# andreeaiana/newsreclib

Hardware: AMD Instinct MI355X
Metric: impressions/sec (train step) NRMS MINDsmall-shape (higher is better)
Workload: dtype f32 (projections: 3xbf16 split MFMA); 1 GPU; NRMS pretrained-emb (d=300, 15 heads, Q=200) MINDsmall-shaped train step: B=128/GPU, H=50, C=5, L=30, V=70000, dropout 0.2, Adam lr 1e-4 (BASELINE.json configs[1]); global_batch=128, parallelism=dp1, gemm_engine=bf16x3

## Files before the change

### include/newsreclib_amd.h

```cpp
#ifndef NEWSRECLIB_AMD_H
#define NEWSRECLIB_AMD_H

#include <stddef.h>
#include <stdint.h>

#ifdef __cplusplus
extern "C" {
#endif

#define NRL_ABI_VERSION 19

#define NRL_OK 0
#define NRL_E_INVALID (-1)
#define NRL_E_WORKSPACE (-2)
#define NRL_E_HIP (-3)

typedef struct NrlBlockParams {
  const float* in_proj_weight;
  const float* in_proj_bias;
  const float* out_proj_weight;
  const float* out_proj_bias;
  const float* att_weight;
  const float* att_bias;
  const float* att_query;
  int32_t embed_dim;
  int32_t num_heads;
  int32_t query_dim;
  int32_t gemm_engine;
  int32_t options;
} NrlBlockParams;
#define NRL_OPTIONS_EXPLICIT 0x40000000

typedef struct NrlBlockGrads {
  float* in_proj_weight;
  float* in_proj_bias;
  float* out_proj_weight;
  float* out_proj_bias;
  float* att_weight;
  float* att_bias;
  float* att_query;
} NrlBlockGrads;

int nrl_abi_version(void);
const char* nrl_build_id(void);
const char* nrl_last_error(void);

int nrl_set_gemm_engine(int32_t engine);
int nrl_get_gemm_engine(void);

int nrl_set_option(const char* name, int32_t value);
int32_t nrl_get_options(void);

int nrl_prof_enable(int32_t on);
int nrl_prof_read(double* total_ms, int64_t* launches, double* total_flops);

uint32_t nrl_dropout_key(uint64_t seed, uint32_t stream);
int nrl_dropout_mask(uint8_t* keep, int64_t n_elems, double p, uint64_t seed, uint32_t stream,
                     void* stream_handle);

size_t nrl_sort_positions_workspace_bytes(int64_t n, int64_t vocab);
int nrl_sort_positions(const int64_t* ids, int64_t n, int64_t vocab, int64_t* order, void* ws, size_t ws_bytes,
                       void* stream);

size_t nrl_news_encoder_workspace_bytes(int64_t n_news, int32_t seq_len, int32_t embed_dim,
                                        int32_t num_heads, int32_t query_dim);
int nrl_news_encoder_fwd(const NrlBlockParams* p, const float* emb_table, int64_t vocab,
                         const int64_t* ids, int64_t n_news, int32_t seq_len, double p_drop,
                         uint64_t seed, uint32_t stream0, int32_t save_for_backward, float* out,
                         void* ws, size_t ws_bytes, void* stream);
int32_t nrl_token_table_supported(int32_t seq_len, int32_t embed_dim, int32_t num_heads, int32_t query_dim);
size_t nrl_token_table_bytes(int64_t vocab, int32_t embed_dim, int32_t num_heads, int32_t query_dim);
int nrl_token_table_build(const NrlBlockParams* p, const float* emb_table, int64_t vocab, void* table, size_t table_bytes,
                          void* stream);
size_t nrl_news_encoder_fwd_table_workspace_bytes(int64_t n_news, int32_t seq_len, int32_t num_heads);
int nrl_news_encoder_fwd_table(const NrlBlockParams* p, const void* table, size_t table_bytes, int64_t vocab,
                               const int64_t* ids, int64_t n_news, int32_t seq_len, float* out, void* ws, size_t ws_bytes,
                               void* stream);
int nrl_news_encoder_bwd(const NrlBlockParams* p, const NrlBlockGrads* g, const float* emb_table,
                         float* d_emb_table, int64_t vocab, const int64_t* ids, const int64_t* sorted_positions,
                         int64_t n_news, int32_t seq_len, double p_drop, uint64_t seed,
                         uint32_t stream0, const float* d_out, int32_t phase, void* ws,
                         size_t ws_bytes, void* stream);

size_t nrl_user_encoder_workspace_bytes(int64_t batch, int64_t hist_len, int32_t embed_dim,
                                        int32_t num_heads, int32_t query_dim);
int nrl_user_encoder_fwd(const NrlBlockParams* p, const float* hist, int64_t batch,
                         int64_t hist_len, double p_drop, uint64_t seed, uint32_t stream0,
                         int32_t input_dropout, int32_t save_for_backward, float* out, void* ws,
                         size_t ws_bytes, void* stream);
int nrl_user_encoder_bwd(const NrlBlockParams* p, const NrlBlockGrads* g, const float* hist,
                         int64_t batch, int64_t hist_len, double p_drop, uint64_t seed,
                         uint32_t stream0, int32_t input_dropout, const float* d_out, float* d_hist,
                         void* ws, size_t ws_bytes, void* stream);
int nrl_user_encoder_bwd_phase(const NrlBlockParams* p, const NrlBlockGrads* g, const float* hist,
                               int64_t batch, int64_t hist_len, double p_drop, uint64_t seed,
                               uint32_t stream0, int32_t input_dropout, const float* d_out,
                               float* d_hist, int32_t phase, void* ws, size_t ws_bytes, void* stream);

int nrl_to_dense_batch_fwd(const float* x, const int64_t* offsets, int64_t batch, int64_t max_len,
                           int32_t dim, float* dense, void* stream);
int nrl_to_dense_batch_bwd(const float* d_dense, const int64_t* offsets, int64_t batch,
                           int64_t max_len, int32_t dim, int64_t n_rows, float* d_x, void* stream);

int nrl_hist_mean_fwd(const float* hist, const int64_t* offsets, int64_t batch, int64_t max_len,
                      int32_t dim, float* user, void* stream);
int nrl_hist_mean_bwd(const float* d_user, const int64_t* offsets, int64_t batch, int64_t max_len,
                      int32_t dim, float* d_hist, void* stream);

int nrl_dot_scores_fwd(const float* user, const float* cand, int64_t batch, int64_t n_cand,
                       int32_t dim, float* scores, void* stream);
int nrl_dot_scores_bwd(const float* d_scores, const float* user, const float* cand, int64_t batch,
                       int64_t n_cand, int32_t dim, float* d_user, float* d_cand, void* stream);

int nrl_ce_loss_fwd_bwd(const float* scores, const float* y_true, int64_t batch, int64_t n_cand,
                        float grad_scale, float* loss, float* d_scores, void* stream);

int nrl_supcon_loss_fwd_bwd(const float* scores, const float* y_true, const int64_t* cand_sizes, int64_t batch,
                            int64_t n_cand, float temperature, float grad_scale, float* loss, float* d_scores,
                            void* stream);

int nrl_adam_step(float* param, float* grad, float* exp_avg, float* exp_avg_sq, int64_t n,
                  double lr, double beta1, double beta2, double eps, int64_t step, float grad_scale,
                  int32_t zero_grad, void* stream);

int nrl_adam_rows_mark(const int64_t* ids, int64_t n_ids, int64_t rows, int32_t* mark, int64_t step, void* stream);
int nrl_adam_rows_advance(float* param, float* grad, float* exp_avg, float* exp_avg_sq, int64_t rows, int32_t dim,
                          int32_t* last_step, const int32_t* mark, int32_t* status, int64_t stride, int64_t offset,
                          int64_t upto_step, int32_t with_grad, double lr, double beta1, double beta2, double eps,
                          float grad_scale, const int32_t* exclude_mark, int32_t exclude_tag, void* stream);

int nrl_dropout_add_layernorm_fwd(const float* x, const float* residual, const float* gamma, const float* beta, int64_t rows,
                                  int32_t dim, float eps, double p_drop, uint64_t seed, uint32_t stream0, float* z_save,
                                  float* mean_save, float* rstd_save, float* y, void* stream);
int nrl_dropout_add_layernorm_bwd(const float* d_y, const float* z_saved, const float* gamma, const float* mean_saved,
                                  const float* rstd_saved, int64_t rows, int32_t dim, double p_drop, uint64_t seed,
                                  uint32_t stream0, float* d_x, float* d_residual, float* d_gamma, float* d_beta, void* stream);


typedef struct NrlCnnParams {
  const float* conv_weight;
  const float* conv_bias;
  const float* att_weight;
  const float* att_bias;
  const float* att_query;
  int32_t embed_dim;
  int32_t num_filters;
  int32_t window;
  int32_t query_dim;
} NrlCnnParams;

typedef struct NrlCnnGrads {
  float* conv_weight;
  float* conv_bias;
  float* att_weight;
  float* att_bias;
  float* att_query;
} NrlCnnGrads;

size_t nrl_cnn_encoder_workspace_bytes(int64_t n_news, int32_t seq_len, int32_t embed_dim,
                                       int32_t num_filters, int32_t window, int32_t query_dim);
int nrl_cnn_encoder_fwd(const NrlCnnParams* p, const float* emb_table, int64_t vocab,
                        const int64_t* ids, int64_t n_news, int32_t seq_len, double p_drop,
                        uint64_t seed, uint32_t stream0, int32_t save_for_backward, float* out,
                        void* ws, size_t ws_bytes, void* stream);
int nrl_cnn_encoder_bwd(const NrlCnnParams* p, const NrlCnnGrads* g, float* d_emb_table,
                        int64_t vocab, const int64_t* ids, const int64_t* sorted_positions,
                        int64_t n_news, int32_t seq_len, double p_drop, uint64_t seed,
                        uint32_t stream0, const float* d_out, void* ws, size_t ws_bytes,
                        void* stream);

size_t nrl_cnn_mhsa_encoder_workspace_bytes(int64_t n_news, int32_t seq_len, int32_t embed_dim,
                                            int32_t num_filters, int32_t window, int32_t num_heads,
                                            int32_t query_dim);
int nrl_cnn_mhsa_encoder_fwd(const NrlCnnParams* cp, const NrlBlockParams* bp, const float* emb_table,
                             int64_t vocab, const int64_t* ids, int64_t n_news, int32_t seq_len,
                             double p_drop, uint64_t seed, uint32_t stream0, int32_t save_for_backward,
                             float* out, void* ws, size_t ws_bytes, void* stream);
int nrl_cnn_mhsa_encoder_bwd(const NrlCnnParams* cp, const NrlCnnGrads* cg, const NrlBlockParams* bp,
                             const NrlBlockGrads* bg, float* d_emb_table, int64_t vocab,
                             const int64_t* ids, const int64_t* sorted_positions, int64_t n_news,
// ... 398 lines not shown
```

### newsreclib_amd/_lib.py

```python
from __future__ import annotations

import ctypes
import os
from ctypes import POINTER, c_char_p, c_double, c_float, c_int32, c_int64, c_size_t, c_uint8, c_uint32, c_uint64, c_void_p

_PKG = os.path.dirname(os.path.abspath(__file__))
LIB_PATH = os.path.join(_PKG, "libnewsreclib_amd.so")
ABI_VERSION = 19


class NrlBlockParams(ctypes.Structure):
    _fields_ = [
        ("in_proj_weight", c_void_p), ("in_proj_bias", c_void_p),
        ("out_proj_weight", c_void_p), ("out_proj_bias", c_void_p),
        ("att_weight", c_void_p), ("att_bias", c_void_p), ("att_query", c_void_p),
        ("embed_dim", c_int32), ("num_heads", c_int32), ("query_dim", c_int32), ("gemm_engine", c_int32),
        ("options", c_int32),
    ]


OPTIONS_EXPLICIT = 0x40000000


class NrlBlockGrads(ctypes.Structure):
# ... 40 lines not shown

class NrlDknGrads(ctypes.Structure):
    _fields_ = [("word_table", c_void_p), ("entity_table", c_void_p), ("context_table", c_void_p),
                ("transform_matrix", c_void_p), ("transform_bias", c_void_p), ("conv_weight", c_void_p * 4),
                ("conv_bias", c_void_p * 4)]


class NrlDknClickParams(ctypes.Structure):
    _fields_ = [("att_w1", c_void_p), ("att_b1", c_void_p), ("att_w2", c_void_p), ("att_b2", c_void_p),
                ("pred_w1", c_void_p), ("pred_b1", c_void_p), ("pred_w2", c_void_p), ("pred_b2", c_void_p),
                ("hidden", c_int32)]


class NrlDknClickGrads(ctypes.Structure):
    _fields_ = [("att_w1", c_void_p), ("att_b1", c_void_p), ("att_w2", c_void_p), ("att_b2", c_void_p),
                ("pred_w1", c_void_p), ("pred_b1", c_void_p), ("pred_w2", c_void_p), ("pred_b2", c_void_p)]


class NrlGruParams(ctypes.Structure):
    _fields_ = [("weight_ih", c_void_p), ("weight_hh", c_void_p), ("bias_ih", c_void_p), ("bias_hh", c_void_p),
                ("input_dim", c_int32), ("hidden_dim", c_int32)]


class NrlGruGrads(ctypes.Structure):
    _fields_ = [("weight_ih", c_void_p), ("weight_hh", c_void_p), ("bias_ih", c_void_p), ("bias_hh", c_void_p)]


class NrlAddAttParams(ctypes.Structure):
    _fields_ = [("att_weight", c_void_p), ("att_bias", c_void_p), ("att_query", c_void_p),
                ("dim", c_int32), ("query_dim", c_int32)]


class NrlAddAttGrads(ctypes.Structure):
    _fields_ = [("att_weight", c_void_p), ("att_bias", c_void_p), ("att_query", c_void_p)]


class NrlMhaParams(ctypes.Structure):
    _fields_ = [("in_proj_weight", c_void_p), ("in_proj_bias", c_void_p), ("out_proj_weight", c_void_p),
                ("out_proj_bias", c_void_p), ("embed_dim", c_int32), ("num_heads", c_int32), ("scale", ctypes.c_float),
                ("gemm_engine", c_int32)]


class NrlMhaGrads(ctypes.Structure):
    _fields_ = [("in_proj_weight", c_void_p), ("in_proj_bias", c_void_p), ("out_proj_weight", c_void_p),
                ("out_proj_bias", c_void_p)]


SIGNATURES = {
    "nrl_abi_version": (c_int32, []),
    "nrl_build_id": (c_char_p, []),
    "nrl_last_error": (c_char_p, []),
    "nrl_set_gemm_engine": (c_int32, [c_int32]),
    "nrl_get_gemm_engine": (c_int32, []),
    "nrl_set_option": (c_int32, [c_char_p, c_int32]),
    "nrl_get_options": (c_int32, []),
    "nrl_prof_enable": (c_int32, [c_int32]),
    "nrl_prof_read": (c_int32, [POINTER(c_double), POINTER(c_int64), POINTER(c_double)]),
    "nrl_dropout_key": (c_uint32, [c_uint64, c_uint32]),
    "nrl_dropout_mask": (c_int32, [c_void_p, c_int64, c_double, c_uint64, c_uint32, c_void_p]),
    "nrl_sort_positions_workspace_bytes": (c_size_t, [c_int64, c_int64]),
    "nrl_sort_positions": (c_int32, [c_void_p, c_int64, c_int64, c_void_p, c_void_p, c_size_t, c_void_p]),
    "nrl_news_encoder_workspace_bytes": (c_size_t, [c_int64, c_int32, c_int32, c_int32, c_int32]),
    "nrl_news_encoder_fwd": (c_int32, [POINTER(NrlBlockParams), c_void_p, c_int64, c_void_p, c_int64, c_int32,
                                       c_double, c_uint64, c_uint32, c_int32, c_void_p, c_void_p, c_size_t,
                                       c_void_p]),
    "nrl_token_table_supported": (c_int32, [c_int32, c_int32, c_int32, c_int32]),
    "nrl_token_table_bytes": (c_size_t, [c_int64, c_int32, c_int32, c_int32]),
    "nrl_token_table_build": (c_int32, [POINTER(NrlBlockParams), c_void_p, c_int64, c_void_p, c_size_t, c_void_p]),
    "nrl_news_encoder_fwd_table_workspace_bytes": (c_size_t, [c_int64, c_int32, c_int32]),
    "nrl_news_encoder_fwd_table": (c_int32, [POINTER(NrlBlockParams), c_void_p, c_size_t, c_int64, c_void_p, c_int64, c_int32,
                                             c_void_p, c_void_p, c_size_t, c_void_p]),
    "nrl_news_encoder_bwd": (c_int32, [POINTER(NrlBlockParams), POINTER(NrlBlockGrads), c_void_p, c_void_p, c_int64,
                                       c_void_p, c_void_p, c_int64, c_int32, c_double, c_uint64, c_uint32,
                                       c_void_p, c_int32, c_void_p, c_size_t, c_void_p]),
    "nrl_user_encoder_workspace_bytes": (c_size_t, [c_int64, c_int64, c_int32, c_int32, c_int32]),
    "nrl_user_encoder_fwd": (c_int32, [POINTER(NrlBlockParams), c_void_p, c_int64, c_int64, c_double, c_uint64,
                                       c_uint32, c_int32, c_int32, c_void_p, c_void_p, c_size_t, c_void_p]),
    "nrl_user_encoder_bwd": (c_int32, [POINTER(NrlBlockParams), POINTER(NrlBlockGrads), c_void_p, c_int64,
                                       c_int64, c_double, c_uint64, c_uint32, c_int32, c_void_p, c_void_p, c_void_p,
                                       c_size_t, c_void_p]),
    "nrl_user_encoder_bwd_phase": (c_int32, [POINTER(NrlBlockParams), POINTER(NrlBlockGrads), c_void_p, c_int64,
                                             c_int64, c_double, c_uint64, c_uint32, c_int32, c_void_p, c_void_p, c_int32,
                                             c_void_p, c_size_t, c_void_p]),
    "nrl_to_dense_batch_fwd": (c_int32, [c_void_p, c_void_p, c_int64, c_int64, c_int32, c_void_p, c_void_p]),
    "nrl_to_dense_batch_bwd": (c_int32, [c_void_p, c_void_p, c_int64, c_int64, c_int32, c_int64, c_void_p,
                                         c_void_p]),
    "nrl_hist_mean_fwd": (c_int32, [c_void_p, c_void_p, c_int64, c_int64, c_int32, c_void_p, c_void_p]),
    "nrl_hist_mean_bwd": (c_int32, [c_void_p, c_void_p, c_int64, c_int64, c_int32, c_void_p, c_void_p]),
    "nrl_dot_scores_fwd": (c_int32, [c_void_p, c_void_p, c_int64, c_int64, c_int32, c_void_p, c_void_p]),
    "nrl_dot_scores_bwd": (c_int32, [c_void_p, c_void_p, c_void_p, c_int64, c_int64, c_int32, c_void_p,
                                     c_void_p, c_void_p]),
    "nrl_ce_loss_fwd_bwd": (c_int32, [c_void_p, c_void_p, c_int64, c_int64, c_float, c_void_p, c_void_p,
                                      c_void_p]),
    "nrl_supcon_loss_fwd_bwd": (c_int32, [c_void_p, c_void_p, c_void_p, c_int64, c_int64, ctypes.c_float,
                                          ctypes.c_float, c_void_p, c_void_p, c_void_p]),
    "nrl_adam_step": (c_int32, [c_void_p, c_void_p, c_void_p, c_void_p, c_int64, c_double, c_double, c_double,
                                c_double, c_int64, c_float, c_int32, c_void_p]),
    "nrl_adam_rows_mark": (c_int32, [c_void_p, c_int64, c_int64, c_void_p, c_int64, c_void_p]),
    "nrl_adam_rows_advance": (c_int32, [c_void_p, c_void_p, c_void_p, c_void_p, c_int64, c_int32, c_void_p, c_void_p, c_void_p,
                                        c_int64, c_int64, c_int64, c_int32, c_double, c_double, c_double, c_double, c_float,
                                        c_void_p, c_int32, c_void_p]),
    "nrl_dropout_add_layernorm_fwd": (c_int32, [c_void_p, c_void_p, c_void_p, c_void_p, c_int64, c_int32, c_float, c_double,
                                                c_uint64, c_uint32, c_void_p, c_void_p, c_void_p, c_void_p, c_void_p]),
    "nrl_dropout_add_layernorm_bwd": (c_int32, [c_void_p, c_void_p, c_void_p, c_void_p, c_void_p, c_int64, c_int32, c_double,
                                                c_uint64, c_uint32, c_void_p, c_void_p, c_void_p, c_void_p, c_void_p]),
    "nrl_cnn_encoder_workspace_bytes": (c_size_t, [c_int64, c_int32, c_int32, c_int32, c_int32, c_int32]),
    "nrl_cnn_encoder_fwd": (c_int32, [POINTER(NrlCnnParams), c_void_p, c_int64, c_void_p, c_int64, c_int32,
                                      c_double, c_uint64, c_uint32, c_int32, c_void_p, c_void_p, c_size_t,
                                      c_void_p]),
    "nrl_cnn_encoder_bwd": (c_int32, [POINTER(NrlCnnParams), POINTER(NrlCnnGrads), c_void_p, c_int64, c_void_p,
                                      c_void_p, c_int64, c_int32, c_double, c_uint64, c_uint32, c_void_p,
                                      c_void_p, c_size_t, c_void_p]),
    "nrl_cnn_mhsa_encoder_workspace_bytes": (c_size_t, [c_int64, c_int32, c_int32, c_int32, c_int32, c_int32, c_int32]),
    "nrl_cnn_mhsa_encoder_fwd": (c_int32, [POINTER(NrlCnnParams), POINTER(NrlBlockParams), c_void_p, c_int64, c_void_p,
                                           c_int64, c_int32, c_double, c_uint64, c_uint32, c_int32, c_void_p, c_void_p,
                                           c_size_t, c_void_p]),
    "nrl_cnn_mhsa_encoder_bwd": (c_int32, [POINTER(NrlCnnParams), POINTER(NrlCnnGrads), POINTER(NrlBlockParams),
                                           POINTER(NrlBlockGrads), c_void_p, c_int64, c_void_p, c_void_p, c_int64,
                                           c_int32, c_double, c_uint64, c_uint32, c_void_p, c_void_p, c_size_t,
                                           c_void_p]),
    "nrl_npa_encoder_workspace_bytes": (c_size_t, [c_int64, c_int32, c_int32, c_int32, c_int32]),
    "nrl_npa_encoder_fwd": (c_int32, [POINTER(NrlCnnParams), c_void_p, c_int64, c_void_p, c_int64, c_int32, c_void_p,
                                      c_void_p, c_int64, c_double, c_uint64, c_uint32, c_int32, c_void_p, c_void_p,
                                      c_size_t, c_void_p]),
    "nrl_npa_encoder_bwd": (c_int32, [POINTER(NrlCnnParams), POINTER(NrlCnnGrads), c_void_p, c_int64, c_void_p,
                                      c_void_p, c_int64, c_int32, c_void_p, c_void_p, c_void_p, c_int64, c_double,
                                      c_uint64, c_uint32, c_void_p, c_void_p, c_void_p, c_size_t, c_void_p]),
    "nrl_npa_conv_features_workspace_bytes": (c_size_t, [c_int64, c_int32, c_int32, c_int32, c_int32]),
    "nrl_npa_conv_features": (c_int32, [POINTER(NrlCnnParams), c_void_p, c_int64, c_void_p, c_int64, c_int32, c_void_p,
                                        c_void_p, c_size_t, c_void_p]),
    "nrl_npa_cached_scores": (c_int32, [c_void_p, c_int64, c_int32, c_int32, c_void_p, c_int64, c_void_p, c_void_p, c_int64,
                                        c_void_p, c_int64, c_void_p, c_void_p, c_void_p, c_int32, c_int32, c_void_p,
                                        c_void_p, c_void_p]),
    "nrl_npa_user_queries_workspace_bytes": (c_size_t, [POINTER(NrlNpaQueryParams), c_int64]),
    "nrl_npa_user_queries_fwd": (c_int32, [POINTER(NrlNpaQueryParams), c_void_p, c_int64, c_double, c_uint64, c_uint32,
                                           c_void_p, c_void_p, c_void_p]),
    "nrl_npa_user_queries_bwd": (c_int32, [POINTER(NrlNpaQueryParams), POINTER(NrlNpaQueryGrads), c_void_p, c_int64,
                                           c_double, c_uint64, c_uint32, c_void_p, c_void_p, c_void_p, c_size_t,
                                           c_void_p]),
    "nrl_personalized_user_attention_fwd": (c_int32, [c_void_p, c_void_p, c_int64, c_int32, c_int32, c_void_p, c_void_p,
                                                      c_void_p]),
    "nrl_personalized_user_attention_bwd": (c_int32, [c_void_p, c_void_p, c_int64, c_int32, c_int32, c_void_p, c_void_p,
                                                      c_void_p, c_void_p, c_void_p]),
    "nrl_dkn_encoder_workspace_bytes": (c_size_t, [POINTER(NrlDknParams), c_int64, c_int32]),
    "nrl_dkn_encoder_fwd": (c_int32, [POINTER(NrlDknParams), c_void_p, c_void_p, c_int64, c_int32, c_void_p, c_void_p,
                                      c_void_p, c_size_t, c_void_p]),
    "nrl_dkn_encoder_bwd": (c_int32, [POINTER(NrlDknParams), POINTER(NrlDknGrads), c_void_p, c_void_p, c_void_p,
                                      c_void_p, c_int64, c_int32, c_void_p, c_void_p, c_void_p, c_void_p, c_size_t,
                                      c_void_p]),
    "nrl_dkn_click_workspace_bytes": (c_size_t, [c_int64, c_int32, c_int32, c_int32]),
    "nrl_dkn_click_fwd": (c_int32, [POINTER(NrlDknClickParams), c_void_p, c_void_p, c_int32, c_void_p, c_void_p, c_int64,
                                    c_int32, c_int32, c_void_p, c_void_p, c_void_p]),
    "nrl_dkn_click_bwd": (c_int32, [POINTER(NrlDknClickParams), POINTER(NrlDknClickGrads), c_void_p, c_void_p, c_int32,
                                    c_void_p, c_void_p, c_int64, c_int32, c_int32, c_void_p, c_void_p, c_void_p, c_void_p,
                                    c_void_p, c_size_t, c_void_p]),
    "nrl_dkn_user_query": (c_int32, [POINTER(NrlDknClickParams), c_void_p, c_void_p, c_int32, c_int64, c_int32, c_void_p,
                                     c_void_p, c_void_p]),
    "nrl_dkn_cand_project": (c_int32, [POINTER(NrlDknClickParams), c_void_p, c_int64, c_int32, c_void_p, c_void_p]),
    "nrl_caum_attn_fwd": (c_int32, [c_void_p, c_void_p, c_void_p, c_int64, c_int64, c_int32, c_int32, c_int32, c_float,
                                    c_void_p]),
    "nrl_caum_attn_bwd": (c_int32, [c_void_p, c_void_p, c_void_p, c_void_p, c_void_p, c_int64, c_int64, c_int32, c_int32,
                                    c_int32, c_float, c_void_p]),
    "nrl_caum_dropout": (c_int32, [c_void_p, c_void_p, c_int64, c_double, c_uint64, c_uint32, c_void_p]),
    "nrl_caum_expand_fwd": (c_int32, [c_void_p, c_void_p, c_int64, c_int32, c_int32, c_int32, c_double, c_uint64, c_uint32,
                                      c_void_p, c_void_p, c_void_p]),
    "nrl_caum_expand_bwd": (c_int32, [c_void_p, c_void_p, c_int64, c_int32, c_int32, c_int32, c_double, c_uint64, c_uint32,
# ... 214 lines not shown
```

### newsreclib_amd/abstract_recommender.py

```python
from __future__ import annotations

import contextlib
import json
from typing import Any, Dict, List, Tuple

import numpy as np
import torch
import torch.distributed as dist

from ._lightning import LightningModuleBase
from . import ops
from .dense_batch import dense_rows
from .metrics import StreamingMetrics, aspect_metrics, ranking_metrics
from .news_encoder import token_tables


STEP_OUTPUT_NAMES = ("loss", "preds", "targets", "cand_news_size", "hist_news_size", "target_categories", "target_sentiments",
                     "hist_categories", "hist_sentiments", "user_ids", "cand_news_ids")
_RECS_OUTPUTS = ("user_ids", "cand_news_ids", "preds", "cand_news_size")


class AbstractRecommender(LightningModuleBase):
    device_metrics = False

    def _init_step_outputs(self, outputs: Dict) -> None:
        self.step_outputs = {stage: {key: [] for key in keys} for stage, keys in outputs.items()}
        self.training_step_outputs = {key: [] for key in self.step_outputs.get("train", {})}
        self.val_step_outputs = {key: [] for key in self.step_outputs.get("val", {})}
        self.test_step_outputs = {key: [] for key in self.step_outputs.get("test", {})}
        self._loss_sums = {"train": [0.0, 0], "val": [0.0, 0], "test": [0.0, 0]}
        self.val_loss_best = float("inf")

    def _get_loss(self, criterion: str):
        from .click_predictor import CrossEntropyLoss, SupConLoss
        if criterion == "cross_entropy_loss":
            return CrossEntropyLoss()
        if criterion == "sup_con_loss":
            return SupConLoss()
        if criterion == "dual_loss":
            return CrossEntropyLoss(), SupConLoss()
        raise ValueError(f"Loss not defined: {criterion}")

    def _init_loss(self, loss: str, dual_loss_training: bool, dual_loss_coef) -> None:
        if not dual_loss_training:
            self.criterion = self._get_loss(loss)
            if isinstance(self.criterion, tuple):
                raise ValueError("loss='dual_loss' needs dual_loss_training=True")
        else:
            assert isinstance(dual_loss_coef, float)
            self.ce_criterion, self.scl_criterion = self._get_loss(loss)

    def _loss(self, scores: torch.Tensor, y_true: torch.Tensor, batch: Dict) -> torch.Tensor:
        hp = self.hparams
        if hp.loss == "cross_entropy_loss":
            return self.criterion(scores, y_true)
        sizes = batch["cand_sizes"]
        if not hp.dual_loss_training:
            return self.criterion(scores, y_true, sizes)
        ce_loss = self.ce_criterion(scores, y_true)
        scl_loss = self.scl_criterion(scores, y_true, sizes)
        return (1 - hp.dual_loss_coef) * ce_loss + hp.dual_loss_coef * scl_loss

    def _plm_text_encoder(self, plm_model, frozen_layers, embed_dim, num_heads, query_dim, dropout_probability):
        from .news_encoder import PLM
        assert isinstance(plm_model, str)
        return PLM(plm_model=plm_model, frozen_layers=frozen_layers, embed_dim=embed_dim, use_mhsa=True,
                   apply_reduce_dim=False, reduced_embed_dim=None, num_heads=num_heads, query_dim=query_dim,
                   dropout_probability=dropout_probability)

    def _encode_news(self, batch: Dict, seed=None):
        if self.hparams.use_plm:
            self.news_encoder.share_plm_bodies(batch["x_hist"], batch["x_cand"])
            return (self.news_encoder(batch["x_hist"], seed=seed),
                    self.news_encoder(batch["x_cand"], seed=seed, stream_base=4))
        n_hist = batch["batch_hist"].shape[0]
        news_vector = self.news_encoder(batch["x_all"], seed=seed)
        return ops.split_rows(news_vector, n_hist)

    def _init_embedding(self, filepath: str) -> torch.Tensor:
        return torch.from_numpy(np.load(filepath)).float()

    def model_step(self, batch: Dict) -> Tuple:
        batch = self._prepare(batch)
        B = batch["batch_size"]
        out = self.forward(batch)
        scores, aux = out if isinstance(out, tuple) else (out, None)
        y_true = dense_rows(batch["labels"], batch["batch_cand"], B, batch["max_cand"],
                            batch["cand_offsets"], batch["cand_flat_idx"], max_is_exact=True)
        loss = self._loss(scores, y_true.float(), batch)
        if aux is not None:
            loss = loss + self._aux_loss(batch, aux)

        if batch["labels"].shape[0] == scores.numel():
            preds = scores.detach().reshape(-1)
        else:
            preds = scores.detach().reshape(-1)[batch["cand_flat_idx"]]
        targets = batch["labels"]
        cand_news_size, hist_news_size = batch["cand_sizes"], batch["hist_sizes"]

        def attr(side, name):
            v = batch["x_" + side].get(name)
            return v if v is not None else torch.empty(0, dtype=torch.int64, device=scores.device)

        return (loss, preds, targets, cand_news_size, hist_news_size, attr("cand", "category"),
                attr("cand", "sentiment"), attr("hist", "category"), attr("hist", "sentiment"),
                batch["user_ids"], attr("cand", "news_ids"))

    def _collect_step_outputs(self, outputs_dict, local_vars):
        for key in outputs_dict.keys():
            outputs_dict[key].append(local_vars.get(key, []))
        return outputs_dict

    def _track(self, stage, loss):
        s = self._loss_sums[stage]
        s[0] = s[0] + loss.detach()
        s[1] += 1

    def training_step(self, batch: Dict, batch_idx: int):
        loss, preds, targets, cand_news_size, *_ = self.model_step(batch)
        self._track("train", loss)
        self.training_step_outputs = self._collect_step_outputs(self.training_step_outputs, locals())
        return loss

    def validation_step(self, batch: Dict, batch_idx: int):
        if self.device_metrics:
            return self._device_metrics_step("val", self.val_step_outputs, self.model_step(batch))
        loss, preds, targets, cand_news_size, *_ = self.model_step(batch)
        self._track("val", loss)
        self.val_step_outputs = self._collect_step_outputs(self.val_step_outputs, locals())

    def test_step(self, batch: Dict, batch_idx: int):
        if self.device_metrics:
            return self._device_metrics_step("test", self.test_step_outputs, self.model_step(batch))
        (loss, preds, targets, cand_news_size, hist_news_size, target_categories, target_sentiments,
         hist_categories, hist_sentiments, user_ids, cand_news_ids) = self.model_step(batch)
        self._track("test", loss)
        self.test_step_outputs = self._collect_step_outputs(self.test_step_outputs, locals())

    def _stream_metrics(self, stage: str, outputs: Dict[str, list]) -> StreamingMetrics:
        if self._world() > 1:
            raise NotImplementedError("device_metrics = True runs in a single process: the cross-rank reduction of the metric "
                                      "accumulator is not built; leave the attribute False under data parallelism")
        streams = self.__dict__.setdefault("_stream_metrics_by_stage", {})
        if stage not in streams:
            def ncls(asp, attr):
                wanted = all(k in outputs for k in (f"target_{asp}", f"hist_{asp}", "hist_news_size"))
                return getattr(self, attr, None) if wanted else None
            streams[stage] = StreamingMetrics(self.hparams.top_k_list, ncls("categories", "num_categ_classes"),
                                              ncls("sentiments", "num_sent_classes"))
        return streams[stage]

    def _device_metrics_step(self, stage: str, outputs: Dict[str, list], step: Tuple) -> None:
        self._track(stage, step[0])
        if all(k in outputs for k in ("preds", "targets", "cand_news_size")):
            self._stream_metrics(stage, outputs).update(step)
        if stage == "test" and getattr(self.hparams, "save_recs", False):
            named = dict(zip(STEP_OUTPUT_NAMES, step))
            for k in _RECS_OUTPUTS:
                if k in outputs:
                    outputs[k].append(named[k])

    @staticmethod
    def _world() -> int:
        return dist.get_world_size() if dist.is_available() and dist.is_initialized() else 1

    def _gather_outputs(self, outputs: Dict[str, list]) -> Dict[str, list]:
        if self._world() == 1:
            return outputs
        local = {k: [t.detach().cpu() for t in v if torch.is_tensor(t)] for k, v in outputs.items()}
        gathered: List[Dict[str, list]] = [None] * self._world()
        dist.all_gather_object(gathered, local)
        dev = self.device
        return {k: [t.to(dev) for part in gathered for t in part.get(k, [])] for k in outputs}

    def _epoch_end(self, stage: str, outputs: Dict[str, list]) -> Dict[str, float]:
# ... 101 lines not shown
```

### newsreclib_amd/csrc/nrl_api.hip

```cpp
#include "nrl_api_internal.h"

namespace nrl {

static thread_local char g_err[512] = "";

void set_error(const char* fmt, ...) {
  va_list ap;
  va_start(ap, fmt);
  vsnprintf(g_err, sizeof(g_err), fmt, ap);
  va_end(ap);
}

ProfState g_prof;
std::atomic<int> g_default_engine{ENGINE_BF16X3};
thread_local int t_engine = -1;
thread_local int64_t t_opts = -1;

static const char* const kOptName[O_COUNT] = {"news_fused", "news_fused_bwd", "news_attn_mfma", "news_planes", "news_od_planes",
                                              "news_aa_planes", "wgrad_2step", "wgrad_ws", "rowpanel", "x3_dma", "news_tail",
                                              "news_tail_bwd", "user_fork", "news_fork", "news_qkv_planes", "news_pad_share", "news_tail_od", "user_proj"};
static const char* const kOptEnv[O_COUNT] = {"NRL_NEWS_FUSED", "NRL_NEWS_FUSED_BWD", "NRL_NEWS_ATTN_MFMA", "NRL_NEWS_PLANES",
                                             "NRL_NEWS_OD_PLANES", "NRL_NEWS_AA_PLANES", "NRL_WGRAD_2STEP", "NRL_WGRAD_WS",
                                             "NRL_ROWPANEL", "NRL_X3_DMA", "NRL_NEWS_TAIL", "NRL_NEWS_TAIL_BWD", "NRL_USER_FORK",
                                             "NRL_NEWS_FORK", "NRL_NEWS_QKV_PLANES", "NRL_NEWS_PAD_SHARE", "NRL_NEWS_TAIL_OD", "NRL_USER_PROJ"};
// ... 312 lines not shown
                         float* d_emb_table, int64_t vocab, const int64_t* ids, const int64_t* sorted_positions,
                         int64_t n_news, int32_t seq_len, double p_drop, uint64_t seed, uint32_t stream0,
                         const float* d_out, int32_t phase, void* ws, size_t ws_bytes, void* stream) {
  NRL_TRY(check_params(p));
  const EngineScope engine_scope(p->gemm_engine);
  const OptScope opt_scope(p->options);
  NRL_TRY(check_grads(g));
  NRL_REQUIRE(d_emb_table && ids && d_out && vocab > 0 && n_news >= 0 && seq_len > 0, "news_encoder_bwd: bad arguments");
  NRL_REQUIRE(phase >= 0 && phase <= 2, "news_encoder_bwd: phase must be 0 (all), 1 or 2");
  if (n_news == 0) return NRL_OK;
  hipStream_t st = (hipStream_t)stream;
  const BlockShape s = news_shape(p, n_news, seq_len);
  BlockWs w;
  NRL_TRY(carve_ws(ws, ws_bytes, s, true, &w));
  const Dropout d1 = make_dropout(p_drop, seed, stream0), d2 = make_dropout(p_drop, seed, stream0 + 1);
  BlockPlanes bp;
  const bool slabs = news_fused_on(s, seq_len) && opt(O_NEWS_ATTN_MFMA);
  const bool planes = slabs && opt(O_NEWS_PLANES);
  BlockShape sb_ = s;
  sb_.od_planes = planes && opt(O_NEWS_OD_PLANES);
  sb_.aa_planes = sb_.od_planes && opt(O_NEWS_AA_PLANES) && w.yp != nullptr && (s.D & 15) == 12 && s.Q <= 224;
  sb_.tail = news_tail_on(sb_, seq_len, w);
  sb_.tail_bwd = sb_.tail && sb_.aa_planes && news_tail_bwd_on(sb_, seq_len, w);
  NRL_TRY(block_planes(p, s, w, false, &bp, st, slabs ? s.heads : 0));
  sb_.forked = news_fork_on(sb_);
  SideFork side;
  hipEvent_t side_in_join = nullptr;
  if (phase != 2) {
    if (sb_.forked) {
      ForkSet* fs = nullptr;
      NRL_TRY(fork_set(&fs));
      side.s = fs->s[0]; side.fork = fs->fork; side.join = fs->join[0];
    }
    NRL_TRY(block_bwd_phase1(p, g, sb_, w, bp, d2, d_out, st, slabs, sb_.forked ? &side : nullptr));
    if (slabs) {
      NewsAttnBwdArgs a;
      a.qkv_hm = w.qkv; a.d_o = w.d_o; a.lse = w.lse; a.dqkv = w.dqkv; a.n_news = n_news; a.L = seq_len; a.D = s.D;
      a.heads = s.heads; a.scale = s.geom.scale; a.hpw = 1; a.planes = planes ? 1 : 0;
      if (planes && opt(O_NEWS_QKV_PLANES)) NRL_TRY(launch_news_attn_bwd_p(a, st));
      else NRL_TRY(launch_news_attn_bwd(a, st));
      if (news_fork_in_on(sb_, planes)) {
        ForkSet* fs = nullptr;
        NRL_TRY(fork_set(&fs));
        const int si = news_fork_in_mode() == 2 ? 0 : 1;
        NRL_HIP(hipEventRecord(fs->fork, st));
        NRL_HIP(hipStreamWaitEvent(fs->s[si], fs->fork, 0));
        NRL_TRY(block_wgrad_in_planes(g, w.x, sb_, w, fs->s[si]));
        NRL_HIP(hipEventRecord(fs->join[1], fs->s[si]));
        side_in_join = fs->join[1];
      }
    }
    const KCSlab dq_hp{w.dqkv, s.M};
    const KCPlanes dq_pl{reinterpret_cast<const unsigned char*>(w.dqkv), s.pad_rows};
    if (sorted_positions != nullptr) {
      float* dx = w.d_o;
      const EpiLinear epi{dx, s.D, nullptr, 0, d1, s.D};
      static const bool live_env = [] { const char* e = getenv("NRL_LIVE_ROWS"); return !(e != nullptr && e[0] == '0'); }();
      if (planes && live_env) {
        NRL_REQUIRE((size_t)s.M * s.heads >= live_compact_ints(s.M), "news_encoder_bwd: scratch for the live-row list");
        const int32_t *list = nullptr, *cidx = nullptr, *n_live = nullptr;
        NRL_TRY(live_compact(ids, s.M, reinterpret_cast<int32_t*>(w.lse), &list, &cidx, &n_live, st));
        const KCPlanesLive dq_live{reinterpret_cast<const unsigned char*>(w.dqkv), s.pad_rows, list, n_live, seq_len};
        NRL_TRY(rp_dispatch(dq_live, bp.rp.in_d_hp, EpiDxLive{dx, s.D, d1, list}, s.M, s.D, s.heads * 64, st));
        NRL_TRY(embedding_grad_sorted(dx, ids, sorted_positions, s.M, s.D, d_emb_table, st, cidx));
      } else {
        if (planes) NRL_TRY(rp_dispatch(dq_pl, bp.rp.in_d_hp, EpiNewsRows<EpiLinear>{epi, seq_len}, s.pad_rows, s.D, s.heads * 64, st));
        else if (slabs) NRL_TRY(rp_dispatch(dq_hp, bp.rp.in_d_hp, epi, s.M, s.D, s.heads * 64, st));
        else NRL_TRY(gemm_dgrad(w.dqkv, p->in_proj_weight, bp.in, epi, s.M, 3 * s.D, s.D, st, bp.rp.on ? &bp.rp.in_d : nullptr));
        NRL_TRY(embedding_grad_sorted(dx, ids, sorted_positions, s.M, s.D, d_emb_table, st));
      }
    } else {
      const EpiScatter epi{d_emb_table, ids, s.D, d1};
      if (planes) NRL_TRY(rp_dispatch(dq_pl, bp.rp.in_d_hp, EpiNewsRows<EpiScatter>{epi, seq_len}, s.pad_rows, s.D, s.heads * 64, st));
      else if (slabs) NRL_TRY(rp_dispatch(dq_hp, bp.rp.in_d_hp, epi, s.M, s.D, s.heads * 64, st));
      else NRL_TRY(gemm_dgrad(w.dqkv, p->in_proj_weight, bp.in, epi, s.M, 3 * s.D, s.D, st, bp.rp.on ? &bp.rp.in_d : nullptr));
    }
  }
  if (phase != 2 && sb_.forked) NRL_HIP(hipStreamWaitEvent(st, side.join, 0));
  if (side_in_join != nullptr) NRL_HIP(hipStreamWaitEvent(st, side_in_join, 0));
  if (phase != 1) NRL_TRY(block_bwd_phase2(g, w.x, sb_, w, st, slabs, planes));
  return NRL_OK;
}

size_t nrl_user_encoder_workspace_bytes(int64_t batch, int64_t hist_len, int32_t embed_dim,
                                        int32_t num_heads, int32_t query_dim) {
  return block_ws_bytes(batch * hist_len, embed_dim, query_dim, num_heads, true);
}

int nrl_user_encoder_fwd(const NrlBlockParams* p, const float* hist, int64_t batch, int64_t hist_len,
                         double p_drop, uint64_t seed, uint32_t stream0, int32_t input_dropout,
                         int32_t save_for_backward, float* out, void* ws, size_t ws_bytes, void* stream) {
  NRL_TRY(check_params(p));
  const EngineScope engine_scope(p->gemm_engine);
  const OptScope opt_scope(p->options);
  NRL_REQUIRE(hist && out && batch > 0 && hist_len > 0, "user_encoder_fwd: bad arguments");
  NRL_REQUIRE(((uintptr_t)hist & 15) == 0, "hist must be 16-byte aligned");
  NRL_REQUIRE(p_drop >= 0.0 && p_drop < 1.0, "dropout probability must be in [0, 1)");
  const BlockShape s = user_shape(p, batch, hist_len);
  NRL_REQUIRE(p_drop == 0.0 || s.M * s.D < (1LL << 32), "activation too large for the 32-bit dropout index space");
  BlockWs w;
  NRL_TRY(carve_ws(ws, ws_bytes, s, true, &w));
  const Dropout d2 = make_dropout(p_drop, seed, stream0 + 1);
  if (p_drop > 0.0 && input_dropout) {
    const Dropout d1 = make_dropout(p_drop, seed, stream0);
    return block_fwd(p, KCGather{hist, nullptr, s.M, s.D, d1, save_for_backward ? w.x : nullptr}, s, w, d2,
                     save_for_backward != 0, false, out, (hipStream_t)stream);
  }
  return block_fwd(p, KCPlain{hist, s.D, s.M}, s, w, d2, save_for_backward != 0, false, out, (hipStream_t)stream);
}

int nrl_user_encoder_bwd(const NrlBlockParams* p, const NrlBlockGrads* g, const float* hist,
                         int64_t batch, int64_t hist_len, double p_drop, uint64_t seed, uint32_t stream0,
                         int32_t input_dropout, const float* d_out, float* d_hist, void* ws, size_t ws_bytes,
                         void* stream) {
  return nrl_user_encoder_bwd_phase(p, g, hist, batch, hist_len, p_drop, seed, stream0, input_dropout, d_out, d_hist, 0, ws,
                                    ws_bytes, stream);
}

int nrl_user_encoder_bwd_phase(const NrlBlockParams* p, const NrlBlockGrads* g, const float* hist,
                               int64_t batch, int64_t hist_len, double p_drop, uint64_t seed, uint32_t stream0,
                               int32_t input_dropout, const float* d_out, float* d_hist, int32_t phase, void* ws,
                               size_t ws_bytes, void* stream) {
  NRL_TRY(check_params(p));
  const EngineScope engine_scope(p->gemm_engine);
  const OptScope opt_scope(p->options);
  NRL_TRY(check_grads(g));
  NRL_REQUIRE(phase >= 0 && phase <= 2, "user_encoder_bwd: phase must be 0 (both), 1 or 2");
  NRL_REQUIRE(hist && batch > 0 && hist_len > 0 && (phase == 2 || (d_out && d_hist)), "user_encoder_bwd: bad arguments");
  hipStream_t st = (hipStream_t)stream;
  const BlockShape s = user_shape(p, batch, hist_len);
  BlockWs w;
  NRL_TRY(carve_ws(ws, ws_bytes, s, true, &w));
  const bool in_drop = p_drop > 0.0 && input_dropout;
  const Dropout d1 = make_dropout(in_drop ? p_drop : 0.0, seed, stream0), d2 = make_dropout(p_drop, seed, stream0 + 1);
  const float* x_rows = in_drop ? w.x : hist;
  if (phase == 2) return block_bwd_phase2(g, x_rows, s, w, st);
  BlockPlanes bp;
  NRL_TRY(block_planes(p, s, w, false, &bp, st));
  NRL_TRY(block_bwd_phase1(p, g, s, w, bp, d2, d_out, st));
  if (phase == 1)
    return gemm_dgrad(w.dqkv, p->in_proj_weight, bp.in, EpiLinear{d_hist, s.D, nullptr, 0, d1, s.D}, s.M, 3 * s.D, s.D, st,
                      bp.rp.on ? &bp.rp.in_d : nullptr);
  if (!opt(O_USER_FORK) || s.M > 65536) {
    NRL_TRY(gemm_dgrad(w.dqkv, p->in_proj_weight, bp.in, EpiLinear{d_hist, s.D, nullptr, 0, d1, s.D}, s.M, 3 * s.D,
                       s.D, st, bp.rp.on ? &bp.rp.in_d : nullptr));
    return block_bwd_phase2(g, x_rows, s, w, st);
  }
  ForkSet* fs = nullptr;
  NRL_TRY(fork_set(&fs));
  NRL_HIP(hipEventRecord(fs->fork, st));
  for (int i = 0; i < 2; ++i) NRL_HIP(hipStreamWaitEvent(fs->s[i], fs->fork, 0));
  const size_t third = opt(O_WGRAD_2STEP) ? qkv_elems(s.M, s.D, s.heads, s.pad_rows) / 3 / 64 * 64 : 0;
  float* const sc = third > 0 ? w.qkv : nullptr;
  int rc = gemm_dgrad(w.dqkv, p->in_proj_weight, bp.in, EpiLinear{d_hist, s.D, nullptr, 0, d1, s.D}, s.M, 3 * s.D, s.D, st,
                      bp.rp.on ? &bp.rp.in_d : nullptr);
  if (rc == NRL_OK) rc = gemm_wgrad(w.dqkv, 3 * s.D, x_rows, s.D, g->in_proj_weight, g->in_proj_bias, s.M, fs->s[0], sc, third);
  if (rc == NRL_OK)
    rc = gemm_wgrad(w.dy, s.D, w.o, s.D, g->out_proj_weight, g->out_proj_bias, s.M, fs->s[1], sc ? sc + third : nullptr, third);
  if (rc == NRL_OK)
    rc = gemm_wgrad(w.t, s.Q, w.y, s.D, g->att_weight, g->att_bias, s.M, fs->s[1], sc ? sc + 2 * third : nullptr, third);
  for (int i = 0; i < 2; ++i) {
    NRL_HIP(hipEventRecord(fs->join[i], fs->s[i]));
    NRL_HIP(hipStreamWaitEvent(st, fs->join[i], 0));
  }
  return rc;
}

int nrl_to_dense_batch_fwd(const float* x, const int64_t* offsets, int64_t batch, int64_t max_len,
                           int32_t dim, float* dense, void* stream) {
  NRL_REQUIRE(offsets && dense && batch >= 0 && max_len >= 0 && dim > 0, "to_dense_batch_fwd: bad arguments");
  return to_dense_fwd(x, offsets, batch, max_len, dim, dense, (hipStream_t)stream);
}

int nrl_to_dense_batch_bwd(const float* d_dense, const int64_t* offsets, int64_t batch,
                           int64_t max_len, int32_t dim, int64_t n_rows, float* d_x, void* stream) {
  NRL_REQUIRE(offsets && d_dense && batch >= 0 && max_len >= 0 && dim > 0, "to_dense_batch_bwd: bad arguments");
  return to_dense_bwd(d_dense, offsets, batch, max_len, dim, n_rows, d_x, (hipStream_t)stream);
}

int nrl_hist_mean_fwd(const float* hist, const int64_t* offsets, int64_t batch, int64_t max_len, int32_t dim,
                      float* user, void* stream) {
  NRL_REQUIRE(hist && offsets && user && batch >= 0 && max_len >= 0 && dim > 0, "hist_mean_fwd: bad arguments");
  return hist_mean_fwd(hist, offsets, batch, max_len, dim, user, (hipStream_t)stream);
}

int nrl_hist_mean_bwd(const float* d_user, const int64_t* offsets, int64_t batch, int64_t max_len, int32_t dim,
                      float* d_hist, void* stream) {
  NRL_REQUIRE(d_user && offsets && d_hist && batch >= 0 && max_len >= 0 && dim > 0, "hist_mean_bwd: bad arguments");
  return hist_mean_bwd(d_user, offsets, batch, max_len, dim, d_hist, (hipStream_t)stream);
}

int nrl_dot_scores_fwd(const float* user, const float* cand, int64_t batch, int64_t n_cand,
                       int32_t dim, float* scores, void* stream) {
  NRL_REQUIRE(user && cand && scores && batch >= 0 && n_cand >= 0 && dim > 0, "dot_scores_fwd: bad arguments");
  return dot_scores_fwd(user, cand, batch, n_cand, dim, scores, (hipStream_t)stream);
}

int nrl_dot_scores_bwd(const float* d_scores, const float* user, const float* cand, int64_t batch,
                       int64_t n_cand, int32_t dim, float* d_user, float* d_cand, void* stream) {
  NRL_REQUIRE(d_scores && user && cand && d_user && d_cand && dim > 0, "dot_scores_bwd: bad arguments");
  return dot_scores_bwd(d_scores, user, cand, batch, n_cand, dim, d_user, d_cand, (hipStream_t)stream);
}

int nrl_ce_loss_fwd_bwd(const float* scores, const float* y_true, int64_t batch, int64_t n_cand,
                        float grad_scale, float* loss, float* d_scores, void* stream) {
  NRL_REQUIRE(scores && y_true && loss, "ce_loss: bad arguments");
  return ce_loss_fwd_bwd(scores, y_true, batch, n_cand, grad_scale, loss, d_scores, (hipStream_t)stream);
}

int nrl_supcon_loss_fwd_bwd(const float* scores, const float* y_true, const int64_t* cand_sizes, int64_t batch,
                            int64_t n_cand, float temperature, float grad_scale, float* loss, float* d_scores,
                            void* stream) {
  NRL_REQUIRE(scores && y_true && cand_sizes && loss, "supcon_loss: bad arguments");
  return supcon_loss_fwd_bwd(scores, y_true, cand_sizes, batch, n_cand, temperature, grad_scale, loss, d_scores,
                             (hipStream_t)stream);
}

int nrl_adam_step(float* param, float* grad, float* exp_avg, float* exp_avg_sq, int64_t n, double lr,
                  double beta1, double beta2, double eps, int64_t step, float grad_scale,
                  int32_t zero_grad, void* stream) {
  NRL_REQUIRE(param && grad && exp_avg && exp_avg_sq && n >= 0, "adam_step: bad arguments");
  return adam_step(param, grad, exp_avg, exp_avg_sq, n, lr, beta1, beta2, eps, step, grad_scale, zero_grad,
                   (hipStream_t)stream);
}

int nrl_adam_rows_mark(const int64_t* ids, int64_t n_ids, int64_t rows, int32_t* mark, int64_t step, void* stream) {
  NRL_REQUIRE((ids || n_ids == 0) && mark && n_ids >= 0 && rows > 0, "adam_rows_mark: bad arguments");
  return adam_rows_mark(ids, n_ids, rows, mark, step, (hipStream_t)stream);
}

int nrl_adam_rows_advance(float* param, float* grad, float* exp_avg, float* exp_avg_sq, int64_t rows, int32_t dim,
                          int32_t* last_step, const int32_t* mark, int32_t* status, int64_t stride, int64_t offset,
                          int64_t upto_step, int32_t with_grad, double lr, double beta1, double beta2, double eps,
                          float grad_scale, const int32_t* exclude_mark, int32_t exclude_tag, void* stream) {
  return adam_rows_advance(param, grad, exp_avg, exp_avg_sq, rows, dim, last_step, mark, status, stride, offset, upto_step,
                           with_grad, lr, beta1, beta2, eps, grad_scale, (hipStream_t)stream, exclude_mark, exclude_tag);
}

int nrl_embedding_gather(const float* table, const int64_t* ids, int64_t n_ids, int32_t dim,
                         float* out, void* stream) {
  NRL_REQUIRE(table && ids && out && n_ids >= 0 && dim > 0, "embedding_gather: bad arguments");
  return embedding_gather(table, ids, n_ids, dim, out, (hipStream_t)stream);
}

static void linear_layout(Arena& a, int n, int k, uint16_t** img) {
  size_t e = split_weight_elems(n, k);
  if (lin_image_elems(n, k) > e) e = lin_image_elems(n, k);
  if (lin_image_elems(k, n) > e) e = lin_image_elems(k, n);
// ... 173 lines not shown
```

### newsreclib_amd/csrc/nrl_api_internal.h

```cpp
#pragma once
#include <stdarg.h>
#include <stdlib.h>
#include <string.h>

#include <atomic>
#include <utility>
#include <vector>

#include "nrl_gemm.h"
#include "nrl_gemm_bf16x3.h"
#include "nrl_gemm_bf16x3_dma.h"
#include "nrl_rowpanel.h"
#include "nrl_gemm_ws.h"
#include "nrl_news_fused.h"
#include "nrl_news_tail_api.h"
#include "nrl_user_tail.h"
#include "nrl_wgrad_planes.h"
#include "nrl_kernels.h"
#include "nrl_conv.h"
#include "nrl_gru_fused.h"

namespace nrl {

struct ProfState {
// ... 112 lines not shown
static size_t block_rp_elems(int D, int Q) {
  if (!block_rp_ok(D, Q)) return 0;
  const int nd = rp_nblk_for(D), nq = rp_nblk_for(Q);
  return rp_image_elems(nd, rp_kblocks(D, false)) * 2
         + rp_image_elems(nq, rp_kblocks(D, false))
         + rp_image_elems(nd, rp_kblocks(Q, false))
         + rp_image_elems(nd, rp_kblocks(3 * D, false))
         + rp_image_elems((D / 20) * 4, NF_KB)
         + rp_image_elems(nd, (D / 20) * 2)
         + rp_image_elems(nd, rp_kblocks(D + 32, false))
         + rp_image_elems(NT_FB, NT_KB) + rp_image_elems(NT_QB, NT_KS)
         + rp_image_elems(NT_FB, NT_QS);
}

static size_t plane_elems(int D, int Q) {
  return split_weight_elems(3 * D, D) + split_weight_elems(D, D) + split_weight_elems(Q, D);
}

static size_t qkv_elems(int64_t M, int D, int heads, int64_t pad_rows) {
  const size_t packed = (size_t)M * 3 * D, slabs = (size_t)(pad_rows > M ? pad_rows : M) * heads * 64;
  return (D == heads * 20 && slabs > packed) ? slabs : packed;
}
static size_t x_elems(int64_t M, int D, int64_t pad_rows) {
  const size_t rows = (size_t)M * D, planes = (size_t)pad_rows * 320;
  return planes > rows ? planes : rows;
}

static size_t od_elems(int64_t M, int D, int heads, int64_t pad_rows) {
  const size_t rows = (size_t)M * D;
  if (pad_rows <= 0 || D != heads * 20) return rows;
  const size_t planes = (size_t)((M + 31) / 32 * 32) * (size_t)(heads + (heads + 3) / 4) * 16;
  return planes > rows ? planes : rows;
}

static void block_layout(Arena& a, int64_t M, int D, int Q, int heads, bool with_x, int64_t pad_rows, BlockWs* out) {
  const size_t rows32 = (size_t)((M + 31) / 32 * 32);
  out->x = with_x ? a.take<float>(x_elems(M, D, pad_rows)) : nullptr;
  out->qkv = a.take<float>(qkv_elems(M, D, heads, pad_rows));
  out->dqkv = a.take<float>(qkv_elems(M, D, heads, pad_rows));
  out->o = a.take<float>(od_elems(M, D, heads, pad_rows));
  out->y = a.take<float>((size_t)M * D);
  out->dy = a.take<float>(od_elems(M, D, heads, pad_rows));
  out->yp = out->tp = nullptr;
  if (pad_rows > 0 && D == heads * 20) {
    out->yp = a.take<float>(rows32 * ((D + 16) / 16) * 16);
    out->tp = a.take<float>(rows32 * ((Q + 15) / 16) * 16);
  }
  out->d_o = a.take<float>((size_t)M * D);
  out->t = a.take<float>((size_t)M * Q);
  out->w = a.take<float>((size_t)M);
  out->lse = a.take<float>((size_t)M * heads);
  out->planes = a.take<uint16_t>(plane_elems(D, Q));
  out->rp = a.take<uint16_t>(block_rp_elems(D, Q));
}
static size_t block_ws_bytes(int64_t M, int D, int Q, int heads, bool with_x, int64_t pad_rows = 0) {
  return measure_workspace<BlockWs>([&](Arena& a, auto* w) { block_layout(a, M, D, Q, heads, with_x, pad_rows, w); });
}
static int carve_ws(void* ws, size_t ws_bytes, const BlockShape& s, bool with_x, BlockWs* out) {
  return carve_workspace(ws, ws_bytes, [&](Arena& a) { block_layout(a, s.M, s.D, s.Q, s.heads, with_x, s.pad_rows, out); });
}

static int check_params(const NrlBlockParams* p) {
  NRL_REQUIRE(p != nullptr, "params struct is null");
  NRL_REQUIRE(p->in_proj_weight && p->in_proj_bias && p->out_proj_weight && p->out_proj_bias &&
                  p->att_weight && p->att_bias && p->att_query, "null parameter pointer");
  NRL_REQUIRE(engine_field_ok(p->gemm_engine), "gemm_engine must be 0 (default), 1 (f32) or 2 (bf16x3)");
  NRL_REQUIRE(options_field_ok(p->options), "options must be 0 (process defaults) or NRL_OPTIONS_EXPLICIT | switch mask");
  NRL_REQUIRE(p->embed_dim > 0 && p->embed_dim % 4 == 0, "embed_dim must be a positive multiple of 4");
  NRL_REQUIRE(p->query_dim > 0 && p->query_dim % 4 == 0, "query_dim must be a positive multiple of 4");
  NRL_REQUIRE(p->num_heads > 0 && p->embed_dim % p->num_heads == 0, "embed_dim must be divisible by num_heads");
  NRL_REQUIRE(attn_head_dim_supported(p->embed_dim / p->num_heads),
              "head dim %d unsupported (16, 20, 32, 48, 64)", p->embed_dim / p->num_heads);
  NRL_REQUIRE((((uintptr_t)p->in_proj_weight | (uintptr_t)p->out_proj_weight | (uintptr_t)p->att_weight) & 15) == 0,
              "weight matrices must be 16-byte aligned");
  return NRL_OK;
}

struct BlockPlanes {
  SplitWeight in, out, att;
  BlockRp rp;
};

static int block_planes(const NrlBlockParams* P, const BlockShape& s, const BlockWs& w, bool fill,
                        BlockPlanes* bp, hipStream_t st, int fused_heads = 0, int proj_heads = 0) {
  const int D = s.D, Q = s.Q;
  uint16_t* p = w.planes;
  const float* ws[3] = {P->in_proj_weight, P->out_proj_weight, P->att_weight};
  const int ns[3] = {3 * D, D, Q};
  SplitWeight* outs[3] = {&bp->in, &bp->out, &bp->att};
  bp->rp.on = block_rp_ok(D, Q) && cur_engine() == ENGINE_BF16X3;
  for (int i = 0; i < 3; ++i) {
    const bool needed = i == 0 ? !((fused_heads > 0 || proj_heads > 0) && bp->rp.on) : !bp->rp.on;
    if (fill && needed) {
      NRL_TRY(split_weight(ws[i], ns[i], D, p, outs[i], st));
    } else {
      *outs[i] = split_weight_view(p, ns[i], D);
    }
    p += split_weight_elems(ns[i], D);
  }
  if (bp->rp.on) {
    const int nd = rp_nblk_for(D), nq = rp_nblk_for(Q);
    uint16_t* q = w.rp;
    RpImageJobs jobs;
    rp_jobs_init(&jobs);
    auto add = [&](RpImage* im, const float* src, int64_t sn, int64_t sk, int N, int K, int nblk) {
      im->img = q; im->nblk = nblk; im->kblocks = rp_kblocks(K, false);
      if (fill) rp_jobs_add(&jobs, src, sn, sk, N, K, nullptr, q, nblk);
      q += rp_image_elems(nblk, im->kblocks);
    };
    add(&bp->rp.out_f, P->out_proj_weight, D, 1, D, D, nd);
    add(&bp->rp.att_f, P->att_weight, D, 1, Q, D, nq);
    add(&bp->rp.att_d, P->att_weight, 1, D, D, Q, nd);
    add(&bp->rp.out_d, P->out_proj_weight, 1, D, D, D, nd);
    add(&bp->rp.in_d, P->in_proj_weight, 1, D, D, 3 * D, nd);
    if (fused_heads > 0) {
      bp->rp.in_heads.img = q; bp->rp.in_heads.nblk = fused_heads * 4; bp->rp.in_heads.kblocks = NF_KB;
      if (fill) rp_jobs_add_qkv_heads(&jobs, P->in_proj_weight, D, P->in_proj_bias, q, fused_heads, D / fused_heads);
      q += rp_image_elems(fused_heads * 4, NF_KB);
      bp->rp.in_d_hp.img = q; bp->rp.in_d_hp.nblk = nd; bp->rp.in_d_hp.kblocks = fused_heads * 2;
      if (fill) rp_jobs_add_kheads(&jobs, P->in_proj_weight, 1, D, D, fused_heads, D / fused_heads, q, nd);
      q += rp_image_elems(nd, fused_heads * 2);
      bp->rp.out_f_perm.img = q; bp->rp.out_f_perm.nblk = nd;
      bp->rp.out_f_perm.kblocks = (16 * (fused_heads + (fused_heads + 3) / 4) + 31) / 32;
      if (fill) rp_jobs_add_kperm(&jobs, P->out_proj_weight, D, 1, D, fused_heads, q, nd);
      q += rp_image_elems(nd, rp_kblocks(D + 32, false));
      if (opt(O_NEWS_TAIL) && news_tail_geometry_ok(32, D, Q, fused_heads)) {
        bp->rp.tail_o.img = q; bp->rp.tail_o.nblk = NT_FB; bp->rp.tail_o.kblocks = NT_KB;
        if (fill) rp_jobs_add_kperm(&jobs, P->out_proj_weight, D, 1, D, fused_heads, q, NT_FB, P->out_proj_bias);
        q += rp_image_elems(NT_FB, NT_KB);
        bp->rp.tail_a.img = q; bp->rp.tail_a.nblk = NT_QB; bp->rp.tail_a.kblocks = NT_KS;
        if (fill) rp_jobs_add_kappa(&jobs, P->att_weight, D, 1, Q, D, P->att_bias, q, NT_QB, NT_KS);
        q += rp_image_elems(NT_QB, NT_KS);
        bp->rp.tail_ad.img = q; bp->rp.tail_ad.nblk = NT_FB; bp->rp.tail_ad.kblocks = NT_QS;
        if (fill && news_tail_bwd_geometry_ok(32, D, Q, fused_heads)) rp_jobs_add_kappa(&jobs, P->att_weight, 1, D, D, Q, nullptr, q, NT_FB, NT_QS);
        q += rp_image_elems(NT_FB, NT_QS);
      }
    } else if (proj_heads > 0) {
      bp->rp.in_heads.img = q; bp->rp.in_heads.nblk = proj_heads * 4; bp->rp.in_heads.kblocks = NF_KB;
      if (fill) rp_jobs_add_qkv_heads(&jobs, P->in_proj_weight, D, P->in_proj_bias, q, proj_heads, D / proj_heads);
      q += rp_image_elems(proj_heads * 4, NF_KB);
    }
    if (fill) NRL_TRY(rp_jobs_launch(jobs, st));
  }
  return NRL_OK;
}

template <class T, class = void>
struct HasStream : std::false_type {};
template <class T>
struct HasStream<T, std::void_t<decltype(std::declval<T&>().stream)>> : std::true_type {};
template <class Epi>
static Epi with_stream(Epi e, int64_t M, int N) {
  static const int64_t thresh = [] {
    const char* env = getenv("NRL_STREAM_MB");
    const int64_t mb = env != nullptr ? atoll(env) : 0;
    return mb <= 0 ? (int64_t)1 << 62 : mb << 20;
  }();
  if constexpr (HasStream<Epi>::value) e.stream = (M * N * (int64_t)sizeof(float) >= thresh) ? 1 : 0;
  return e;
}

template <class AOp, class Epi>
static int rp_dispatch(const AOp& a, const RpImage& b, const Epi& epi_in, int64_t M, int N, int K, hipStream_t st) {
  const Epi epi = with_stream(epi_in, M, N);
  static const int64_t half_rows = [] { const char* e = getenv("NRL_RP_HALF_ROWS"); return e ? atoll(e) : (int64_t)16384; }();
  if constexpr (std::is_same<AOp, KCPlain>::value) {
    if (M <= half_rows) {
      switch (b.nblk) {
        case 13: return launch_rp_gemm<13, 4, 0, 1>(a, b, epi, M, N, K, st);
        case 19: return launch_rp_gemm<19, 4, 0, 1>(a, b, epi, M, N, K, st);
        case 20: return launch_rp_gemm<20, 4, 0, 1>(a, b, epi, M, N, K, st);
      }
    }
  }
  switch (b.nblk) {
    case 13: return launch_rp_gemm<13>(a, b, epi, M, N, K, st);
    case 19: return launch_rp_gemm<19>(a, b, epi, M, N, K, st);
    case 20: return launch_rp_gemm<20>(a, b, epi, M, N, K, st);
  }
  set_error("row-panel GEMM: no instantiation for %d column blocks", b.nblk);
  return NRL_E_INVALID;
}

static bool big_tiles(int64_t M, int N) { return ceil_div(M, 256) * ceil_div(N, 160) >= 512; }

template <class AOp, class Epi>
static int gemm_fwd(const AOp& a, const float* W, const SplitWeight& sw, const Epi& epi_in, int64_t M, int N, int K,
// ... 42 lines not shown
      if (sp * tiles < 512) sp = ceil_div(512, tiles);
      const int64_t max_s = ceil_div(M, 256);
      return (int)(sp > max_s ? max_s : (sp < 1 ? 1 : sp));
    };
    if (I > 512 && opt(O_WGRAD_WS)) {
      static const int forced = [] { const char* e = getenv("NRL_WGRAD_WS_SPLITS"); return e ? atoi(e) : 0; }();
      int ws_splits = forced;
      if (ws_splits <= 0) {
        const int64_t tiles = ceil_div(I, 256) * ceil_div(J + 1, 160), ktiles = ceil_div(M, 32);
        int64_t best = -1;
        for (int sp = 8; sp <= 64; sp += 8) {
          if (sp > 8 && ktiles / sp < 8) break;
          const int64_t cost = ceil_div(tiles * sp, 256) * (ceil_div(ktiles, sp) + 12);
          if (best < 0 || cost < best) best = cost, ws_splits = sp;
        }
      }
      return launch_gemm_bf16x3_ws<4, 2, 2, 8, 5>(a, b, epi, I, J + 1, M, ws_splits, st, scratch, scratch_floats);
    }
    if (I > 512) return launch_gemm_bf16x3<X3_TILE_BIG>(a, b, epi, I, J + 1, M, splits(256), st);
    if (opt(O_X3_DMA)) return launch_gemm_bf16x3_dma_tn<2, 2, 2, 5, 2>(a, b, epi, I, J + 1, M, splits(64), st, scratch, scratch_floats);
    return launch_gemm_bf16x3<X3_TILE_W>(a, b, epi, I, J + 1, M, splits(64), st);
  }
  if (I > 512) return launch_gemm<NRL_TILE>(a, b, epi, I, J + 1, M, wgrad_splits(I, J + 1, M, 128, 160), st);
  return launch_gemm<NRL_TILE_W>(a, b, epi, I, J + 1, M, wgrad_splits(I, J + 1, M, 64, 160), st);
}

static __global__ void split_conv_weight_t_kernel(const float* __restrict__ w, int F, int D, int W, int Kp,
                                           uint16_t* __restrict__ hi) {
  const int64_t total = (int64_t)D * Kp;
  for (int64_t i = (int64_t)blockIdx.x * blockDim.x + threadIdx.x; i < total;
       i += (int64_t)gridDim.x * blockDim.x) {
    const int d = (int)(i / Kp), k = (int)(i % Kp);
    float v = 0.f;
    if (k < W * F) {
      const int tr = k / F, f = k - tr * F;
      v = w[((int64_t)f * W + (W - 1 - tr)) * D + d];
    }
    const __bf16 h = (__bf16)v;
    const int64_t pos = split_pos(d, k, 2 * Kp);
    hi[pos] = __builtin_bit_cast(unsigned short, h);
    hi[pos + 32] = __builtin_bit_cast(unsigned short, (__bf16)(v - (float)h));
  }
}

template <class AOp, class BRc, class Epi>
static int gemm_any(const AOp& a, const BRc& b_rc, const uint16_t* hi, const uint16_t* lo, int64_t ldp,
                    const Epi& epi, int64_t M, int N, int K, hipStream_t st, const RpImage* rp = nullptr) {
  if (cur_engine() == ENGINE_BF16X3) {
    if (rp != nullptr && rp->img != nullptr) return rp_dispatch(a, *rp, epi, M, N, K, st);
    const KCSplit b{hi, lo, ldp, N};
    return launch_gemm_bf16x3_dma<X3_DMA_TILE>(a, b, epi, M, N, K, st);
  }
  return launch_gemm<NRL_TILE>(a, b_rc, epi, M, N, K, 1, st);
}

template <class BOp>
static int gemm_wgrad_any(const float* dy, int I, const BOp& b, int J, float* dW, float* db, int64_t M,
                          hipStream_t st) {
  const RCPlain a{dy, I, I, 0};
  const EpiAtomicWB epi{dW, J, db, J};
  if (cur_engine() == ENGINE_BF16X3) {
    auto splits = [&](int bm) {
      const int64_t tiles = ceil_div(I, bm) * ceil_div(J + 1, 160);
      int64_t sp = ceil_div(M, 1664);
      if (sp * tiles < 512) sp = ceil_div(512, tiles);
      const int64_t max_s = ceil_div(M, 256);
      return (int)(sp > max_s ? max_s : (sp < 1 ? 1 : sp));
    };
    if (opt(O_X3_DMA)) return launch_gemm_bf16x3_dma_tn<2, 2, 2, 5, 2>(a, b, epi, I, J + 1, M, splits(64), st);
    return launch_gemm_bf16x3<X3_TILE_W>(a, b, epi, I, J + 1, M, splits(64), st);
  }
  return launch_gemm<NRL_TILE_W>(a, b, epi, I, J + 1, M, wgrad_splits(I, J + 1, M, 64, 160), st);
}

static int block_fwd_tail(const NrlBlockParams* P, const BlockShape& s, const BlockWs& w, const BlockPlanes& bp,
                          Dropout drop2, float* out, hipStream_t st);

static inline bool block_attn_x3(const BlockShape& s) {
  static const int min_s = [] { const char* e = getenv("NRL_ATTN_X3_MIN_S"); return e ? atoi(e) : 32; }();
  return cur_engine() == ENGINE_BF16X3 && s.geom.S >= min_s && attn_x3_ok(s.geom);
}

template <class AOp>
static int block_fwd(const NrlBlockParams* P, const AOp& a_in, const BlockShape& s, const BlockWs& w,
                     Dropout drop2, bool save, bool prof_in_proj, float* out, hipStream_t st) {
  const int D = s.D;
  const Dropout nodrop = make_dropout(0.0, 0, 0);
  BlockPlanes bp;
  bool proj = false;
  if constexpr (std::is_same<AOp, KCPlain>::value) {
    proj = opt(O_USER_PROJ) && cur_engine() == ENGINE_BF16X3 && block_rp_ok(D, s.Q) && block_attn_x3(s) && a_in.ld == D &&
           D == s.heads * 20 && attn_x3_proj_ok(s.geom, s.heads * 4, NF_KB) && s.geom.q_outer % 3 == 0 && s.geom.q_seq % 3 == 0;
  }
  NRL_TRY(block_planes(P, s, w, cur_engine() == ENGINE_BF16X3, &bp, st, 0, proj ? s.heads : 0));
  if constexpr (std::is_same<AOp, KCPlain>::value) {
    if (proj) {
      NRL_TRY(attn_fwd_x3_proj(a_in.p, s.geom.q_outer / 3, s.geom.q_seq / 3, bp.rp.in_heads.img, bp.rp.in_heads.nblk,
                               save ? w.qkv : nullptr, w.o, save ? w.lse : nullptr, s.geom, st));
      return block_fwd_tail(P, s, w, bp, drop2, out, st);
    }
  }
  {
    ProfScope prof(st, prof_in_proj ? 2.0 * (double)s.M * 3.0 * D * D : 0.0);
    NRL_TRY(gemm_fwd(a_in, P->in_proj_weight, bp.in, EpiLinear{w.qkv, 3 * D, P->in_proj_bias, 0, nodrop, 3 * D},
                     s.M, 3 * D, D, false, st));
  }
  if (block_attn_x3(s)) NRL_TRY(attn_fwd_x3(w.qkv, w.o, save ? w.lse : nullptr, s.geom, st));
  else NRL_TRY(attn_fwd(w.qkv, w.o, save ? w.lse : nullptr, s.geom, st));
  return block_fwd_tail(P, s, w, bp, drop2, out, st);
}

static int block_fwd_tail(const NrlBlockParams* P, const BlockShape& s, const BlockWs& w, const BlockPlanes& bp,
                          Dropout drop2, float* out, hipStream_t st) {
  const int D = s.D, Q = s.Q;
  const Dropout nodrop = make_dropout(0.0, 0, 0);
  if (!s.od_planes && !s.aa_planes && bp.rp.on &&
      user_tail_ok(s.pool_groups, s.pool_len, D, Q, bp.rp.out_f.nblk, bp.rp.att_f.nblk) && s.pool_groups * s.pool_len == s.M) {
    UserTailArgs a;
    a.o = w.o; a.img_o = bp.rp.out_f.img; a.img_a = bp.rp.att_f.img; a.nblk_o = bp.rp.out_f.nblk; a.nblk_a = bp.rp.att_f.nblk;
    a.b_o = P->out_proj_bias; a.b_a = P->att_bias; a.q_a = P->att_query; a.groups = s.pool_groups; a.H = s.pool_len; a.D = D;
    a.Q = Q; a.drop2 = drop2; a.y = w.y; a.t = w.t; a.w = w.w; a.out = out;
    return user_tail_fwd(a, st);
  }
  const int ncb_y = (D + 16) / 16;
  unsigned char* const ypl = reinterpret_cast<unsigned char*>(w.yp);
  if (s.od_planes) {
    const int ncb = s.heads + (s.heads + 3) / 4;
    const KCPlanesG a_o{reinterpret_cast<const unsigned char*>(w.o), s.M, ncb};
    const EpiLinear epi{w.y, D, P->out_proj_bias, 0, drop2, D};
    if (s.aa_planes) {
      if (s.M % 32 != 0)
        NRL_HIP(hipMemsetAsync(ypl + (s.M / 32) * 2 * ncb_y * 1024, 0, (size_t)2 * ncb_y * 1024, st));
      NRL_TRY(rp_dispatch(a_o, bp.rp.out_f_perm, EpiLinearPlanes{epi, ypl, ncb_y}, s.M, D, 16 * ncb, st));
    } else {
      NRL_TRY(rp_dispatch(a_o, bp.rp.out_f_perm, epi, s.M, D, 16 * ncb, st));
    }
  } else {
    NRL_TRY(gemm_fwd(KCPlain{w.o, D, s.M}, P->out_proj_weight, bp.out,
                     EpiLinear{w.y, D, P->out_proj_bias, 0, drop2, D}, s.M, D, D, false, st,
                     bp.rp.on ? &bp.rp.out_f : nullptr));
  }
  if (s.aa_planes) {
    NRL_TRY(rp_dispatch(KCPlanesG{ypl, s.M, ncb_y}, bp.rp.att_f, EpiLinear{w.t, Q, P->att_bias, 1, nodrop, Q}, s.M, Q, D, st));
  } else {
    NRL_TRY(gemm_fwd(KCPlain{w.y, D, s.M}, P->att_weight, bp.att, EpiLinear{w.t, Q, P->att_bias, 1, nodrop, Q},
                     s.M, Q, D, true, st, bp.rp.on ? &bp.rp.att_f : nullptr));
  }
  NRL_TRY(pool_fwd(w.t, P->att_query, w.y, s.pool_groups, s.pool_len, Q, D, w.w, out, st));
  return NRL_OK;
}

struct SideFork {
  hipStream_t s = nullptr;
  hipEvent_t fork = nullptr, join = nullptr;
};

static inline int wgrad_planes_waves() {
  static const int v = [] { const char* e = getenv("NRL_WGRAD_PLANES_WAVES"); return e ? atoi(e) : 8; }();
  return v;
}
template <int TM, int TN, class Epi>
static int wgrad_planes_g_dispatch(const void* a, int ncb_a, const void* b, int ncb_b, int64_t rows, int64_t m_valid, int n_valid,
                                   const Epi& epi, int nsplit, hipStream_t st, float* scratch) {
  if (wgrad_planes_waves() == 4) return launch_wgrad_planes_g<TM, TN, 4>(a, ncb_a, b, ncb_b, rows, m_valid, n_valid, epi, nsplit, st, scratch);
  return launch_wgrad_planes_g<TM, TN, 8>(a, ncb_a, b, ncb_b, rows, m_valid, n_valid, epi, nsplit, st, scratch);
}

static int block_wgrads_back_half(const NrlBlockGrads* G, const BlockShape& s, const BlockWs& w, hipStream_t st,
                                  float* scratch, size_t scratch_floats) {
  const int D = s.D, Q = s.Q;
  auto scratch_for = [&](size_t need) -> float* { return need <= scratch_floats ? scratch : nullptr; };
  {
    static const int sp = [] { const char* e = getenv("NRL_WGRAD_PLANES_AA_SPLITS"); return e ? atoi(e) : 128; }();
    NRL_TRY((wgrad_planes_g_dispatch<7, 5>(w.tp, (Q + 15) / 16, w.yp, (D + 16) / 16, (s.M + 31) / 32 * 32, Q, D + 1,
                                         EpiAtomicWB{G->att_weight, D, G->att_bias, D}, sp, st,
                                         scratch_for(wgrad_planes_g_scratch_floats(7, 5, (Q + 15) / 16, (D + 16) / 16, sp)))));
  }
  {
    static const int sp = [] { const char* e = getenv("NRL_WGRAD_PLANES_G_SPLITS"); return e ? atoi(e) : 64; }();
    const int ncb_o = s.heads + (s.heads + 3) / 4, ncb_dy = (D + 15) / 16;
    NRL_TRY((wgrad_planes_g_dispatch<5, 5>(w.dy, ncb_dy, w.o, ncb_o, (s.M + 31) / 32 * 32, D, 16 * ncb_o,
                                         EpiAtomicWBPerm{G->out_proj_weight, D, G->out_proj_bias, s.heads}, sp, st,
                                         scratch_for(wgrad_planes_g_scratch_floats(5, 5, ncb_dy, ncb_o, sp)))));
  }
  return NRL_OK;
}

static inline bool news_fork_on(const BlockShape& s) {
  return s.tail_bwd && s.aa_planes && s.od_planes && opt(O_NEWS_FORK) && opt(O_WGRAD_2STEP);
}

// ... 182 lines not shown
```

### newsreclib_amd/csrc/nrl_kernels.hip

```cpp
#include <math.h>
#include <stdlib.h>

#include "nrl_kernels.h"
#include <cfloat>

namespace nrl {

template <int DH>
__device__ __forceinline__ float dot_row(const float (&q)[DH], const float* row) {
  const float4* r4 = reinterpret_cast<const float4*>(row);
  float acc = 0.f;
#pragma unroll
  for (int d4 = 0; d4 < DH / 4; ++d4) {
    const float4 kv = r4[d4];
    acc = fmaf(q[4 * d4 + 0], kv.x, acc);
    acc = fmaf(q[4 * d4 + 1], kv.y, acc);
    acc = fmaf(q[4 * d4 + 2], kv.z, acc);
    acc = fmaf(q[4 * d4 + 3], kv.w, acc);
  }
  return acc;
}

template <int DH>
__device__ __forceinline__ void axpy_row(float a, const float* row, float (&o)[DH]) {
  const float4* r4 = reinterpret_cast<const float4*>(row);
#pragma unroll
  for (int d4 = 0; d4 < DH / 4; ++d4) {
    const float4 vv = r4[d4];
    o[4 * d4 + 0] = fmaf(a, vv.x, o[4 * d4 + 0]);
    o[4 * d4 + 1] = fmaf(a, vv.y, o[4 * d4 + 1]);
    o[4 * d4 + 2] = fmaf(a, vv.z, o[4 * d4 + 2]);
    o[4 * d4 + 3] = fmaf(a, vv.w, o[4 * d4 + 3]);
  }
}

template <int DH>
__device__ __forceinline__ void load_row(const float* src, float (&r)[DH], float mul) {
  const float4* s4 = reinterpret_cast<const float4*>(src);
#pragma unroll
  for (int d4 = 0; d4 < DH / 4; ++d4) {
    const float4 v = s4[d4];
    r[4 * d4 + 0] = v.x * mul;
    r[4 * d4 + 1] = v.y * mul;
    r[4 * d4 + 2] = v.z * mul;
    r[4 * d4 + 3] = v.w * mul;
  }
}

template <int DH>
__device__ __forceinline__ void store_row(float* dst, const float (&r)[DH], float mul) {
  float4* d4p = reinterpret_cast<float4*>(dst);
#pragma unroll
  for (int d4 = 0; d4 < DH / 4; ++d4)
    d4p[d4] = make_float4(r[4 * d4] * mul, r[4 * d4 + 1] * mul, r[4 * d4 + 2] * mul, r[4 * d4 + 3] * mul);
}

template <int DH>
__device__ __forceinline__ void attend_rows(const float (&q)[DH], const float* Ks, const float* Vs,
                                            int nrows, float& m, float& l, float (&o)[DH]) {
  for (int cb = 0; cb < nrows; cb += 8) {
    float s[8];
    float mx = -INFINITY;
#pragma unroll
    for (int u = 0; u < 8; ++u) {
      const int c = cb + u;
      const float acc = dot_row<DH>(q, Ks + (c < nrows ? c : 0) * DH);
      s[u] = c < nrows ? acc : -INFINITY;
      mx = fmaxf(mx, s[u]);
    }
    const float m_new = fmaxf(m, mx);
    const float alpha = expf(m - m_new);
    l *= alpha;
#pragma unroll
    for (int d = 0; d < DH; ++d) o[d] *= alpha;
#pragma unroll
    for (int u = 0; u < 8; ++u) {
      const int c = cb + u;
      const float p = expf(s[u] - m_new);
      l += p;
      axpy_row<DH>(p, Vs + (c < nrows ? c : 0) * DH, o);
    }
    m = m_new;
  }
}

// ... 598 lines not shown
    const float inv = 1.0f / (float)(offsets[b + 1] - offsets[b]);
    float4 acc = make_float4(0.f, 0.f, 0.f, 0.f);
    for (int64_t h = 0; h < max_len; ++h) {
      const float4 v = hist[(b * max_len + h) * D4 + d4];
      acc.x += v.x; acc.y += v.y; acc.z += v.z; acc.w += v.w;
    }
    user[i] = make_float4(acc.x * inv, acc.y * inv, acc.z * inv, acc.w * inv);
  }
}

__global__ void hist_mean_bwd_kernel(const float4* __restrict__ d_user, const int64_t* __restrict__ offsets,
                                     int64_t total4, int64_t max_len, int D4, float4* __restrict__ d_hist) {
  for (int64_t i = (int64_t)blockIdx.x * blockDim.x + threadIdx.x; i < total4;
       i += (int64_t)gridDim.x * blockDim.x) {
    const int d4 = (int)(i % D4);
    const int64_t b = (i / D4) / max_len;
    const float inv = 1.0f / (float)(offsets[b + 1] - offsets[b]);
    const float4 g = d_user[b * D4 + d4];
    d_hist[i] = make_float4(g.x * inv, g.y * inv, g.z * inv, g.w * inv);
  }
}

int hist_mean_fwd(const float* hist, const int64_t* offsets, int64_t B, int64_t max_len, int D, float* user,
                  hipStream_t stream) {
  NRL_REQUIRE(D % 4 == 0, "hist_mean: dim must be a multiple of 4");
  const int64_t total4 = B * (D / 4);
  if (total4 == 0) return NRL_OK;
  hipLaunchKernelGGL(hist_mean_fwd_kernel, dim3(grid_for(total4, 256)), dim3(256), 0, stream, (const float4*)hist,
                     offsets, total4, max_len, D / 4, (float4*)user);
  NRL_LAUNCH_CHECK();
  return NRL_OK;
}

int hist_mean_bwd(const float* d_user, const int64_t* offsets, int64_t B, int64_t max_len, int D, float* d_hist,
                  hipStream_t stream) {
  NRL_REQUIRE(D % 4 == 0, "hist_mean: dim must be a multiple of 4");
  const int64_t total4 = B * max_len * (D / 4);
  if (total4 == 0) return NRL_OK;
  hipLaunchKernelGGL(hist_mean_bwd_kernel, dim3(grid_for(total4, 256)), dim3(256), 0, stream, (const float4*)d_user,
                     offsets, total4, max_len, D / 4, (float4*)d_hist);
  NRL_LAUNCH_CHECK();
  return NRL_OK;
}

__global__ void __launch_bounds__(256)
    dot_scores_fwd_kernel(const float* __restrict__ user, const float* __restrict__ cand, int64_t BC,
                          int64_t C, int D, float* __restrict__ scores) {
  const int lane = threadIdx.x & 63;
  const int64_t pair = (int64_t)blockIdx.x * 4 + (threadIdx.x >> 6);
  if (pair >= BC) return;
  const float* u = user + (pair / C) * D;
  const float* cv = cand + pair * D;
  float part = 0.f;
  for (int d = lane; d < D; d += 64) part = fmaf(u[d], cv[d], part);
  part = wave_sum(part);
  if (lane == 0) scores[pair] = part;
}

__global__ void dot_scores_bwd_kernel(const float* __restrict__ ds, const float* __restrict__ user,
                                      const float* __restrict__ cand, int64_t B, int64_t C, int D,
                                      float* __restrict__ d_user, float* __restrict__ d_cand) {
  const int64_t i = (int64_t)blockIdx.x * blockDim.x + threadIdx.x;
  if (i >= B * D) return;
  const int64_t b = i / D;
  const int d = (int)(i % D);
  const float u = user[i];
  float acc = 0.f;
  for (int64_t c = 0; c < C; ++c) {
    const float s = ds[b * C + c];
    const int64_t idx = (b * C + c) * D + d;
    acc = fmaf(s, cand[idx], acc);
    d_cand[idx] = s * u;
  }
  d_user[i] = acc;
}

__global__ void __launch_bounds__(256)
    ce_kernel(const float* __restrict__ scores, const float* __restrict__ y, int64_t B, int64_t C,
              float grad_scale, float* __restrict__ loss, float* __restrict__ d_scores) {
  __shared__ float red[4];
  const int tid = threadIdx.x;
  float local = 0.f;
  const float invB = 1.0f / (float)B;
  for (int64_t b = tid; b < B; b += 256) {
    const float* s = scores + b * C;
    const float* yy = y + b * C;
    float mx = -INFINITY;
    for (int64_t c = 0; c < C; ++c) mx = fmaxf(mx, s[c]);
    float sum = 0.f, ysum = 0.f;
    for (int64_t c = 0; c < C; ++c) { sum += expf(s[c] - mx); ysum += yy[c]; }
    const float lse = mx + logf(sum);
    float lb = 0.f;
    for (int64_t c = 0; c < C; ++c) {
      const float logp = s[c] - lse;
      lb -= yy[c] * logp;
      if (d_scores != nullptr) d_scores[b * C + c] = (expf(logp) * ysum - yy[c]) * invB * grad_scale;
    }
    local += lb;
  }
  local = wave_sum(local);
  if ((tid & 63) == 0) red[tid >> 6] = local;
  __syncthreads();
  if (tid == 0) *loss = (red[0] + red[1] + red[2] + red[3]) * invB;
}

struct SupConRow {
  float loss, lse, mx;
  int npos, n;
};

__device__ __forceinline__ SupConRow supcon_row(const float* s, const float* y, int64_t C, int64_t n, float inv_t) {
  SupConRow r;
  r.n = (int)n;
  float mx = n > 0 ? -INFINITY : 0.f;
  for (int64_t c = 0; c < n; ++c) mx = fmaxf(mx, s[c] * inv_t);
  float sum = 0.f, possum = 0.f;
  int npos = 0;
  for (int64_t c = 0; c < n; ++c) {
    const float x = s[c] * inv_t - mx;
    sum += expf(x);
    if (y[c] != 0.f) { ++npos; possum += x; }
  }
  for (int64_t c = n; c < C; ++c) npos += y[c] != 0.f;
  r.mx = mx;
  r.npos = npos;
  r.lse = n > 0 ? logf(sum) : 0.f;
  r.loss = -(possum - (float)npos * r.lse) / ((float)npos + FLT_MIN);
  return r;
}

__global__ void __launch_bounds__(256)
    supcon_kernel(const float* __restrict__ scores, const float* __restrict__ y, const int64_t* __restrict__ sizes,
                  int64_t B, int64_t C, float inv_t, float grad_scale, float* __restrict__ loss,
                  float* __restrict__ d_scores) {
  __shared__ float red[4][4];
  const int tid = threadIdx.x;
  float lsum = 0.f, lcnt = 0.f, tpos = 0.f, tneg = 0.f;
  for (int64_t b = tid; b < B; b += 256) {
    const SupConRow r = supcon_row(scores + b * C, y + b * C, C, sizes[b], inv_t);
    if (r.loss > 0.f) { lsum += r.loss; lcnt += 1.f; }
    tpos += (float)r.npos;
    tneg += (float)(r.n - r.npos);
  }
  float v[4] = {wave_sum(lsum), wave_sum(lcnt), wave_sum(tpos), wave_sum(tneg)};
  if ((tid & 63) == 0)
    for (int i = 0; i < 4; ++i) red[i][tid >> 6] = v[i];
  __syncthreads();
  float tot[4];
  for (int i = 0; i < 4; ++i) tot[i] = red[i][0] + red[i][1] + red[i][2] + red[i][3];
  const bool zero = (tot[2] <= 1.f && tot[3] <= 1.f) || !(tot[2] > 0.f && tot[3] > 0.f) || tot[1] < 1.f;
  if (tid == 0) *loss = zero ? 0.f : tot[0] / tot[1];
  if (d_scores == nullptr) return;
  const float k = zero ? 0.f : inv_t * grad_scale / tot[1];
  for (int64_t b = tid; b < B; b += 256) {
    const float* s = scores + b * C;
    const float* yy = y + b * C;
    const int64_t n = sizes[b];
    const SupConRow r = supcon_row(s, yy, C, n, inv_t);
    const float live = (r.loss > 0.f) ? k / ((float)r.npos + FLT_MIN) : 0.f;
    for (int64_t c = 0; c < C; ++c) {
      float g = 0.f;
      if (c < n && live != 0.f) {
        const float p = expf(s[c] * inv_t - r.mx - r.lse);
        g = ((float)r.npos * p - (yy[c] != 0.f ? 1.f : 0.f)) * live;
      }
      d_scores[b * C + c] = g;
    }
  }
}

int supcon_loss_fwd_bwd(const float* scores, const float* y, const int64_t* sizes, int64_t B, int64_t C,
                        float temperature, float grad_scale, float* loss, float* d_scores, hipStream_t stream) {
  NRL_REQUIRE(B > 0 && C > 0 && temperature > 0.f, "supcon: bad arguments");
  hipLaunchKernelGGL(supcon_kernel, dim3(1), dim3(256), 0, stream, scores, y, sizes, B, C, 1.0f / temperature,
                     grad_scale, loss, d_scores);
  NRL_LAUNCH_CHECK();
  return NRL_OK;
}

int dot_scores_fwd(const float* user, const float* cand, int64_t B, int64_t C, int D, float* scores,
                   hipStream_t stream) {
  const int64_t BC = B * C;
// ... 645 lines not shown
```

### newsreclib_amd/csrc/nrl_rowpanel.h

```cpp
#pragma once
#include "nrl_gemm_bf16x3_dma.h"

namespace nrl {

struct RpImageJob {
  const float* src;
  const float* bias;
  uint16_t* img;
  int64_t sn, sk;
  int N, K, nblk, kblocks;
  int heads, dh;
  int conv_f, conv_w;
  int kheads, kdh;
  int kperm_heads;
  int kappa;
  int kpad_d, kpad_dp;
};
constexpr int RP_MAX_JOBS = 12;
struct RpImageJobs {
  RpImageJob job[RP_MAX_JOBS];
  int count;
  int overflow;
  int64_t first_thread[RP_MAX_JOBS + 1];
};

static inline int rp_kblocks(int K, bool bias) { return (K + (bias ? 1 : 0) + 31) / 32; }
static inline size_t rp_image_elems(int nblk, int kblocks) { return (size_t)kblocks * nblk * 1024; }

__device__ __forceinline__ int rp_image_row(const RpImageJob& J, int n) {
  if (J.heads <= 0) return n < J.N ? n : -1;
  const int head = n >> 6, c = n & 63;
  if (head >= J.heads || c >= 3 * J.dh) return -1;
  const int part = c / J.dh, d = c - part * J.dh;
  return part * (J.heads * J.dh) + head * J.dh + d;
}

static __global__ void __launch_bounds__(256) rp_weight_image_kernel(const RpImageJobs jobs) {
  const int64_t tid = (int64_t)blockIdx.x * 256 + threadIdx.x;
  if (tid >= jobs.first_thread[jobs.count]) return;
  int j = 0;
#pragma unroll
  for (int q = 1; q < RP_MAX_JOBS; ++q)
    if (q < jobs.count && tid >= jobs.first_thread[q]) j = q;
  const RpImageJob& J = jobs.job[j];
  const int64_t t = tid - jobs.first_thread[j];
  const int lane = (int)(t & 63);
  const int nb = (int)((t >> 6) % J.nblk), kb = (int)((t >> 6) / J.nblk);
  const int n = nb * 16 + (lane & 15), k0 = kb * 32 + 8 * (lane >> 4);
  const int row = rp_image_row(J, n);
  float v[8];
#pragma unroll
  for (int e = 0; e < 8; ++e) {
    int k = k0 + e;
    if (J.kappa != 0) {
      const int gg = lane >> 4;
      k = kb * 32 + (e < 4 ? 4 * gg + e : 16 + 4 * gg + (e - 4));
    }
    float x = 0.f;
    bool live = row >= 0;
    if (J.kperm_heads > 0) {
      const int cb = k >> 4, c = k & 15;
      int head, d;
      if (cb < J.kperm_heads) { head = cb; d = c; }
      else { head = 4 * (cb - J.kperm_heads) + (c >> 2); d = 16 + (c & 3); }
      if (head < J.kperm_heads) k = head * 20 + d;
      else if (k != J.K || J.bias == nullptr) live = false;
    }
    if (J.kpad_dp > 0) {
      const int tap = k / J.kpad_dp, d = k - tap * J.kpad_dp;
      live = live && d < J.kpad_d;
      k = tap * J.kpad_d + d;
    }
    if (J.kheads > 0) {
      const int head = k >> 6, c = k & 63;
      live = live && head < J.kheads && c < 3 * J.kdh;
      const int part = c / J.kdh, d = c - part * J.kdh;
      k = part * (J.kheads * J.kdh) + head * J.kdh + d;
    }
    if (live) {
      if (k < J.K) {
        if (J.conv_w > 0) {
          const int tr = k / J.conv_f, f = k - tr * J.conv_f;
          x = J.src[((int64_t)f * J.conv_w + (J.conv_w - 1 - tr)) * J.N + row];
        } else {
          x = J.src[row * J.sn + k * J.sk];
        }
      }
      else if (k == J.K && J.bias != nullptr)
        x = J.bias[row];
    }
    v[e] = x;
  }
  uint32_t h[4], l[4];
#pragma unroll
  for (int q = 0; q < 4; ++q) split_pair(v[2 * q], v[2 * q + 1], h[q], l[q]);
  uint4* dst = reinterpret_cast<uint4*>(J.img) + ((int64_t)(kb * J.nblk + nb) * 2) * 64 + lane;
  dst[0] = make_uint4(h[0], h[1], h[2], h[3]);
  dst[64] = make_uint4(l[0], l[1], l[2], l[3]);
}

static inline void rp_jobs_init(RpImageJobs* js) { js->count = 0; js->overflow = 0; js->first_thread[0] = 0; }
static inline RpImageJob* rp_jobs_add(RpImageJobs* js, const float* src, int64_t sn, int64_t sk, int N, int K,
                                      const float* bias, uint16_t* img, int nblk) {
  if (js->count >= RP_MAX_JOBS) {
    js->overflow = 1;
    js->count = RP_MAX_JOBS - 1;
  }
  RpImageJob& J = js->job[js->count];
  J.src = src; J.bias = bias; J.img = img; J.sn = sn; J.sk = sk; J.N = N; J.K = K; J.nblk = nblk;
  J.kblocks = rp_kblocks(K, bias != nullptr); J.heads = 0; J.dh = 0; J.conv_f = 0; J.conv_w = 0; J.kheads = 0; J.kdh = 0; J.kperm_heads = 0;
  J.kappa = 0; J.kpad_d = 0; J.kpad_dp = 0;
  js->first_thread[js->count + 1] = js->first_thread[js->count] + (int64_t)J.kblocks * nblk * 64;
  js->count += 1;
  return &J;
}
static inline RpImageJob* rp_jobs_add_qkv_heads(RpImageJobs* js, const float* w_in, int D, const float* b_in,
                                                uint16_t* img, int heads, int dh) {
  RpImageJob* J = rp_jobs_add(js, w_in, D, 1, heads * 64, D, b_in, img, heads * 4);
  J->heads = heads;
  J->dh = dh;
  return J;
}
static inline RpImageJob* rp_jobs_add_kpad(RpImageJobs* js, const float* src, int64_t sn, int64_t sk, int N, int taps, int d,
                                           int dp, uint16_t* img, int nblk) {
  RpImageJob* J = rp_jobs_add(js, src, sn, sk, N, taps * d, nullptr, img, nblk);
  J->kpad_d = d;
  J->kpad_dp = dp;
  J->kblocks = rp_kblocks(taps * dp, false);
  js->first_thread[js->count] = js->first_thread[js->count - 1] + (int64_t)J->kblocks * nblk * 64;
  return J;
}
static inline RpImageJob* rp_jobs_add_kheads(RpImageJobs* js, const float* src, int64_t sn, int64_t sk, int N, int heads,
                                             int dh, uint16_t* img, int nblk) {
  RpImageJob* J = rp_jobs_add(js, src, sn, sk, N, 3 * heads * dh, nullptr, img, nblk);
  J->kheads = heads;
  J->kdh = dh;
  J->kblocks = heads * 2;
  js->first_thread[js->count] = js->first_thread[js->count - 1] + (int64_t)J->kblocks * nblk * 64;
  return J;
}
static inline RpImageJob* rp_jobs_add_kperm(RpImageJobs* js, const float* src, int64_t sn, int64_t sk, int N, int heads,
                                            uint16_t* img, int nblk, const float* bias = nullptr) {
  RpImageJob* J = rp_jobs_add(js, src, sn, sk, N, heads * 20, bias, img, nblk);
  J->kperm_heads = heads;
  J->kblocks = (16 * (heads + (heads + 3) / 4) + 31) / 32;
  js->first_thread[js->count] = js->first_thread[js->count - 1] + (int64_t)J->kblocks * nblk * 64;
  return J;
}
static inline RpImageJob* rp_jobs_add_kappa(RpImageJobs* js, const float* src, int64_t sn, int64_t sk, int N, int K,
                                            const float* bias, uint16_t* img, int nblk, int kblocks = 0) {
  RpImageJob* J = rp_jobs_add(js, src, sn, sk, N, K, bias, img, nblk);
  J->kappa = 1;
  if (kblocks > J->kblocks) {
    J->kblocks = kblocks;
    js->first_thread[js->count] = js->first_thread[js->count - 1] + (int64_t)J->kblocks * nblk * 64;
  }
  return J;
}
static inline int rp_jobs_launch(const RpImageJobs& js, hipStream_t st) {
  NRL_REQUIRE(js.overflow == 0, "row-panel image jobs: more than %d images in one launch", RP_MAX_JOBS);
  if (js.count == 0) return NRL_OK;
  const int64_t total = js.first_thread[js.count];
  hipLaunchKernelGGL(rp_weight_image_kernel, dim3((unsigned)((total + 255) / 256)), dim3(256), 0, st, js);
  NRL_LAUNCH_CHECK();
  return NRL_OK;
}

struct RpImage {
  const uint16_t* img = nullptr;
  int nblk = 0, kblocks = 0;
};

__device__ __forceinline__ void rp_split8(const float4& v0, const float4& v1, bf16x8& hi, bf16x8& lo) {
  uint32_t h[4], l[4];
  split_pair(v0.x, v0.y, h[0], l[0]);
  split_pair(v0.z, v0.w, h[1], l[1]);
  split_pair(v1.x, v1.y, h[2], l[2]);
  split_pair(v1.z, v1.w, h[3], l[3]);
  hi = __builtin_bit_cast(bf16x8, make_uint4(h[0], h[1], h[2], h[3]));
  lo = __builtin_bit_cast(bf16x8, make_uint4(l[0], l[1], l[2], l[3]));
}

struct EpiPoolBwdPlanes {
  EpiPoolBwd inner;
// ... 279 lines not shown
```

### newsreclib_amd/csrc/nrl_user_tail.h

```cpp
#pragma once
#include "nrl_common.h"

namespace nrl {

struct UserTailArgs {
  const float* o;
  const uint16_t* img_o;
  const uint16_t* img_a;
  int nblk_o, nblk_a;
  const float *b_o, *b_a, *q_a;
  int64_t groups;
  int H, D, Q;
  Dropout drop2;
  float *y, *t, *w, *out;
};

struct UserTailBwdArgs {
  const float* d_out;
  const float* y;
  float* t;
  const float* w;
  const float* q_a;
  const uint16_t* img_ad;
  const uint16_t* img_od;
  int nblk_ad, nblk_od;
  int64_t groups;
  int H, D, Q;
  Dropout drop2;
  float *dy, *d_o, *dq_a;
};

bool user_tail_bwd_ok(int64_t groups, int H, int D, int Q, int nblk_ad, int nblk_od, int kb_ad, int kb_od);
int user_tail_bwd(const UserTailBwdArgs& a, hipStream_t st);
bool user_tail_ok(int64_t groups, int H, int D, int Q, int nblk_o, int nblk_a);
int user_tail_fwd(const UserTailArgs& a, hipStream_t st);

}
```

### newsreclib_amd/csrc/nrl_user_tail.hip

```cpp
#include <math.h>

#include "nrl_kernels.h"
#include "nrl_news_fused.h"
#include "nrl_user_tail.h"

namespace nrl {

constexpr int UT_WAVES = 8, UT_RB = 4, UT_KB = 10, UT_FBK = 2 * UT_KB;
constexpr int UT_NCB_Y = 19, UT_NCB_T = 13;
constexpr int UT_PLANE = UT_RB * UT_FBK * 512;
constexpr int UT_CB1 = 3, UT_CB2 = 2;

#define UT_MFMA3(acc, ah, al, bh, bl)                                          \
  do {                                                                         \
    acc = __builtin_amdgcn_mfma_f32_16x16x32_bf16(ah, bl, acc, 0, 0, 0);       \
    acc = __builtin_amdgcn_mfma_f32_16x16x32_bf16(al, bh, acc, 0, 0, 0);       \
    acc = __builtin_amdgcn_mfma_f32_16x16x32_bf16(ah, bh, acc, 0, 0, 0);       \
  } while (0)

template <int FBK>
__device__ __forceinline__ void ut_arow(const unsigned char* __restrict__ planes, int rb, int kb, int l15, int g, bf16x8& hi,
                                        bf16x8& lo) {
  const int off = ((rb * FBK) + 2 * kb + (g >> 1)) * 512 + l15 * 32 + (g & 1) * 16;
  hi = *reinterpret_cast<const bf16x8*>(planes + off);
  lo = *reinterpret_cast<const bf16x8*>(planes + UT_RB * FBK * 512 + off);
}
__device__ __forceinline__ void ut_bfrag(const uint16_t* __restrict__ img, int nblk, int kb, int cb, int lane, bf16x8& hi, bf16x8& lo) {
  const unsigned char* p = reinterpret_cast<const unsigned char*>(img) + ((size_t)(kb * nblk + cb) * 2) * 1024 + lane * 16;
  hi = *reinterpret_cast<const bf16x8*>(p);
  lo = *reinterpret_cast<const bf16x8*>(p + 1024);
}

__device__ __forceinline__ float ut_row_sum(float v) {
  v += __shfl_xor(v, 1, 64);
  v += __shfl_xor(v, 2, 64);
  v += __shfl_xor(v, 4, 64);
  v += __shfl_xor(v, 8, 64);
  return v;
}

template <int NC, int KB = UT_KB, int FBK = UT_FBK>
__device__ __forceinline__ void ut_gemm(const unsigned char* __restrict__ planes, const uint16_t* __restrict__ img, int nblk,
                                        const int (&cbs)[NC], int ncb_valid, int l15, int g, int lane, f32x4 (&acc)[NC][UT_RB]) {
  bf16x8 bh[2][NC], bl[2][NC];
#pragma unroll
  for (int ci = 0; ci < NC; ++ci) ut_bfrag(img, nblk, 0, cbs[ci] < ncb_valid ? cbs[ci] : ncb_valid - 1, lane, bh[0][ci], bl[0][ci]);
#pragma unroll
  for (int kb = 0; kb < KB; ++kb) {
    const int cur = kb & 1, nxt = cur ^ 1;
    if (kb + 1 < KB) {
#pragma unroll
      for (int ci = 0; ci < NC; ++ci)
        ut_bfrag(img, nblk, kb + 1, cbs[ci] < ncb_valid ? cbs[ci] : ncb_valid - 1, lane, bh[nxt][ci], bl[nxt][ci]);
    }
    bf16x8 ah[UT_RB], al[UT_RB];
#pragma unroll
    for (int rb = 0; rb < UT_RB; ++rb) ut_arow<FBK>(planes, rb, kb, l15, g, ah[rb], al[rb]);
#pragma unroll
    for (int ci = 0; ci < NC; ++ci)
#pragma unroll
      for (int rb = 0; rb < UT_RB; ++rb) UT_MFMA3(acc[ci][rb], ah[rb], al[rb], bh[cur][ci], bl[cur][ci]);
  }
}

__global__ void __launch_bounds__(UT_WAVES * 64) ut_fwd_kernel(const UserTailArgs P) {
  __shared__ __attribute__((aligned(1024))) unsigned char planes[2 * UT_PLANE];
  __shared__ float a_part[UT_WAVES][64], w_s[64];
  const int tid = threadIdx.x, lane = tid & 63;
  const int wave = __builtin_amdgcn_readfirstlane(tid >> 6);
  const int l15 = lane & 15, g = lane >> 4;
  const int64_t grp = blockIdx.x;
  const int H = P.H, D = P.D, Q = P.Q;
  const int64_t row0 = grp * H;

#pragma unroll
  for (int i = 0; i < 5; ++i) {
    const int idx = tid + i * UT_WAVES * 64;
    const int row = idx / 40, c8 = idx - row * 40;
    const int r = row < H ? row : H - 1;
    const float* rp = P.o + (row0 + r) * D + 8 * c8;
    float4 v0 = make_float4(0.f, 0.f, 0.f, 0.f), v1 = v0;
    if (8 * c8 < D) v0 = *reinterpret_cast<const float4*>(rp);
    if (8 * c8 + 4 < D) v1 = *reinterpret_cast<const float4*>(rp + 4);
    bf16x8 hi, lo;
    rp_split8(v0, v1, hi, lo);
    const int off = ((row >> 4) * UT_FBK + (c8 >> 1)) * 512 + (row & 15) * 32 + (c8 & 1) * 16;
    *reinterpret_cast<bf16x8*>(planes + off) = hi;
    *reinterpret_cast<bf16x8*>(planes + UT_PLANE + off) = lo;
  }
  __syncthreads();

  const int cb1[UT_CB1] = {wave, wave + 8, wave + 16};
  f32x4 y[UT_CB1][UT_RB];
#pragma unroll
  for (int ci = 0; ci < UT_CB1; ++ci)
#pragma unroll
    for (int rb = 0; rb < UT_RB; ++rb) y[ci][rb] = f32x4{0.f, 0.f, 0.f, 0.f};
  ut_gemm<UT_CB1>(planes, P.img_o, P.nblk_o, cb1, UT_NCB_Y, l15, g, lane, y);
  __syncthreads();
#pragma unroll
  for (int ci = 0; ci < UT_CB1; ++ci) {
    const int cb = cb1[ci];
    if (cb >= UT_NCB_Y) continue;
    const int col = 16 * cb + l15;
    const bool col_ok = col < D;
    const float bias = col_ok ? P.b_o[col] : 0.f;
#pragma unroll
    for (int rb = 0; rb < UT_RB; ++rb) {
      uint16_t* ph = reinterpret_cast<uint16_t*>(planes + (rb * UT_FBK + cb) * 512) + l15;
      uint16_t* pl = reinterpret_cast<uint16_t*>(planes + UT_PLANE + (rb * UT_FBK + cb) * 512) + l15;
#pragma unroll
      for (int r = 0; r < 4; ++r) {
        const int row = 16 * rb + 4 * g + r;
        const int64_t m = row0 + (row < H ? row : H - 1);
        float v = col_ok ? y[ci][rb][r] + bias : 0.f;
        if (P.drop2.thresh != 0u) v *= P.drop2.mult((uint32_t)m * (uint32_t)D + (uint32_t)col);
        y[ci][rb][r] = v;
        if (row < H && col_ok) P.y[m * D + col] = v;
        uint32_t h, l;
        split_pair(v, 0.f, h, l);
        ph[(4 * g + r) * 16] = (uint16_t)(h & 0xFFFFu);
        pl[(4 * g + r) * 16] = (uint16_t)(l & 0xFFFFu);
      }
    }
  }
  __syncthreads();

  const int cb2[UT_CB2] = {wave, wave + 8};
  const int ncb_t = (Q + 15) / 16;
  f32x4 pre[UT_CB2][UT_RB];
#pragma unroll
  for (int ci = 0; ci < UT_CB2; ++ci)
#pragma unroll
    for (int rb = 0; rb < UT_RB; ++rb) pre[ci][rb] = f32x4{0.f, 0.f, 0.f, 0.f};
  ut_gemm<UT_CB2>(planes, P.img_a, P.nblk_a, cb2, ncb_t, l15, g, lane, pre);
  float apart[UT_RB][4];
#pragma unroll
  for (int rb = 0; rb < UT_RB; ++rb)
#pragma unroll
    for (int r = 0; r < 4; ++r) apart[rb][r] = 0.f;
#pragma unroll
  for (int ci = 0; ci < UT_CB2; ++ci) {
    const int cb = cb2[ci];
    if (cb >= ncb_t) continue;
    const int col = 16 * cb + l15;
    const bool col_ok = col < Q;
    const float bias = col_ok ? P.b_a[col] : 0.f, qa = col_ok ? P.q_a[col] : 0.f;
#pragma unroll
    for (int rb = 0; rb < UT_RB; ++rb)
#pragma unroll
      for (int r = 0; r < 4; ++r) {
        const int row = 16 * rb + 4 * g + r;
        const float tv = tanhf(pre[ci][rb][r] + bias);
        if (row < H && col_ok) P.t[(row0 + row) * Q + col] = tv;
        apart[rb][r] = fmaf(tv, qa, apart[rb][r]);
      }
  }
#pragma unroll
  for (int rb = 0; rb < UT_RB; ++rb)
#pragma unroll
    for (int r = 0; r < 4; ++r) {
      const float v = ut_row_sum(apart[rb][r]);
      if (l15 == 0) a_part[wave][16 * rb + 4 * g + r] = v;
    }
  __syncthreads();

  if (wave == 0) {
    float a = 0.f;
#pragma unroll
    for (int wv = 0; wv < UT_WAVES; ++wv) a += a_part[wv][lane];
    if (lane >= H) a = -INFINITY;
    const float mx = wave_max(a);
    const float e = lane < H ? expf(a - mx) : 0.f;
    const float inv = 1.0f / wave_sum(e);
    const float wl = e * inv;
    w_s[lane] = wl;
    if (lane < H) P.w[row0 + lane] = wl;
  }
  __syncthreads();

  float wr[UT_RB][4];
#pragma unroll
  for (int rb = 0; rb < UT_RB; ++rb) {
    const float4 w4 = *reinterpret_cast<const float4*>(w_s + 16 * rb + 4 * g);
    wr[rb][0] = w4.x; wr[rb][1] = w4.y; wr[rb][2] = w4.z; wr[rb][3] = w4.w;
  }
#pragma unroll
  for (int ci = 0; ci < UT_CB1; ++ci) {
    const int cb = cb1[ci];
    if (cb >= UT_NCB_Y) continue;
    float s = 0.f;
#pragma unroll
    for (int rb = 0; rb < UT_RB; ++rb)
#pragma unroll
      for (int r = 0; r < 4; ++r) s = fmaf(wr[rb][r], y[ci][rb][r], s);
    s += nf_xor16(s, lane);
    s += nf_xor32(s, lane);
    const int col = 16 * cb + l15;
    if (g == 0 && col < D) P.out[grp * D + col] = s;
  }
}

bool user_tail_ok(int64_t groups, int H, int D, int Q, int nblk_o, int nblk_a) {
  static const bool on = [] {
    const char* e = getenv("NRL_USER_TAIL");
    return !(e != nullptr && e[0] == '0');
  }();
  return on && groups > 0 && groups < (1LL << 31) && H >= 1 && H <= 64 && D == 300 && Q % 4 == 0 && Q >= 16 && Q <= 16 * UT_NCB_T &&
         nblk_o >= UT_NCB_Y && nblk_a >= (Q + 15) / 16;
}

int user_tail_fwd(const UserTailArgs& a, hipStream_t st) {
  NRL_REQUIRE(user_tail_ok(a.groups, a.H, a.D, a.Q, a.nblk_o, a.nblk_a), "fused user tail: unsupported geometry");
  NRL_REQUIRE((((uintptr_t)a.o) & 15) == 0, "fused user tail: 16-byte alignment");
  hipLaunchKernelGGL(ut_fwd_kernel, dim3((unsigned)a.groups), dim3(UT_WAVES * 64), 0, st, a);
  NRL_LAUNCH_CHECK();
  return NRL_OK;
}

constexpr int UT_KBQ = 7, UT_FBQ = 2 * UT_KBQ;
constexpr int UT_PLANE_Q = UT_RB * UT_FBQ * 512;

__global__ void __launch_bounds__(UT_WAVES * 64) ut_bwd_kernel(const UserTailBwdArgs P) {
  __shared__ __attribute__((aligned(1024))) unsigned char pq[2 * UT_PLANE_Q];
  __shared__ __attribute__((aligned(1024))) unsigned char py[2 * UT_PLANE];
  __shared__ __attribute__((aligned(16))) float d_s[320];
  __shared__ __attribute__((aligned(16))) float c_s[64], w_s[64];
  const int tid = threadIdx.x, lane = tid & 63;
  const int wave = __builtin_amdgcn_readfirstlane(tid >> 6);
  const int l15 = lane & 15, g = lane >> 4;
  const int64_t grp = blockIdx.x;
  const int H = P.H, D = P.D, Q = P.Q;
  const int64_t row0 = grp * H;
  const int D4 = D >> 2;

  if (tid < 320) d_s[tid] = tid < D ? P.d_out[grp * D + tid] : 0.f;
  {
    const uint4 z = make_uint4(0u, 0u, 0u, 0u);
#pragma unroll
    for (int i = 0; i < 2 * UT_PLANE_Q / (UT_WAVES * 64 * 16); ++i) reinterpret_cast<uint4*>(pq)[tid + i * UT_WAVES * 64] = z;
    if (tid < 256) {
      const int pl = tid >> 7, rb = (tid >> 5) & 3, q16 = tid & 31;
      reinterpret_cast<uint4*>(py + pl * UT_PLANE + (rb * UT_FBK + 19) * 512)[q16] = z;
    }
  }
  __syncthreads();
  {
    const int gi = tid >> 4, li = tid & 15;
    const float4* d4 = reinterpret_cast<const float4*>(d_s);
    for (int l = gi; l < H; l += UT_WAVES * 4) {
      const float4* yr = reinterpret_cast<const float4*>(P.y + (row0 + l) * D);
      float acc = 0.f;
      for (int d = li; d < D4; d += 16) {
        const float4 a = d4[d], b = yr[d];
        acc = fmaf(a.x, b.x, acc); acc = fmaf(a.y, b.y, acc); acc = fmaf(a.z, b.z, acc); acc = fmaf(a.w, b.w, acc);
      }
      acc = ut_row_sum(acc);
      if (li == 0) c_s[l] = acc;
    }
  }
  __syncthreads();
  if (wave == 0) {
    const float wl = lane < H ? P.w[row0 + lane] : 0.f;
    const float c = lane < H ? c_s[lane] : 0.f;
    const float dbar = wave_sum(wl * c);
    c_s[lane] = wl * (c - dbar);
    w_s[lane] = wl;
  }
  __syncthreads();
  if (tid < Q) {
    const int q = tid;
    const float qa = P.q_a[q];
    float sumq = 0.f;
    float* tcol = P.t + row0 * Q + q;
    uint16_t* ph = reinterpret_cast<uint16_t*>(pq + (q >> 4) * 512) + (q & 15);
    uint16_t* pl = reinterpret_cast<uint16_t*>(pq + UT_PLANE_Q + (q >> 4) * 512) + (q & 15);
    for (int l0 = 0; l0 < H; l0 += 8) {
      float tv[8];
#pragma unroll
      for (int u = 0; u < 8; ++u) tv[u] = l0 + u < H ? tcol[(int64_t)(l0 + u) * Q] : 0.f;
#pragma unroll
      for (int u = 0; u < 8; ++u) {
        const int l = l0 + u;
        if (l < H) {
// ... 12 lines not shown
    atomicAdd(P.dq_a + q, sumq);
  }
  __syncthreads();

  const int cb1[UT_CB1] = {wave, wave + 8, wave + 16};
  {
    f32x4 acc[UT_CB1][UT_RB];
#pragma unroll
    for (int ci = 0; ci < UT_CB1; ++ci)
#pragma unroll
      for (int rb = 0; rb < UT_RB; ++rb) acc[ci][rb] = f32x4{0.f, 0.f, 0.f, 0.f};
    ut_gemm<UT_CB1, UT_KBQ, UT_FBQ>(pq, P.img_ad, P.nblk_ad, cb1, UT_NCB_Y, l15, g, lane, acc);
#pragma unroll
    for (int ci = 0; ci < UT_CB1; ++ci) {
      const int cb = cb1[ci];
      if (cb >= UT_NCB_Y) continue;
      const int col = 16 * cb + l15;
      const bool col_ok = col < D;
      const float dv = d_s[col];
#pragma unroll
      for (int rb = 0; rb < UT_RB; ++rb) {
        uint16_t* ph = reinterpret_cast<uint16_t*>(py + (rb * UT_FBK + cb) * 512) + l15;
        uint16_t* pl = reinterpret_cast<uint16_t*>(py + UT_PLANE + (rb * UT_FBK + cb) * 512) + l15;
        const float4 w4 = *reinterpret_cast<const float4*>(w_s + 16 * rb + 4 * g);
        const float wr[4] = {w4.x, w4.y, w4.z, w4.w};
#pragma unroll
        for (int r = 0; r < 4; ++r) {
          const int row = 16 * rb + 4 * g + r;
          const int64_t m = row0 + (row < H ? row : H - 1);
          float v = col_ok && row < H ? fmaf(wr[r], dv, acc[ci][rb][r]) : 0.f;
          if (P.drop2.thresh != 0u) v *= P.drop2.mult((uint32_t)m * (uint32_t)D + (uint32_t)col);
          if (row < H && col_ok) P.dy[m * D + col] = v;
          uint32_t h, lo;
          split_pair(v, 0.f, h, lo);
          ph[(4 * g + r) * 16] = (uint16_t)(h & 0xFFFFu);
          pl[(4 * g + r) * 16] = (uint16_t)(lo & 0xFFFFu);
        }
      }
    }
  }
  __syncthreads();

  {
    f32x4 acc[UT_CB1][UT_RB];
#pragma unroll
    for (int ci = 0; ci < UT_CB1; ++ci)
#pragma unroll
      for (int rb = 0; rb < UT_RB; ++rb) acc[ci][rb] = f32x4{0.f, 0.f, 0.f, 0.f};
    ut_gemm<UT_CB1, UT_KB, UT_FBK>(py, P.img_od, P.nblk_od, cb1, UT_NCB_Y, l15, g, lane, acc);
#pragma unroll
    for (int ci = 0; ci < UT_CB1; ++ci) {
      const int cb = cb1[ci];
      if (cb >= UT_NCB_Y) continue;
      const int col = 16 * cb + l15;
      if (col >= D) continue;
#pragma unroll
      for (int rb = 0; rb < UT_RB; ++rb)
#pragma unroll
        for (int r = 0; r < 4; ++r) {
          const int row = 16 * rb + 4 * g + r;
          if (row < H) P.d_o[(row0 + row) * D + col] = acc[ci][rb][r];
        }
    }
  }
}

bool user_tail_bwd_ok(int64_t groups, int H, int D, int Q, int nblk_ad, int nblk_od, int kb_ad, int kb_od) {
  static const int mode = [] {
    const char* e = getenv("NRL_USER_TAIL_BWD");
    return e == nullptr ? -1 : (e[0] == '1' ? 1 : 0);
  }();
  const bool on = mode < 0 ? groups <= 64 : mode == 1;
  return on && user_tail_ok(groups, H, D, Q, nblk_od, 16 * UT_NCB_T) && nblk_ad >= UT_NCB_Y && kb_ad == UT_KBQ && kb_od == UT_KB && Q <= 224;
}

int user_tail_bwd(const UserTailBwdArgs& a, hipStream_t st) {
  NRL_REQUIRE(a.groups > 0 && a.H >= 1 && a.H <= 64 && a.D == 300, "fused user tail backward: unsupported geometry");
  NRL_REQUIRE((((uintptr_t)a.y | (uintptr_t)a.d_out) & 15) == 0, "fused user tail backward: 16-byte alignment");
  hipLaunchKernelGGL(ut_bwd_kernel, dim3((unsigned)a.groups), dim3(UT_WAVES * 64), 0, st, a);
  NRL_LAUNCH_CHECK();
  return NRL_OK;
}

}
```

### newsreclib_amd/dot_product_recommender.py

```python
from __future__ import annotations

from typing import Dict, Optional

import torch

from . import ops
from .abstract_recommender import AbstractRecommender
from .batch_layout import prepare_batch, text_vocab
from .dense_batch import dense_rows
from .news_encoder import _draw_seed


class DotProductRecommender(AbstractRecommender):
    dot_product_scorer = True
    dense_max_is_exact = False

    def _prepare(self, batch: Dict) -> Dict:
        return prepare_batch(batch, text_vocab(self))

    def _encode_user(self, hist_dense: torch.Tensor, batch: Dict, seed: Optional[int]) -> torch.Tensor:
        raise NotImplementedError

    def _encode_and_score(self, batch: Dict, seed: Optional[int]):
        batch = self._prepare(batch)
        if self.training and seed is None:
            seed = _draw_seed()
        hist_vec, cand_vec = self._encode_news(batch, seed)
        return self.score_news_vectors(hist_vec, cand_vec, batch, seed=seed), hist_vec, cand_vec

    def forward(self, batch: Dict, seed: Optional[int] = None) -> torch.Tensor:
        return self._encode_and_score(batch, seed)[0]

    def score_news_vectors(self, hist_news_vector: torch.Tensor, cand_news_vector: torch.Tensor, batch: Dict,
                           seed: Optional[int] = None) -> torch.Tensor:
        user_vector = self.user_vectors(hist_news_vector, batch, seed=seed)
        cand_news_vector_agg = dense_rows(cand_news_vector, batch["batch_cand"], batch["batch_size"], batch["max_cand"],
                                          batch["cand_offsets"], max_is_exact=self.dense_max_is_exact)
        return self.click_predictor(user_vector.unsqueeze(dim=1), cand_news_vector_agg.permute(0, 2, 1))

    def user_vectors(self, hist_news_vector: torch.Tensor, batch: Dict, seed: Optional[int] = None) -> torch.Tensor:
        hist_news_vector_agg = dense_rows(hist_news_vector, batch["batch_hist"], batch["batch_size"], batch["max_hist"],
                                          batch["hist_offsets"], max_is_exact=self.dense_max_is_exact)
        if not self.hparams.late_fusion:
            return self._encode_user(hist_news_vector_agg, batch, seed)
        return ops.HistMeanFn.apply(hist_news_vector_agg, batch["hist_offsets"])
```

### newsreclib_amd/nrms_module.py

```python
from __future__ import annotations

from typing import Any, Dict, List, Optional

import torch

from . import ops
from .batch_layout import attach_layout, prepare_batch, text_vocab
from .click_predictor import DotProduct
from .dot_product_recommender import DotProductRecommender
from .news_encoder import PLM, MHSAAddAtt, NewsEncoder
from .user_encoder import UserEncoder


class NRMSModule(DotProductRecommender):
    dense_max_is_exact = True

    def __init__(
        self,
        dataset_attributes: List[str],
        attributes2encode: List[str],
        outputs: Dict[str, List[str]],
        dual_loss_training: bool,
        dual_loss_coef: Optional[float],
        loss: str,
        late_fusion: bool,
        temperature: Optional[float],
        use_plm: bool,
        pretrained_embeddings_path: Optional[str],
        plm_model: Optional[str],
        frozen_layers: Optional[List[int]],
        embed_dim: int,
        num_heads: int,
        query_dim: int,
        dropout_probability: float,
        top_k_list: List[int],
        num_categ_classes: int,
        num_sent_classes: int,
        save_recs: bool,
        recs_fpath: Optional[str],
        optimizer: Any,
        scheduler: Any,
        pretrained_embeddings: Optional[torch.Tensor] = None,
    ) -> None:
        super().__init__()
        self.save_hyperparameters(logger=False, ignore=["pretrained_embeddings"])
        hp = self.hparams
        self.num_categ_classes = num_categ_classes + 1
        self.num_sent_classes = num_sent_classes + 1
        if save_recs:
            assert isinstance(recs_fpath, str)
        self._init_loss(loss, dual_loss_training, dual_loss_coef)

        if not use_plm:
            if pretrained_embeddings is None:
                assert isinstance(pretrained_embeddings_path, str)
                pretrained_embeddings = self._init_embedding(pretrained_embeddings_path)
            text_encoder = MHSAAddAtt(pretrained_embeddings=pretrained_embeddings, embed_dim=embed_dim,
                                      num_heads=num_heads, query_dim=query_dim,
                                      dropout_probability=dropout_probability)
        else:
            assert isinstance(plm_model, str)
            text_encoder = PLM(plm_model=plm_model, frozen_layers=frozen_layers, embed_dim=embed_dim,
                               use_mhsa=True, apply_reduce_dim=False, reduced_embed_dim=None,
                               num_heads=num_heads, query_dim=query_dim, dropout_probability=dropout_probability)
        self.news_encoder = NewsEncoder(
            dataset_attributes=dataset_attributes, attributes2encode=attributes2encode,
            concatenate_inputs=False, text_encoder=text_encoder, category_encoder=None,
            entity_encoder=None, combine_vectors=False, combine_type=None, input_dim=None,
            query_dim=None, output_dim=None)
        if not late_fusion:
            self.user_encoder = UserEncoder(news_embed_dim=embed_dim, num_heads=num_heads, query_dim=query_dim)
        self.click_predictor = DotProduct()
        self._text_attr = next(iter(self.news_encoder.text_encoders.keys()))

        self._init_step_outputs(outputs)
        assert hp is not None

    def _prepare(self, batch: Dict) -> Dict:
        te = self.news_encoder.text_encoders[self._text_attr]
        emb = getattr(te, "embedding_layer", None)
        return prepare_batch(batch, emb.weight.shape[0] if emb is not None else None)

    def forward(self, batch: Dict) -> torch.Tensor:
        batch = self._prepare(batch)
        B = batch["batch_size"]
        hist_text = batch["x_hist"][self._text_attr]
        n_hist = (hist_text if torch.is_tensor(hist_text) else next(iter(hist_text.values()))).shape[0]
        if self.hparams.use_plm:
            self.news_encoder.share_plm_bodies(batch["x_hist"], batch["x_cand"])
            hist_vec = self.news_encoder(batch["x_hist"])
            cand_vec = self.news_encoder(batch["x_cand"])
            return self.score_news_vectors(hist_vec, cand_vec, batch)
        news_vector = self.news_encoder(batch["x_all"])
        return self.score_news_vectors(*ops.split_rows(news_vector, n_hist), batch)

    def _encode_user(self, hist_dense: torch.Tensor, batch: Dict, seed=None) -> torch.Tensor:
        return self.user_encoder(hist_dense)
```

### newsreclib_amd/ops.py

```python
from __future__ import annotations

import ctypes
import os
from typing import Optional, Sequence, Tuple

import torch

from . import _lib
from ._lib import NrlBlockGrads, NrlBlockParams


_RAW_STREAM = getattr(torch._C, "_cuda_getCurrentRawStream", None)
_GET_DEVICE = getattr(torch._C, "_cuda_getDevice", None)


def _stream() -> int:
    if _RAW_STREAM is not None and _GET_DEVICE is not None:
        return _RAW_STREAM(_GET_DEVICE())
    return torch.cuda.current_stream().cuda_stream


def workspace(nbytes: int, device) -> torch.Tensor:
    return torch.empty(max(int(nbytes), 256), dtype=torch.uint8, device=device)

# ... 142 lines not shown
        if hook is None:
            run(0)
        else:
            run(1)
            _call_table_grad_hook(hook, bufs[0], ids)
            run(2)
        ctx.ws = None
        return (None, *rets, None, None, None, None, None, None, None)


def _call_table_grad_hook(hook, grad: torch.Tensor, ids: torch.Tensor) -> None:
    import inspect
    try:
        params = [p for p in inspect.signature(hook).parameters.values()
                  if p.kind in (p.POSITIONAL_ONLY, p.POSITIONAL_OR_KEYWORD, p.VAR_POSITIONAL)]
        two = any(p.kind == p.VAR_POSITIONAL for p in params) or len(params) >= 2
    except (TypeError, ValueError):
        two = True
    if two:
        hook(grad, ids)
    else:
        hook(grad)


class UserEncoderFn(GradAwareFunction):

    @staticmethod
    def forward(ctx, hist, w_in, b_in, w_o, b_o, w_a, b_a, q_a, heads, grad_bufs, p_drop=0.0, seed=0,
                input_dropout=True, stream0=0):
        lib = _lib.load()
        hist = _chk(hist, torch.float32, "hist_news_vector")
        params = [_chk(t, torch.float32, "user encoder parameter") for t in (w_in, b_in, w_o, b_o, w_a, b_a, q_a)]
        if hist.dim() != 3:
            raise ValueError("newsreclib_amd: hist_news_vector must be (batch, history, dim)")
        B, H, D = hist.shape
        engine = _lib.engine_code()
        options = _lib.options_word()
        bp = _block_params(params, heads, engine, options)
        if bp.embed_dim != D:
            raise ValueError("newsreclib_amd: hist feature dim does not match the encoder")
        save = saving(ctx)
        ws_bytes = lib.nrl_user_encoder_workspace_bytes(B, H, D, heads, bp.query_dim)
        ws = workspace(ws_bytes, hist.device)
        out = torch.empty((B, D), dtype=torch.float32, device=hist.device)
        _lib.check(lib.nrl_user_encoder_fwd(ctypes.byref(bp), hist.data_ptr(), B, H, float(p_drop), int(seed),
                                            int(stream0), int(bool(input_dropout)), int(save), out.data_ptr(),
                                            ws.data_ptr(), ws.numel(), _stream()), "nrl_user_encoder_fwd")
        if save:
            ctx.save_for_backward(hist, *params)
            ctx.ws, ctx.heads, ctx.grad_bufs, ctx.engine = ws, heads, grad_bufs, engine
            ctx.options = options
            ctx.drop = (float(p_drop), int(seed), int(stream0), int(bool(input_dropout)))
        return out

    @staticmethod
    def backward(ctx, d_out):
        lib = _lib.load()
        hist, *params = ctx.saved_tensors
        B, H, D = hist.shape
        d_out = _chk(d_out, torch.float32, "d_out")
        bp = _block_params(params, ctx.heads, ctx.engine, ctx.options)
        bufs, rets = _grad_targets(params, ctx.grad_bufs)
        bg = _block_grads(bufs)
        d_hist = torch.empty_like(hist)
        ws = ctx.ws

        def run(phase):
            _lib.check(lib.nrl_user_encoder_bwd_phase(ctypes.byref(bp), ctypes.byref(bg), hist.data_ptr(), B, H,
                                                      ctx.drop[0], ctx.drop[1], ctx.drop[2], ctx.drop[3], d_out.data_ptr(),
                                                      d_hist.data_ptr(), phase, ws.data_ptr(), ws.numel(), _stream()),
                       "nrl_user_encoder_bwd_phase")

        defer = deferred_weight_grads._active
        if defer is None or any(r is not None for r in rets):
            run(0)
        else:
            run(1)
            defer.stream.wait_stream(torch.cuda.current_stream())
            with torch.cuda.stream(defer.stream):
                run(2)
            defer.keep.append((ws, hist, params, bufs))
        ctx.ws = None
        return (d_hist, *rets, None, None, None, None, None, None)


class ToDenseBatchFn(GradAwareFunction):

    @staticmethod
    def forward(ctx, x, offsets, batch_size, max_len):
        lib = _lib.load()
        x = _chk(x, torch.float32, "x")
        offsets = _chk(offsets, torch.int64, "offsets")
        N, D = x.shape
        dense = torch.empty((batch_size, max_len, D), dtype=torch.float32, device=x.device)
        _lib.check(lib.nrl_to_dense_batch_fwd(x.data_ptr(), offsets.data_ptr(), batch_size, max_len, D,
                                              dense.data_ptr(), _stream()), "nrl_to_dense_batch_fwd")
        ctx.save_for_backward(offsets)
        ctx.shape = (N, D, batch_size, max_len)
        return dense

    @staticmethod
    def backward(ctx, d_dense):
        lib = _lib.load()
        (offsets,) = ctx.saved_tensors
        N, D, B, max_len = ctx.shape
        d_dense = _chk(d_dense, torch.float32, "d_dense")
        d_x = torch.empty((N, D), dtype=torch.float32, device=d_dense.device)
        _lib.check(lib.nrl_to_dense_batch_bwd(d_dense.data_ptr(), offsets.data_ptr(), B, max_len, D, N,
                                              d_x.data_ptr(), _stream()), "nrl_to_dense_batch_bwd")
        return d_x, None, None, None


class HistMeanFn(GradAwareFunction):

    @staticmethod
    def forward(ctx, hist, offsets):
        lib = _lib.load()
        hist = _chk(hist, torch.float32, "hist_news_vector")
        offsets = _chk(offsets, torch.int64, "offsets")
        B, H, D = hist.shape
        user = torch.empty((B, D), dtype=torch.float32, device=hist.device)
        _lib.check(lib.nrl_hist_mean_fwd(hist.data_ptr(), offsets.data_ptr(), B, H, D, user.data_ptr(), _stream()),
                   "nrl_hist_mean_fwd")
        ctx.save_for_backward(offsets)
        ctx.shape = (B, H, D)
        return user

    @staticmethod
    def backward(ctx, d_user):
        lib = _lib.load()
        (offsets,) = ctx.saved_tensors
        B, H, D = ctx.shape
        d_user = _chk(d_user, torch.float32, "d_user")
        d_hist = torch.empty((B, H, D), dtype=torch.float32, device=d_user.device)
        _lib.check(lib.nrl_hist_mean_bwd(d_user.data_ptr(), offsets.data_ptr(), B, H, D, d_hist.data_ptr(), _stream()),
                   "nrl_hist_mean_bwd")
        return d_hist, None


class DotScoresFn(GradAwareFunction):

    @staticmethod
    def forward(ctx, user, cand):
        lib = _lib.load()
        user = _chk(user, torch.float32, "user_vec")
        cand = _chk(cand, torch.float32, "cand_news_vector")
        B, C, D = cand.shape
        scores = torch.empty((B, C), dtype=torch.float32, device=user.device)
        _lib.check(lib.nrl_dot_scores_fwd(user.data_ptr(), cand.data_ptr(), B, C, D, scores.data_ptr(),
                                          _stream()), "nrl_dot_scores_fwd")
        ctx.save_for_backward(user, cand)
        return scores

    @staticmethod
    def backward(ctx, d_scores):
        lib = _lib.load()
        user, cand = ctx.saved_tensors
        B, C, D = cand.shape
        d_scores = _chk(d_scores, torch.float32, "d_scores")
        d_user, d_cand = torch.empty_like(user), torch.empty_like(cand)
        _lib.check(lib.nrl_dot_scores_bwd(d_scores.data_ptr(), user.data_ptr(), cand.data_ptr(), B, C, D,
                                          d_user.data_ptr(), d_cand.data_ptr(), _stream()),
                   "nrl_dot_scores_bwd")
        return d_user, d_cand


# ... 446 lines not shown
```

### newsreclib_amd/sentirec_module.py

```python
from __future__ import annotations

from typing import Any, Dict, List, Optional

import torch
import torch.nn as nn

from . import ops, ops_blocks
from .dense_batch import dense_rows
from .nrms_module import NRMSModule, prepare_batch, text_vocab


class SentiRecModule(NRMSModule):
    def __init__(
        self,
        dataset_attributes: List[str],
        attributes2encode: List[str],
        outputs: Dict[str, List[str]],
        dual_loss_training: bool,
        dual_loss_coef: Optional[float],
        loss: str,
        late_fusion: bool,
        temperature: Optional[float],
        use_plm: bool,
        pretrained_embeddings_path: Optional[str],
        plm_model: Optional[str],
        frozen_layers: Optional[List[int]],
        embed_dim: int,
        num_heads: int,
        query_dim: int,
        dropout_probability: float,
        sent_pred_loss_coef: float,
        sent_div_loss_coef: float,
        top_k_list: List[int],
        num_categ_classes: int,
        num_sent_classes: int,
        save_recs: bool,
        recs_fpath: Optional[str],
        optimizer: Any,
        scheduler: Any,
        pretrained_embeddings: Optional[torch.Tensor] = None,
    ) -> None:
        super().__init__(
            dataset_attributes=dataset_attributes, attributes2encode=attributes2encode, outputs=outputs,
            dual_loss_training=dual_loss_training, dual_loss_coef=dual_loss_coef, loss=loss, late_fusion=late_fusion,
            temperature=temperature, use_plm=use_plm, pretrained_embeddings_path=pretrained_embeddings_path,
            plm_model=plm_model, frozen_layers=frozen_layers, embed_dim=embed_dim, num_heads=num_heads,
            query_dim=query_dim, dropout_probability=dropout_probability, top_k_list=top_k_list,
            num_categ_classes=num_categ_classes, num_sent_classes=num_sent_classes, save_recs=save_recs,
            recs_fpath=recs_fpath, optimizer=optimizer, scheduler=scheduler, pretrained_embeddings=pretrained_embeddings)
        self.sent_pred_loss = nn.L1Loss()
        self.sent_predictor = nn.Linear(in_features=embed_dim, out_features=self.num_sent_classes)

    def forward(self, batch: Dict):
        batch = prepare_batch(batch, text_vocab(self))
        if self.hparams.use_plm:
            hist_vec = self.news_encoder(batch["x_hist"])
            cand_vec = self.news_encoder(batch["x_cand"])
        else:
            n_hist = batch["batch_hist"].shape[0]
            news_vector = self.news_encoder(batch["x_all"])
            hist_vec, cand_vec = ops.split_rows(news_vector, n_hist)
        scores = self.score_news_vectors(hist_vec, cand_vec, batch)
        w, b = self.sent_predictor.weight, self.sent_predictor.bias
        n_cls = w.shape[0]
        pad = (-n_cls) % 4
        wp = torch.cat([w, w.new_zeros(pad, w.shape[1])]) if pad else w
        bp = torch.cat([b, b.new_zeros(pad)]) if pad else b
        rows = torch.cat((cand_vec, hist_vec), dim=0)
        sent_scores = ops_blocks.LinearActFn.apply(rows.contiguous(), wp, bp, "none", None)[:, :n_cls]
        return scores, (sent_scores, scores)

    def _aux_loss(self, batch: Dict, aux) -> torch.Tensor:
        _, scores = aux
        B = batch["batch_size"]
        sent_labels = torch.cat((batch["x_cand"]["sentiment_score"], batch["x_hist"]["sentiment_score"]))
        loss = self.hparams.sent_pred_loss_coef * self.sent_pred_loss(sent_labels.flatten(), sent_labels)
        sent_hist = dense_rows(batch["x_hist"]["sentiment_score"], batch["batch_hist"], B, batch["max_hist"],
                                      batch["hist_offsets"])
        sent_cand = dense_rows(batch["x_cand"]["sentiment_score"], batch["batch_cand"], B, batch["max_cand"],
                                      batch["cand_offsets"], batch["cand_flat_idx"])
        user_mean_sent_score = sent_hist.sum(dim=1) / batch["hist_sizes"].to(sent_hist.dtype)
        sent_div_loss = torch.relu(user_mean_sent_score.unsqueeze(dim=-1) * sent_cand * scores).mean()
        return loss + self.hparams.sent_div_loss_coef * sent_div_loss
```

Measured before the change: 48590 impressions/s.

## Fuse NRMS user-encoder tail with dot scores and CE loss

Adds a fused user-encoder-plus-loss path for NRMS training. The forward runs the attention front, then one tail kernel that does out-projection, additive pooling, candidate dot scores, cross-entropy loss and the early backward pieces (d_cand, per-row query grads). A matching backward-phase entry resumes from the saved attention gradients. The goal is to cut kernel launches and global-memory round trips between the user encoder, the scoring op and the loss. It only applies under the bf16x3 engine with row-panel weight images and up to 64 candidates; an environment flag allows it to be switched off, and other cases fall back to the old path.

```diff
diff --git a/include/newsreclib_amd.h b/include/newsreclib_amd.h
--- a/include/newsreclib_amd.h
+++ b/include/newsreclib_amd.h
@@ -96,6 +96,18 @@
                                int64_t batch, int64_t hist_len, double p_drop, uint64_t seed,
                                uint32_t stream0, int32_t input_dropout, const float* d_out,
                                float* d_hist, int32_t phase, void* ws, size_t ws_bytes, void* stream);
+
+int nrl_user_encoder_loss_supported(int64_t batch, int64_t hist_len, int32_t embed_dim, int32_t num_heads,
+                                    int32_t query_dim, int64_t n_cand, int32_t engine);
+int nrl_user_encoder_loss_fwd(const NrlBlockParams* p, const float* hist, int64_t batch, int64_t hist_len,
+                              const float* cand, int64_t n_cand, const float* y_true, float grad_scale,
+                              double p_drop, uint64_t seed, uint32_t stream0, float* user_out, float* scores,
+                              float* loss, float* d_cand, float* loss_terms, float* dqa_rows, uint32_t* ticket,
+                              void* ws, size_t ws_bytes, void* stream);
+int nrl_user_encoder_loss_bwd_phase(const NrlBlockParams* p, const NrlBlockGrads* g, const float* hist,
+                                    int64_t batch, int64_t hist_len, double p_drop, uint64_t seed,
+                                    uint32_t stream0, float* d_hist, const float* dqa_rows, int32_t phase,
+                                    void* ws, size_t ws_bytes, void* stream);
 
 int nrl_to_dense_batch_fwd(const float* x, const int64_t* offsets, int64_t batch, int64_t max_len,
                            int32_t dim, float* dense, void* stream);
diff --git a/newsreclib_amd/_lib.py b/newsreclib_amd/_lib.py
--- a/newsreclib_amd/_lib.py
+++ b/newsreclib_amd/_lib.py
@@ -146,6 +146,13 @@
     "nrl_user_encoder_bwd_phase": (c_int32, [POINTER(NrlBlockParams), POINTER(NrlBlockGrads), c_void_p, c_int64,
                                              c_int64, c_double, c_uint64, c_uint32, c_int32, c_void_p, c_void_p, c_int32,
                                              c_void_p, c_size_t, c_void_p]),
+    "nrl_user_encoder_loss_supported": (c_int32, [c_int64, c_int64, c_int32, c_int32, c_int32, c_int64, c_int32]),
+    "nrl_user_encoder_loss_fwd": (c_int32, [POINTER(NrlBlockParams), c_void_p, c_int64, c_int64, c_void_p, c_int64, c_void_p,
+                                            c_float, c_double, c_uint64, c_uint32, c_void_p, c_void_p, c_void_p, c_void_p,
+                                            c_void_p, c_void_p, c_void_p, c_void_p, c_size_t, c_void_p]),
+    "nrl_user_encoder_loss_bwd_phase": (c_int32, [POINTER(NrlBlockParams), POINTER(NrlBlockGrads), c_void_p, c_int64, c_int64,
+                                                  c_double, c_uint64, c_uint32, c_void_p, c_void_p, c_int32, c_void_p,
+                                                  c_size_t, c_void_p]),
     "nrl_to_dense_batch_fwd": (c_int32, [c_void_p, c_void_p, c_int64, c_int64, c_int32, c_void_p, c_void_p]),
     "nrl_to_dense_batch_bwd": (c_int32, [c_void_p, c_void_p, c_int64, c_int64, c_int32, c_int64, c_void_p,
                                          c_void_p]),
diff --git a/newsreclib_amd/abstract_recommender.py b/newsreclib_amd/abstract_recommender.py
--- a/newsreclib_amd/abstract_recommender.py
+++ b/newsreclib_amd/abstract_recommender.py
@@ -90,7 +90,9 @@
         loss = self._loss(scores, y_true.float(), batch)
         if aux is not None:
             loss = loss + self._aux_loss(batch, aux)
-
+        return self._step_outputs(loss, scores, batch)
+
+    def _step_outputs(self, loss: torch.Tensor, scores: torch.Tensor, batch: Dict) -> Tuple:
         if batch["labels"].shape[0] == scores.numel():
             preds = scores.detach().reshape(-1)
         else:
diff --git a/newsreclib_amd/csrc/nrl_api.hip b/newsreclib_amd/csrc/nrl_api.hip
--- a/newsreclib_amd/csrc/nrl_api.hip
+++ b/newsreclib_amd/csrc/nrl_api.hip
@@ -418,6 +418,36 @@
   return NRL_OK;
 }
 
+static int user_bwd_finish(const NrlBlockParams* p, const NrlBlockGrads* g, const float* x_rows, const BlockShape& s,
+                           const BlockWs& w, const BlockPlanes& bp, Dropout d1, float* d_hist, int32_t phase, hipStream_t st) {
+  if (phase == 1)
+    return gemm_dgrad(w.dqkv, p->in_proj_weight, bp.in, EpiLinear{d_hist, s.D, nullptr, 0, d1, s.D}, s.M, 3 * s.D, s.D, st,
+                      bp.rp.on ? &bp.rp.in_d : nullptr);
+  if (!opt(O_USER_FORK) || s.M > 65536) {
+    NRL_TRY(gemm_dgrad(w.dqkv, p->in_proj_weight, bp.in, EpiLinear{d_hist, s.D, nullptr, 0, d1, s.D}, s.M, 3 * s.D,
+                       s.D, st, bp.rp.on ? &bp.rp.in_d : nullptr));
+    return block_bwd_phase2(g, x_rows, s, w, st);
+  }
+  ForkSet* fs = nullptr;
+  NRL_TRY(fork_set(&fs));
+  NRL_HIP(hipEventRecord(fs->fork, st));
+  for (int i = 0; i < 2; ++i) NRL_HIP(hipStreamWaitEvent(fs->s[i], fs->fork, 0));
+  const size_t third = opt(O_WGRAD_2STEP) ? qkv_elems(s.M, s.D, s.heads, s.pad_rows) / 3 / 64 * 64 : 0;
+  float* const sc = third > 0 ? w.qkv : nullptr;
+  int rc = gemm_dgrad(w.dqkv, p->in_proj_weight, bp.in, EpiLinear{d_hist, s.D, nullptr, 0, d1, s.D}, s.M, 3 * s.D, s.D, st,
+                      bp.rp.on ? &bp.rp.in_d : nullptr);
+  if (rc == NRL_OK) rc = gemm_wgrad(w.dqkv, 3 * s.D, x_rows, s.D, g->in_proj_weight, g->in_proj_bias, s.M, fs->s[0], sc, third);
+  if (rc == NRL_OK)
+    rc = gemm_wgrad(w.dy, s.D, w.o, s.D, g->out_proj_weight, g->out_proj_bias, s.M, fs->s[1], sc ? sc + third : nullptr, third);
+  if (rc == NRL_OK)
+    rc = gemm_wgrad(w.t, s.Q, w.y, s.D, g->att_weight, g->att_bias, s.M, fs->s[1], sc ? sc + 2 * third : nullptr, third);
+  for (int i = 0; i < 2; ++i) {
+    NRL_HIP(hipEventRecord(fs->join[i], fs->s[i]));
+    NRL_HIP(hipStreamWaitEvent(st, fs->join[i], 0));
+  }
+  return rc;
+}
+
 size_t nrl_user_encoder_workspace_bytes(int64_t batch, int64_t hist_len, int32_t embed_dim,
                                         int32_t num_heads, int32_t query_dim) {
   return block_ws_bytes(batch * hist_len, embed_dim, query_dim, num_heads, true);
@@ -474,32 +504,86 @@
   BlockPlanes bp;
   NRL_TRY(block_planes(p, s, w, false, &bp, st));
   NRL_TRY(block_bwd_phase1(p, g, s, w, bp, d2, d_out, st));
-  if (phase == 1)
-    return gemm_dgrad(w.dqkv, p->in_proj_weight, bp.in, EpiLinear{d_hist, s.D, nullptr, 0, d1, s.D}, s.M, 3 * s.D, s.D, st,
-                      bp.rp.on ? &bp.rp.in_d : nullptr);
-  if (!opt(O_USER_FORK) || s.M > 65536) {
-    NRL_TRY(gemm_dgrad(w.dqkv, p->in_proj_weight, bp.in, EpiLinear{d_hist, s.D, nullptr, 0, d1, s.D}, s.M, 3 * s.D,
-                       s.D, st, bp.rp.on ? &bp.rp.in_d : nullptr));
-    return block_bwd_phase2(g, x_rows, s, w, st);
-  }
-  ForkSet* fs = nullptr;
-  NRL_TRY(fork_set(&fs));
-  NRL_HIP(hipEventRecord(fs->fork, st));
-  for (int i = 0; i < 2; ++i) NRL_HIP(hipStreamWaitEvent(fs->s[i], fs->fork, 0));
-  const size_t third = opt(O_WGRAD_2STEP) ? qkv_elems(s.M, s.D, s.heads, s.pad_rows) / 3 / 64 * 64 : 0;
-  float* const sc = third > 0 ? w.qkv : nullptr;
-  int rc = gemm_dgrad(w.dqkv, p->in_proj_weight, bp.in, EpiLinear{d_hist, s.D, nullptr, 0, d1, s.D}, s.M, 3 * s.D, s.D, st,
-                      bp.rp.on ? &bp.rp.in_d : nullptr);
-  if (rc == NRL_OK) rc = gemm_wgrad(w.dqkv, 3 * s.D, x_rows, s.D, g->in_proj_weight, g->in_proj_bias, s.M, fs->s[0], sc, third);
-  if (rc == NRL_OK)
-    rc = gemm_wgrad(w.dy, s.D, w.o, s.D, g->out_proj_weight, g->out_proj_bias, s.M, fs->s[1], sc ? sc + third : nullptr, third);
-  if (rc == NRL_OK)
-    rc = gemm_wgrad(w.t, s.Q, w.y, s.D, g->att_weight, g->att_bias, s.M, fs->s[1], sc ? sc + 2 * third : nullptr, third);
-  for (int i = 0; i < 2; ++i) {
-    NRL_HIP(hipEventRecord(fs->join[i], fs->s[i]));
-    NRL_HIP(hipStreamWaitEvent(st, fs->join[i], 0));
-  }
-  return rc;
+  return user_bwd_finish(p, g, x_rows, s, w, bp, d1, d_hist, phase, st);
+}
+
+static bool user_loss_shape_ok(const BlockShape& s, int64_t n_cand) {
+  if (cur_engine() != ENGINE_BF16X3 || !block_rp_ok(s.D, s.Q) || n_cand < 1 || n_cand > 64) return false;
+  const int nd = rp_nblk_for(s.D), nq = rp_nblk_for(s.Q);
+  return user_tail_loss_ok(s.pool_groups, s.pool_len, s.D, s.Q, (int)n_cand, nd, nq, nd, nd, rp_kblocks(s.Q, false), rp_kblocks(s.D, false));
+}
+
+int nrl_user_encoder_loss_supported(int64_t batch, int64_t hist_len, int32_t embed_dim, int32_t num_heads, int32_t query_dim,
+                                    int64_t n_cand, int32_t engine) {
+  if (batch <= 0 || hist_len <= 0 || hist_len > 64 || embed_dim <= 0 || num_heads <= 0 || query_dim <= 0 || !engine_field_ok(engine) ||
+      embed_dim % num_heads != 0 || !attn_head_dim_supported(embed_dim / num_heads))
+    return 0;
+  const EngineScope engine_scope(engine);
+  const OptScope opt_scope(0);
+  NrlBlockParams p{};
+  p.embed_dim = embed_dim; p.num_heads = num_heads; p.query_dim = query_dim;
+  return user_loss_shape_ok(user_shape(&p, batch, hist_len), n_cand) ? 1 : 0;
+}
+
+int nrl_user_encoder_loss_fwd(const NrlBlockParams* p, const float* hist, int64_t batch, int64_t hist_len, const float* cand,
+                              int64_t n_cand, const float* y_true, float grad_scale, double p_drop, uint64_t seed,
+                              uint32_t stream0, float* user_out, float* scores, float* loss, float* d_cand, float* loss_terms,
+                              float* dqa_rows, uint32_t* ticket, void* ws, size_t ws_bytes, void* stream) {
+  NRL_TRY(check_params(p));
+  const EngineScope engine_scope(p->gemm_engine);
+  const OptScope opt_scope(p->options);
+  NRL_REQUIRE(hist && cand && y_true && user_out && scores && loss && d_cand && loss_terms && dqa_rows && ticket && batch > 0 &&
+                  hist_len > 0 && n_cand > 0, "user_encoder_loss_fwd: bad arguments");
+  NRL_REQUIRE(((uintptr_t)hist & 15) == 0, "hist must be 16-byte aligned");
+  NRL_REQUIRE(p_drop >= 0.0 && p_drop < 1.0, "dropout probability must be in [0, 1)");
+  const BlockShape s = user_shape(p, batch, hist_len);
+  NRL_REQUIRE(user_loss_shape_ok(s, n_cand), "user_encoder_loss_fwd: unsupported geometry or engine (nrl_user_encoder_loss_supported)");
+  NRL_REQUIRE(p_drop == 0.0 || s.M * s.D < (1LL << 32), "activation too large for the 32-bit dropout index space");
+  BlockWs w;
+  NRL_TRY(carve_ws(ws, ws_bytes, s, true, &w));
+  hipStream_t st = (hipStream_t)stream;
+  BlockPlanes bp;
+  NRL_TRY(block_fwd_front(p, KCPlain{hist, s.D, s.M}, s, w, true, false, &bp, st, ticket));
+  NRL_REQUIRE(bp.rp.on, "user_encoder_loss_fwd: row-panel weight images are off");
+  UserTailLossArgs a;
+  a.f.o = w.o; a.f.img_o = bp.rp.out_f.img; a.f.img_a = bp.rp.att_f.img; a.f.nblk_o = bp.rp.out_f.nblk; a.f.nblk_a = bp.rp.att_f.nblk;
+  a.f.b_o = p->out_proj_bias; a.f.b_a = p->att_bias; a.f.q_a = p->att_query; a.f.groups = s.pool_groups; a.f.H = s.pool_len;
+  a.f.D = s.D; a.f.Q = s.Q; a.f.drop2 = make_dropout(p_drop, seed, stream0 + 1); a.f.y = w.y; a.f.t = w.t; a.f.w = w.w;
+  a.f.out = user_out;
+  a.cand = cand; a.y_true = y_true; a.C = (int)n_cand; a.grad_scale = grad_scale; a.img_ad = bp.rp.att_d.img;
+  a.img_od = bp.rp.out_d.img; a.nblk_ad = bp.rp.att_d.nblk; a.nblk_od = bp.rp.out_d.nblk; a.kb_ad = bp.rp.att_d.kblocks;
+  a.scores = scores; a.loss = loss; a.d_cand = d_cand; a.loss_terms = loss_terms; a.dqa_rows = dqa_rows; a.ticket = ticket;
+  a.dy = w.dy; a.d_o = w.d_o;
+  return user_tail_loss(a, st);
+}
+
+int nrl_user_encoder_loss_bwd_phase(const NrlBlockParams* p, const NrlBlockGrads* g, const float* hist, int64_t batch,
+                                    int64_t hist_len, double p_drop, uint64_t seed, uint32_t stream0, float* d_hist,
+                                    const float* dqa_rows, int32_t phase, void* ws, size_t ws_bytes, void* stream) {
+  NRL_TRY(check_params(p));
+  const EngineScope engine_scope(p->gemm_engine);
+  const OptScope opt_scope(p->options);
+  NRL_TRY(check_grads(g));
+  NRL_REQUIRE(phase >= 0 && phase <= 2, "user_encoder_loss_bwd: phase must be 0 (both), 1 or 2");
+  NRL_REQUIRE(hist && batch > 0 && hist_len > 0 && (phase == 2 || d_hist) && (phase == 1 || dqa_rows),
+              "user_encoder_loss_bwd: bad arguments");
+  NRL_REQUIRE(p_drop >= 0.0 && p_drop < 1.0, "dropout probability must be in [0, 1)");
+  hipStream_t st = (hipStream_t)stream;
+  const BlockShape s = user_shape(p, batch, hist_len);
+  BlockWs w;
+  NRL_TRY(carve_ws(ws, ws_bytes, s, true, &w));
+  if (phase != 2) {
+    const Dropout d1 = make_dropout(0.0, seed, stream0);
+    BlockPlanes bp;
+    NRL_TRY(block_planes(p, s, w, false, &bp, st));
+    if (block_attn_x3(s)) NRL_TRY(attn_bwd_x3(w.qkv, w.o, w.d_o, w.lse, w.dqkv, s.geom, st));
+    else NRL_TRY(attn_bwd(w.qkv, w.o, w.d_o, w.lse, w.dqkv, s.geom, st));
+    NRL_TRY(user_bwd_finish(p, g, hist, s, w, bp, d1, d_hist, phase, st));
+  } else {
+    NRL_TRY(block_bwd_phase2(g, hist, s, w, st));
+  }
+  if (phase != 1) NRL_TRY(user_tail_dqa_reduce(dqa_rows, s.pool_groups, s.Q, g->att_query, st));
+  return NRL_OK;
 }
 
 int nrl_to_dense_batch_fwd(const float* x, const int64_t* offsets, int64_t batch, int64_t max_len,
diff --git a/newsreclib_amd/csrc/nrl_api_internal.h b/newsreclib_amd/csrc/nrl_api_internal.h
--- a/newsreclib_amd/csrc/nrl_api_internal.h
+++ b/newsreclib_amd/csrc/nrl_api_internal.h
@@ -218,7 +218,7 @@
 };
 
 static int block_planes(const NrlBlockParams* P, const BlockShape& s, const BlockWs& w, bool fill,
-                        BlockPlanes* bp, hipStream_t st, int fused_heads = 0, int proj_heads = 0) {
+                        BlockPlanes* bp, hipStream_t st, int fused_heads = 0, int proj_heads = 0, unsigned int* clear_word = nullptr) {
   const int D = s.D, Q = s.Q;
   uint16_t* p = w.planes;
   const float* ws[3] = {P->in_proj_weight, P->out_proj_weight, P->att_weight};
@@ -239,6 +239,7 @@
     uint16_t* q = w.rp;
     RpImageJobs jobs;
     rp_jobs_init(&jobs);
+    jobs.clear_word = clear_word;
     auto add = [&](RpImage* im, const float* src, int64_t sn, int64_t sk, int N, int K, int nblk) {
       im->img = q; im->nblk = nblk; im->kblocks = rp_kblocks(K, false);
       if (fill) rp_jobs_add(&jobs, src, sn, sk, N, K, nullptr, q, nblk);
@@ -447,31 +448,36 @@
 }
 
 template <class AOp>
-static int block_fwd(const NrlBlockParams* P, const AOp& a_in, const BlockShape& s, const BlockWs& w,
-                     Dropout drop2, bool save, bool prof_in_proj, float* out, hipStream_t st) {
+static int block_fwd_front(const NrlBlockParams* P, const AOp& a_in, const BlockShape& s, const BlockWs& w, bool save,
+                           bool prof_in_proj, BlockPlanes* bp_out, hipStream_t st, unsigned int* clear_word = nullptr) {
   const int D = s.D;
   const Dropout nodrop = make_dropout(0.0, 0, 0);
-  BlockPlanes bp;
+  BlockPlanes& bp = *bp_out;
   bool proj = false;
   if constexpr (std::is_same<AOp, KCPlain>::value) {
     proj = opt(O_USER_PROJ) && cur_engine() == ENGINE_BF16X3 && block_rp_ok(D, s.Q) && block_attn_x3(s) && a_in.ld == D &&
            D == s.heads * 20 && attn_x3_proj_ok(s.geom, s.heads * 4, NF_KB) && s.geom.q_outer % 3 == 0 && s.geom.q_seq % 3 == 0;
   }
-  NRL_TRY(block_planes(P, s, w, cur_engine() == ENGINE_BF16X3, &bp, st, 0, proj ? s.heads : 0));
+  NRL_TRY(block_planes(P, s, w, cur_engine() == ENGINE_BF16X3, &bp, st, 0, proj ? s.heads : 0, clear_word));
   if constexpr (std::is_same<AOp, KCPlain>::value) {
-    if (proj) {
-      NRL_TRY(attn_fwd_x3_proj(a_in.p, s.geom.q_outer / 3, s.geom.q_seq / 3, bp.rp.in_heads.img, bp.rp.in_heads.nblk,
-                               save ? w.qkv : nullptr, w.o, save ? w.lse : nullptr, s.geom, st));
-      return block_fwd_tail(P, s, w, bp, drop2, out, st);
-    }
+    if (proj)
+      return attn_fwd_x3_proj(a_in.p, s.geom.q_outer / 3, s.geom.q_seq / 3, bp.rp.in_heads.img, bp.rp.in_heads.nblk,
+                              save ? w.qkv : nullptr, w.o, save ? w.lse : nullptr, s.geom, st);
   }
   {
     ProfScope prof(st, prof_in_proj ? 2.0 * (double)s.M * 3.0 * D * D : 0.0);
     NRL_TRY(gemm_fwd(a_in, P->in_proj_weight, bp.in, EpiLinear{w.qkv, 3 * D, P->in_proj_bias, 0, nodrop, 3 * D},
                      s.M, 3 * D, D, false, st));
   }
-  if (block_attn_x3(s)) NRL_TRY(attn_fwd_x3(w.qkv, w.o, save ? w.lse : nullptr, s.geom, st));
-  else NRL_TRY(attn_fwd(w.qkv, w.o, save ? w.lse : nullptr, s.geom, st));
+  if (block_attn_x3(s)) return attn_fwd_x3(w.qkv, w.o, save ? w.lse : nullptr, s.geom, st);
+  return attn_fwd(w.qkv, w.o, save ? w.lse : nullptr, s.geom, st);
+}
+
+template <class AOp>
+static int block_fwd(const NrlBlockParams* P, const AOp& a_in, const BlockShape& s, const BlockWs& w,
+                     Dropout drop2, bool save, bool prof_in_proj, float* out, hipStream_t st) {
+  BlockPlanes bp;
+  NRL_TRY(block_fwd_front(P, a_in, s, w, save, prof_in_proj, &bp, st));
   return block_fwd_tail(P, s, w, bp, drop2, out, st);
 }
 
diff --git a/newsreclib_amd/csrc/nrl_ce_row.h b/newsreclib_amd/csrc/nrl_ce_row.h
--- /dev/null
+++ b/newsreclib_amd/csrc/nrl_ce_row.h
@@ -0,0 +1,24 @@
+#pragma once
+#include <math.h>
+#include <stdint.h>
+
+#include <hip/hip_runtime.h>
+
+namespace nrl {
+
+__device__ __forceinline__ float ce_row(const float* s, const float* yy, int64_t C, float inv_b, float grad_scale, float* d_row) {
+  float mx = -INFINITY;
+  for (int64_t c = 0; c < C; ++c) mx = fmaxf(mx, s[c]);
+  float sum = 0.f, ysum = 0.f;
+  for (int64_t c = 0; c < C; ++c) { sum += expf(s[c] - mx); ysum += yy[c]; }
+  const float lse = mx + logf(sum);
+  float lb = 0.f;
+  for (int64_t c = 0; c < C; ++c) {
+    const float logp = s[c] - lse;
+    lb -= yy[c] * logp;
+    if (d_row != nullptr) d_row[c] = (expf(logp) * ysum - yy[c]) * inv_b * grad_scale;
+  }
+  return lb;
+}
+
+}
diff --git a/newsreclib_amd/csrc/nrl_kernels.hip b/newsreclib_amd/csrc/nrl_kernels.hip
--- a/newsreclib_amd/csrc/nrl_kernels.hip
+++ b/newsreclib_amd/csrc/nrl_kernels.hip
@@ -1,6 +1,7 @@
 #include <math.h>
 #include <stdlib.h>
 
+#include "nrl_ce_row.h"
 #include "nrl_kernels.h"
 #include <cfloat>
 
@@ -765,22 +766,8 @@
   const int tid = threadIdx.x;
   float local = 0.f;
   const float invB = 1.0f / (float)B;
-  for (int64_t b = tid; b < B; b += 256) {
-    const float* s = scores + b * C;
-    const float* yy = y + b * C;
-    float mx = -INFINITY;
-    for (int64_t c = 0; c < C; ++c) mx = fmaxf(mx, s[c]);
-    float sum = 0.f, ysum = 0.f;
-    for (int64_t c = 0; c < C; ++c) { sum += expf(s[c] - mx); ysum += yy[c]; }
-    const float lse = mx + logf(sum);
-    float lb = 0.f;
-    for (int64_t c = 0; c < C; ++c) {
-      const float logp = s[c] - lse;
-      lb -= yy[c] * logp;
-      if (d_scores != nullptr) d_scores[b * C + c] = (expf(logp) * ysum - yy[c]) * invB * grad_scale;
-    }
-    local += lb;
-  }
+  for (int64_t b = tid; b < B; b += 256)
+    local += ce_row(scores + b * C, y + b * C, C, invB, grad_scale, d_scores != nullptr ? d_scores + b * C : nullptr);
   local = wave_sum(local);
   if ((tid & 63) == 0) red[tid >> 6] = local;
   __syncthreads();
diff --git a/newsreclib_amd/csrc/nrl_rowpanel.h b/newsreclib_amd/csrc/nrl_rowpanel.h
--- a/newsreclib_amd/csrc/nrl_rowpanel.h
+++ b/newsreclib_amd/csrc/nrl_rowpanel.h
@@ -22,6 +22,7 @@
   int count;
   int overflow;
   int64_t first_thread[RP_MAX_JOBS + 1];
+  unsigned int* clear_word;
 };
 
 static inline int rp_kblocks(int K, bool bias) { return (K + (bias ? 1 : 0) + 31) / 32; }
@@ -37,6 +38,7 @@
 
 static __global__ void __launch_bounds__(256) rp_weight_image_kernel(const RpImageJobs jobs) {
   const int64_t tid = (int64_t)blockIdx.x * 256 + threadIdx.x;
+  if (tid == 0 && jobs.clear_word != nullptr) *jobs.clear_word = 0u;
   if (tid >= jobs.first_thread[jobs.count]) return;
   int j = 0;
 #pragma unroll
@@ -99,7 +101,7 @@
   dst[64] = make_uint4(l[0], l[1], l[2], l[3]);
 }
 
-static inline void rp_jobs_init(RpImageJobs* js) { js->count = 0; js->overflow = 0; js->first_thread[0] = 0; }
+static inline void rp_jobs_init(RpImageJobs* js) { js->count = 0; js->overflow = 0; js->first_thread[0] = 0; js->clear_word = nullptr; }
 static inline RpImageJob* rp_jobs_add(RpImageJobs* js, const float* src, int64_t sn, int64_t sk, int N, int K,
                                       const float* bias, uint16_t* img, int nblk) {
   if (js->count >= RP_MAX_JOBS) {
diff --git a/newsreclib_amd/csrc/nrl_user_tail.h b/newsreclib_amd/csrc/nrl_user_tail.h
--- a/newsreclib_amd/csrc/nrl_user_tail.h
+++ b/newsreclib_amd/csrc/nrl_user_tail.h
@@ -30,6 +30,27 @@
   float *dy, *d_o, *dq_a;
 };
 
+struct UserTailLossArgs {
+  UserTailArgs f;
+  const float* cand;
+  const float* y_true;
+  int C;
+  float grad_scale;
+  const uint16_t* img_ad;
+  const uint16_t* img_od;
+  int nblk_ad, nblk_od, kb_ad;
+  float *scores, *loss;
+  float* d_cand;
+  float* loss_terms;
+  float* dqa_rows;
+  unsigned int* ticket;
+  float *dy, *d_o;
+};
+
+bool user_tail_loss_ok(int64_t groups, int H, int D, int Q, int C, int nblk_o, int nblk_a, int nblk_ad, int nblk_od, int kb_ad,
+                       int kb_od);
+int user_tail_loss(const UserTailLossArgs& a, hipStream_t st);
+int user_tail_dqa_reduce(const float* dqa_rows, int64_t groups, int Q, float* grad_q, hipStream_t st);
 bool user_tail_bwd_ok(int64_t groups, int H, int D, int Q, int nblk_ad, int nblk_od, int kb_ad, int kb_od);
 int user_tail_bwd(const UserTailBwdArgs& a, hipStream_t st);
 bool user_tail_ok(int64_t groups, int H, int D, int Q, int nblk_o, int nblk_a);
diff --git a/newsreclib_amd/csrc/nrl_user_tail.hip b/newsreclib_amd/csrc/nrl_user_tail.hip
--- a/newsreclib_amd/csrc/nrl_user_tail.hip
+++ b/newsreclib_amd/csrc/nrl_user_tail.hip
@@ -1,5 +1,6 @@
 #include <math.h>
 
+#include "nrl_ce_row.h"
 #include "nrl_kernels.h"
 #include "nrl_news_fused.h"
 #include "nrl_user_tail.h"
@@ -41,18 +42,20 @@
 
 template <int NC, int KB = UT_KB, int FBK = UT_FBK>
 __device__ __forceinline__ void ut_gemm(const unsigned char* __restrict__ planes, const uint16_t* __restrict__ img, int nblk,
-                                        const int (&cbs)[NC], int ncb_valid, int l15, int g, int lane, f32x4 (&acc)[NC][UT_RB]) {
+                                        const int (&cbs)[NC], int ncb_valid, int l15, int g, int lane, f32x4 (&acc)[NC][UT_RB],
+                                        int kb_valid = KB) {
   bf16x8 bh[2][NC], bl[2][NC];
 #pragma unroll
   for (int ci = 0; ci < NC; ++ci) ut_bfrag(img, nblk, 0, cbs[ci] < ncb_valid ? cbs[ci] : ncb_valid - 1, lane, bh[0][ci], bl[0][ci]);
 #pragma unroll
   for (int kb = 0; kb < KB; ++kb) {
     const int cur = kb & 1, nxt = cur ^ 1;
-    if (kb + 1 < KB) {
+    if (kb + 1 < KB && kb + 1 < kb_valid) {
 #pragma unroll
       for (int ci = 0; ci < NC; ++ci)
         ut_bfrag(img, nblk, kb + 1, cbs[ci] < ncb_valid ? cbs[ci] : ncb_valid - 1, lane, bh[nxt][ci], bl[nxt][ci]);
     }
+    if (kb >= kb_valid) continue;
     bf16x8 ah[UT_RB], al[UT_RB];
 #pragma unroll
     for (int rb = 0; rb < UT_RB; ++rb) ut_arow<FBK>(planes, rb, kb, l15, g, ah[rb], al[rb]);
@@ -63,13 +66,10 @@
   }
 }
 
-__global__ void __launch_bounds__(UT_WAVES * 64) ut_fwd_kernel(const UserTailArgs P) {
-  __shared__ __attribute__((aligned(1024))) unsigned char planes[2 * UT_PLANE];
-  __shared__ float a_part[UT_WAVES][64], w_s[64];
-  const int tid = threadIdx.x, lane = tid & 63;
-  const int wave = __builtin_amdgcn_readfirstlane(tid >> 6);
-  const int l15 = lane & 15, g = lane >> 4;
-  const int64_t grp = blockIdx.x;
+template <bool KEEP_T>
+__device__ __forceinline__ void ut_fwd_body(const UserTailArgs& P, unsigned char* planes, float (*a_part)[64], float* w_s, int tid,
+                                            int lane, int wave, int l15, int g, int64_t grp, f32x4 (&y)[UT_CB1][UT_RB],
+                                            f32x4 (&pre)[UT_CB2][UT_RB], float (&outv)[UT_CB1]) {
   const int H = P.H, D = P.D, Q = P.Q;
   const int64_t row0 = grp * H;
 
@@ -91,7 +91,6 @@
   __syncthreads();
 
   const int cb1[UT_CB1] = {wave, wave + 8, wave + 16};
-  f32x4 y[UT_CB1][UT_RB];
 #pragma unroll
   for (int ci = 0; ci < UT_CB1; ++ci)
 #pragma unroll
@@ -128,7 +127,6 @@
 
   const int cb2[UT_CB2] = {wave, wave + 8};
   const int ncb_t = (Q + 15) / 16;
-  f32x4 pre[UT_CB2][UT_RB];
 #pragma unroll
   for (int ci = 0; ci < UT_CB2; ++ci)
 #pragma unroll
@@ -152,7 +150,8 @@
       for (int r = 0; r < 4; ++r) {
         const int row = 16 * rb + 4 * g + r;
         const float tv = tanhf(pre[ci][rb][r] + bias);
-        if (row < H && col_ok) P.t[(row0 + row) * Q + col] = tv;
+        if (!KEEP_T && row < H && col_ok) P.t[(row0 + row) * Q + col] = tv;
+        pre[ci][rb][r] = tv;
         apart[rb][r] = fmaf(tv, qa, apart[rb][r]);
       }
   }
@@ -188,6 +187,7 @@
 #pragma unroll
   for (int ci = 0; ci < UT_CB1; ++ci) {
     const int cb = cb1[ci];
+    outv[ci] = 0.f;
     if (cb >= UT_NCB_Y) continue;
     float s = 0.f;
 #pragma unroll
@@ -196,10 +196,27 @@
       for (int r = 0; r < 4; ++r) s = fmaf(wr[rb][r], y[ci][rb][r], s);
     s += nf_xor16(s, lane);
     s += nf_xor32(s, lane);
-    const int col = 16 * cb + l15;
-    if (g == 0 && col < D) P.out[grp * D + col] = s;
-  }
-}
+    outv[ci] = s;
+  }
+}
+
+__global__ void __launch_bounds__(UT_WAVES * 64) ut_fwd_kernel(const UserTailArgs P) {
+  __shared__ __attribute__((aligned(1024))) unsigned char planes[2 * UT_PLANE];
+  __shared__ float a_part[UT_WAVES][64], w_s[64];
+  const int tid = threadIdx.x, lane = tid & 63;
+  const int wave = __builtin_amdgcn_readfirstlane(tid >> 6);
+  const int l15 = lane & 15, g = lane >> 4;
+  const int64_t grp = blockIdx.x;
+  f32x4 y[UT_CB1][UT_RB], pre[UT_CB2][UT_RB];
+  float outv[UT_CB1];
+  ut_fwd_body<false>(P, planes, a_part, w_s, tid, lane, wave, l15, g, grp, y, pre, outv);
+#pragma unroll
+  for (int ci = 0; ci < UT_CB1; ++ci) {
+    const int cb = wave + 8 * ci, col = 16 * cb + l15;
+    if (cb < UT_NCB_Y && g == 0 && col < P.D) P.out[grp * P.D + col] = outv[ci];
+  }
+}
+
 
 bool user_tail_ok(int64_t groups, int H, int D, int Q, int nblk_o, int nblk_a) {
   static const bool on = [] {
@@ -378,4 +395,263 @@
   return NRL_OK;
 }
 
-}
+__global__ void __launch_bounds__(UT_WAVES * 64) ut_loss_kernel(const UserTailLossArgs P) {
+  __shared__ __attribute__((aligned(1024))) unsigned char planes[2 * UT_PLANE];
+  __shared__ __attribute__((aligned(1024))) unsigned char pq[2 * UT_PLANE_Q];
+  __shared__ float a_part[UT_WAVES][64];
+  __shared__ __attribute__((aligned(16))) float w_s[64], da_s[64], out_s[320], d_s[320];
+  __shared__ float sc_s[64], ds_s[64], red[4];
+  __shared__ int last_s;
+  const int tid = threadIdx.x, lane = tid & 63;
+  const int wave = __builtin_amdgcn_readfirstlane(tid >> 6);
+  const int l15 = lane & 15, g = lane >> 4;
+  const int64_t grp = blockIdx.x;
+  const int H = P.f.H, D = P.f.D, Q = P.f.Q, C = P.C;
+  const int64_t row0 = grp * H;
+  const int cb1[UT_CB1] = {wave, wave + 8, wave + 16};
+  const int cb2[UT_CB2] = {wave, wave + 8};
+  const int ncb_t = (Q + 15) / 16;
+
+  f32x4 y[UT_CB1][UT_RB], tv[UT_CB2][UT_RB];
+  {
+    float outv[UT_CB1];
+    ut_fwd_body<true>(P.f, planes, a_part, w_s, tid, lane, wave, l15, g, grp, y, tv, outv);
+#pragma unroll
+    for (int ci = 0; ci < UT_CB1; ++ci) {
+      const int cb = cb1[ci], col = 16 * cb + l15;
+      if (cb < UT_NCB_Y && g == 0 && col < D) {
+        P.f.out[grp * D + col] = outv[ci];
+        out_s[col] = outv[ci];
+      }
+    }
+  }
+  __syncthreads();
+
+  for (int c = wave; c < C; c += UT_WAVES) {
+    const float* cv = P.cand + (grp * C + c) * D;
+    float part = 0.f;
+    for (int d = lane; d < D; d += 64) part = fmaf(out_s[d], cv[d], part);
+    part = wave_sum(part);
+    if (lane == 0) {
+      sc_s[c] = part;
+      P.scores[grp * C + c] = part;
+    }
+  }
+  __syncthreads();
+
+  const int ce_tid = (UT_WAVES - 1) * 64;
+  float lb = 0.f;
+  if (tid == ce_tid) lb = ce_row(sc_s, P.y_true + grp * C, C, 1.0f / (float)gridDim.x, P.grad_scale, ds_s);
+  __syncthreads();
+  bool last = false;
+  if (tid == ce_tid) {
+    __hip_atomic_store(P.loss_terms + grp, lb, __ATOMIC_RELAXED, __HIP_MEMORY_SCOPE_AGENT);
+    __builtin_amdgcn_fence(__ATOMIC_RELEASE, "agent");
+    asm volatile("s_waitcnt vmcnt(0)" ::: "memory");
+    last = __hip_atomic_fetch_add(P.ticket, 1u, __ATOMIC_RELAXED, __HIP_MEMORY_SCOPE_AGENT) == gridDim.x - 1;
+  }
+
+  if (tid < 320) {
+    float acc = 0.f;
+    if (tid < D) {
+      const float u = out_s[tid];
+      for (int c = 0; c < C; ++c) {
+        const float sv = ds_s[c];
+        const int64_t idx = (grp * C + c) * D + tid;
+        acc = fmaf(sv, P.cand[idx], acc);
+        P.d_cand[idx] = sv * u;
+      }
+    }
+    d_s[tid] = acc;
+  }
+  __syncthreads();
+
+  {
+    float dv[UT_CB1];
+#pragma unroll
+    for (int ci = 0; ci < UT_CB1; ++ci) dv[ci] = cb1[ci] < UT_NCB_Y ? d_s[16 * cb1[ci] + l15] : 0.f;
+#pragma unroll
+    for (int rb = 0; rb < UT_RB; ++rb)
+#pragma unroll
+      for (int r = 0; r < 4; ++r) {
+        float pc = 0.f;
+#pragma unroll
+        for (int ci = 0; ci < UT_CB1; ++ci)
+          if (cb1[ci] < UT_NCB_Y) pc = fmaf(dv[ci], y[ci][rb][r], pc);
+        pc = ut_row_sum(pc);
+        if (l15 == 0) a_part[wave][16 * rb + 4 * g + r] = pc;
+      }
+  }
+  __syncthreads();
+  if (wave == 0) {
+    float c = 0.f;
+#pragma unroll
+    for (int wv = 0; wv < UT_WAVES; ++wv) c += a_part[wv][lane];
+    const float wl = lane < H ? w_s[lane] : 0.f;
+    if (lane >= H) c = 0.f;
+    const float dbar = wave_sum(wl * c);
+    da_s[lane] = wl * (c - dbar);
+  }
+  __syncthreads();
+
+#pragma unroll
+  for (int ci = 0; ci < UT_CB2; ++ci) {
+    const int cb = cb2[ci];
+    if (cb >= UT_FBQ) continue;
+    const int col = 16 * cb + l15;
+    const bool col_ok = cb < ncb_t && col < Q;
+    const float qa = col_ok ? P.f.q_a[col] : 0.f;
+    float sumq = 0.f;
+#pragma unroll
+    for (int rb = 0; rb < UT_RB; ++rb) {
+      uint16_t* ph = reinterpret_cast<uint16_t*>(pq + (rb * UT_FBQ + cb) * 512) + l15;
+      uint16_t* pl = reinterpret_cast<uint16_t*>(pq + UT_PLANE_Q + (rb * UT_FBQ + cb) * 512) + l15;
+      const float4 d4 = *reinterpret_cast<const float4*>(da_s + 16 * rb + 4 * g);
+      const float dar[4] = {d4.x, d4.y, d4.z, d4.w};
+#pragma unroll
+      for (int r = 0; r < 4; ++r) {
+        const int row = 16 * rb + 4 * g + r;
+        float dp = 0.f;
+        if (col_ok && row < H) {
+          const float t = tv[ci][rb][r], da = dar[r];
+          sumq = fmaf(da, t, sumq);
+          dp = da * qa * (1.0f - t * t);
+          P.f.t[(row0 + row) * Q + col] = dp;
+        }
+        uint32_t h, lo;
+        split_pair(dp, 0.f, h, lo);
+        ph[(4 * g + r) * 16] = (uint16_t)(h & 0xFFFFu);
+        pl[(4 * g + r) * 16] = (uint16_t)(lo & 0xFFFFu);
+      }
+    }
+    sumq += nf_xor16(sumq, lane);
+    sumq += nf_xor32(sumq, lane);
+    if (g == 0 && col_ok) P.dqa_rows[grp * Q + col] = sumq;
+  }
+  if (tid == ce_tid) last_s = last ? 1 : 0;
+  __syncthreads();
+
+  {
+    f32x4 acc[UT_CB1][UT_RB];
+#pragma unroll
+    for (int ci = 0; ci < UT_CB1; ++ci)
+#pragma unroll
+      for (int rb = 0; rb < UT_RB; ++rb) acc[ci][rb] = f32x4{0.f, 0.f, 0.f, 0.f};
+    ut_gemm<UT_CB1, UT_KBQ, UT_FBQ>(pq, P.img_ad, P.nblk_ad, cb1, UT_NCB_Y, l15, g, lane, acc, P.kb_ad);
+#pragma unroll
+    for (int ci = 0; ci < UT_CB1; ++ci) {
+      const int cb = cb1[ci];
+      if (cb >= UT_NCB_Y) continue;
+      const int col = 16 * cb + l15;
+      const bool col_ok = col < D;
+      const float dv = d_s[col];
+#pragma unroll
+      for (int rb = 0; rb < UT_RB; ++rb) {
+        uint16_t* ph = reinterpret_cast<uint16_t*>(planes + (rb * UT_FBK + cb) * 512) + l15;
+        uint16_t* pl = reinterpret_cast<uint16_t*>(planes + UT_PLANE + (rb * UT_FBK + cb) * 512) + l15;
+        const float4 w4 = *reinterpret_cast<const float4*>(w_s + 16 * rb + 4 * g);
+        const float wr[4] = {w4.x, w4.y, w4.z, w4.w};
+#pragma unroll
+        for (int r = 0; r < 4; ++r) {
+          const int row = 16 * rb + 4 * g + r;
+          const int64_t m = row0 + (row < H ? row : H - 1);
+          float v = col_ok && row < H ? fmaf(wr[r], dv, acc[ci][rb][r]) : 0.f;
+          if (P.f.drop2.thresh != 0u) v *= P.f.drop2.mult((uint32_t)m * (uint32_t)D + (uint32_t)col);
+          if (row < H && col_ok) P.dy[m * D + col] = v;
+          uint32_t h, lo;
+          split_pair(v, 0.f, h, lo);
+          ph[(4 * g + r) * 16] = (uint16_t)(h & 0xFFFFu);
+          pl[(4 * g + r) * 16] = (uint16_t)(lo & 0xFFFFu);
+        }
+      }
+    }
+  }
+  __syncthreads();
+
+  {
+    f32x4 acc[UT_CB1][UT_RB];
+#pragma unroll
+    for (int ci = 0; ci < UT_CB1; ++ci)
+#pragma unroll
+      for (int rb = 0; rb < UT_RB; ++rb) acc[ci][rb] = f32x4{0.f, 0.f, 0.f, 0.f};
+    ut_gemm<UT_CB1, UT_KB, UT_FBK>(planes, P.img_od, P.nblk_od, cb1, UT_NCB_Y, l15, g, lane, acc);
+#pragma unroll
+    for (int ci = 0; ci < UT_CB1; ++ci) {
+      const int cb = cb1[ci];
+      if (cb >= UT_NCB_Y) continue;
+      const int col = 16 * cb + l15;
+      if (col >= D) continue;
+#pragma unroll
+      for (int rb = 0; rb < UT_RB; ++rb)
+#pragma unroll
+        for (int r = 0; r < 4; ++r) {
+          const int row = 16 * rb + 4 * g + r;
+          if (row < H) P.d_o[(row0 + row) * D + col] = acc[ci][rb][r];
+        }
+    }
+  }
+
+  if (last_s != 0) {
+    if (tid < 256) {
+      __builtin_amdgcn_fence(__ATOMIC_ACQUIRE, "agent");
+      float local = 0.f;
+      for (int64_t b = tid; b < (int64_t)gridDim.x; b += 256)
+        local += __hip_atomic_load(P.loss_terms + b, __ATOMIC_RELAXED, __HIP_MEMORY_SCOPE_AGENT);
+      local = wave_sum(local);
+      if (lane == 0) red[wave] = local;
+    }
+    __syncthreads();
+    if (tid == 0) *P.loss = (red[0] + red[1] + red[2] + red[3]) * (1.0f / (float)gridDim.x);
+  }
+}
+
+bool user_tail_loss_ok(int64_t groups, int H, int D, int Q, int C, int nblk_o, int nblk_a, int nblk_ad, int nblk_od, int kb_ad,
+                       int kb_od) {
+  return user_tail_ok(groups, H, D, Q, nblk_o, nblk_a) && C >= 1 && C <= 64 && nblk_ad >= UT_NCB_Y && nblk_od >= UT_NCB_Y &&
+         kb_ad == (Q + 31) / 32 && kb_ad <= UT_KBQ && kb_od == UT_KB;
+}
+
+int user_tail_loss(const UserTailLossArgs& a, hipStream_t st) {
+  NRL_REQUIRE(user_tail_loss_ok(a.f.groups, a.f.H, a.f.D, a.f.Q, a.C, a.f.nblk_o, a.f.nblk_a, a.nblk_ad, a.nblk_od, a.kb_ad, UT_KB),
+              "fused user tail + loss: unsupported geometry");
+  NRL_REQUIRE((((uintptr_t)a.f.o) & 15) == 0, "fused user tail + loss: 16-byte alignment");
+  hipLaunchKernelGGL(ut_loss_kernel, dim3((unsigned)a.f.groups), dim3(UT_WAVES * 64), 0, st, a);
+  NRL_LAUNCH_CHECK();
+  return NRL_OK;
+}
+
+__global__ void __launch_bounds__(256) ut_dqa_reduce_kernel(const float* __restrict__ rows, int64_t groups, int Q, float* __restrict__ grad_q) {
+  __shared__ float part[8][32];
+  const int ql = threadIdx.x & 31, pr = threadIdx.x >> 5;
+  const int q = blockIdx.x * 32 + ql;
+  const int64_t per = (groups + 7) / 8, b0 = pr * per, b1 = b0 + per < groups ? b0 + per : groups;
+  float acc = 0.f;
+  if (q < Q) {
+    int64_t b = b0;
+    for (; b + 8 <= b1; b += 8) {
+      float v[8];
+#pragma unroll
+      for (int u = 0; u < 8; ++u) v[u] = rows[(b + u) * Q + q];
+#pragma unroll
+      for (int u = 0; u < 8; ++u) acc += v[u];
+    }
+    for (; b < b1; ++b) acc += rows[b * Q + q];
+  }
+  part[pr][ql] = acc;
+  __syncthreads();
+  if (pr == 0 && q < Q) {
+    float t = part[0][ql];
+#pragma unroll
+    for (int i = 1; i < 8; ++i) t += part[i][ql];
+    grad_q[q] += t;
+  }
+}
+
+int user_tail_dqa_reduce(const float* dqa_rows, int64_t groups, int Q, float* grad_q, hipStream_t st) {
+  NRL_REQUIRE(dqa_rows && grad_q && groups > 0 && Q > 0, "dqa reduce: bad arguments");
+  hipLaunchKernelGGL(ut_dqa_reduce_kernel, dim3((unsigned)((Q + 31) / 32)), dim3(256), 0, st, dqa_rows, groups, Q, grad_q);
+  NRL_LAUNCH_CHECK();
+  return NRL_OK;
+}
+
+}
diff --git a/newsreclib_amd/dot_product_recommender.py b/newsreclib_amd/dot_product_recommender.py
--- a/newsreclib_amd/dot_product_recommender.py
+++ b/newsreclib_amd/dot_product_recommender.py
@@ -1,6 +1,6 @@
 from __future__ import annotations
 
-from typing import Dict, Optional
+from typing import Dict, Optional, Tuple
 
 import torch
 
@@ -15,8 +15,52 @@
     dot_product_scorer = True
     dense_max_is_exact = False
 
+    user_loss_fusable = False
+
     def _prepare(self, batch: Dict) -> Dict:
         return prepare_batch(batch, text_vocab(self))
+
+    def _news_vectors(self, batch: Dict):
+        raise NotImplementedError
+
+    def _fused_user_loss_args(self, batch: Dict):
+        from .user_encoder import UserEncoder
+        hp = self.hparams
+        if not (self.user_loss_fusable and self.training and torch.is_grad_enabled() and ops.user_loss_fused_enabled()):
+            return None
+        if hp.loss != "cross_entropy_loss" or hp.dual_loss_training or hp.late_fusion:
+            return None
+        ue = getattr(self, "user_encoder", None)
+        if type(ue) is not UserEncoder:
+            return None
+        mha, att = ue.multihead_attention, ue.additive_attention
+        params = (mha.in_proj_weight, mha.in_proj_bias, mha.out_proj.weight, mha.out_proj.bias,
+                  att.linear.weight, att.linear.bias, att.query)
+        D, Q = params[2].shape[0], params[4].shape[0]
+        if not params[0].is_cuda or not ops.user_loss_supported(batch["batch_size"], batch["max_hist"], D, ue.num_heads, Q,
+                                                                batch["max_cand"]):
+            return None
+        return params, ue.num_heads
+
+    def model_step(self, batch: Dict) -> Tuple:
+        if not self.user_loss_fusable:
+            return super().model_step(batch)
+        batch = self._prepare(batch)
+        fused = self._fused_user_loss_args(batch)
+        if fused is None:
+            return super().model_step(batch)
+        from .news_encoder import _grad_bufs
+        params, heads = fused
+        B = batch["batch_size"]
+        hist_vec, cand_vec = self._news_vectors(batch)
+        hist = dense_rows(hist_vec, batch["batch_hist"], B, batch["max_hist"], batch["hist_offsets"],
+                          max_is_exact=self.dense_max_is_exact)
+        cand = dense_rows(cand_vec, batch["batch_cand"], B, batch["max_cand"], batch["cand_offsets"],
+                          max_is_exact=self.dense_max_is_exact)
+        y_true = dense_rows(batch["labels"], batch["batch_cand"], B, batch["max_cand"], batch["cand_offsets"],
+                            batch["cand_flat_idx"], max_is_exact=True)
+        loss, scores, _user = ops.UserEncoderLossFn.apply(hist, cand, y_true.float(), *params, heads, _grad_bufs(params), 1.0)
+        return self._step_outputs(loss, scores, batch)
 
     def _encode_user(self, hist_dense: torch.Tensor, batch: Dict, seed: Optional[int]) -> torch.Tensor:
         raise NotImplementedError
diff --git a/newsreclib_amd/nrms_module.py b/newsreclib_amd/nrms_module.py
--- a/newsreclib_amd/nrms_module.py
+++ b/newsreclib_amd/nrms_module.py
@@ -81,18 +81,22 @@
         emb = getattr(te, "embedding_layer", None)
         return prepare_batch(batch, emb.weight.shape[0] if emb is not None else None)
 
-    def forward(self, batch: Dict) -> torch.Tensor:
-        batch = self._prepare(batch)
-        B = batch["batch_size"]
+    user_loss_fusable = True
+
+    def _news_vectors(self, batch: Dict):
         hist_text = batch["x_hist"][self._text_attr]
         n_hist = (hist_text if torch.is_tensor(hist_text) else next(iter(hist_text.values()))).shape[0]
         if self.hparams.use_plm:
             self.news_encoder.share_plm_bodies(batch["x_hist"], batch["x_cand"])
             hist_vec = self.news_encoder(batch["x_hist"])
             cand_vec = self.news_encoder(batch["x_cand"])
-            return self.score_news_vectors(hist_vec, cand_vec, batch)
+            return hist_vec, cand_vec
         news_vector = self.news_encoder(batch["x_all"])
-        return self.score_news_vectors(*ops.split_rows(news_vector, n_hist), batch)
+        return ops.split_rows(news_vector, n_hist)
+
+    def forward(self, batch: Dict) -> torch.Tensor:
+        batch = self._prepare(batch)
+        return self.score_news_vectors(*self._news_vectors(batch), batch)
 
     def _encode_user(self, hist_dense: torch.Tensor, batch: Dict, seed=None) -> torch.Tensor:
         return self.user_encoder(hist_dense)
diff --git a/newsreclib_amd/ops.py b/newsreclib_amd/ops.py
--- a/newsreclib_amd/ops.py
+++ b/newsreclib_amd/ops.py
@@ -248,6 +248,104 @@
             defer.keep.append((ws, hist, params, bufs))
         ctx.ws = None
         return (d_hist, *rets, None, None, None, None, None, None)
+
+
+def user_loss_fused_enabled() -> bool:
+    return os.environ.get("NRL_USER_LOSS_FUSED", "1") not in ("", "0")
+
+
+def user_loss_supported(B: int, H: int, D: int, heads: int, Q: int, C: int) -> bool:
+    if D % heads != 0:
+        return False
+    return bool(_lib.load().nrl_user_encoder_loss_supported(B, H, D, heads, Q, C, _lib.engine_code()))
+
+
+class UserEncoderLossFn(GradAwareFunction):
+
+    @staticmethod
+    def forward(ctx, hist, cand, y_true, w_in, b_in, w_o, b_o, w_a, b_a, q_a, heads, grad_bufs, grad_scale=1.0, p_drop=0.0,
+                seed=0, stream0=0):
+        lib = _lib.load()
+        hist = _chk(hist, torch.float32, "hist_news_vector")
+        cand = _chk(cand, torch.float32, "cand_news_vector")
+        y_true = _chk(y_true, torch.float32, "y_true")
+        params = [_chk(t, torch.float32, "user encoder parameter") for t in (w_in, b_in, w_o, b_o, w_a, b_a, q_a)]
+        if hist.dim() != 3 or cand.dim() != 3 or y_true.dim() != 2:
+            raise ValueError("newsreclib_amd: hist (batch, history, dim), cand (batch, candidates, dim), y_true (batch, candidates)")
+        B, H, D = hist.shape
+        C = cand.shape[1]
+        if cand.shape != (B, C, D) or y_true.shape != (B, C):
+            raise ValueError("newsreclib_amd: hist, cand and y_true disagree in shape")
+        engine, options = _lib.engine_code(), _lib.options_word()
+        bp = _block_params(params, heads, engine, options)
+        if bp.embed_dim != D:
+            raise ValueError("newsreclib_amd: hist feature dim does not match the encoder")
+        Q = bp.query_dim
+        dev = hist.device
+        ws = workspace(lib.nrl_user_encoder_workspace_bytes(B, H, D, heads, Q), dev)
+        user = torch.empty((B, D), dtype=torch.float32, device=dev)
+        scores = torch.empty((B, C), dtype=torch.float32, device=dev)
+        loss = torch.empty((), dtype=torch.float32, device=dev)
+        d_cand = torch.empty_like(cand)
+        small = torch.empty(B + B * Q + 1, dtype=torch.float32, device=dev)
+        dqa_rows = small[B:B + B * Q]
+        drop = (float(p_drop), int(seed), int(stream0))
+        _lib.check(lib.nrl_user_encoder_loss_fwd(ctypes.byref(bp), hist.data_ptr(), B, H, cand.data_ptr(), C, y_true.data_ptr(),
+                                                 float(grad_scale), *drop, user.data_ptr(), scores.data_ptr(), loss.data_ptr(),
+                                                 d_cand.data_ptr(), small.data_ptr(), dqa_rows.data_ptr(),
+                                                 small[B + B * Q:].data_ptr(), ws.data_ptr(), ws.numel(), _stream()),
+                   "nrl_user_encoder_loss_fwd")
+        ctx.mark_non_differentiable(scores, user)
+        ctx.set_materialize_grads(False)
+        if saving(ctx):
+            ctx.save_for_backward(hist, *params)
+            ctx.ws, ctx.d_cand, ctx.dqa_rows = ws, d_cand, dqa_rows
+            ctx.heads, ctx.grad_bufs, ctx.engine, ctx.options, ctx.drop = heads, grad_bufs, engine, options, drop
+            ctx.need_cand = ctx.needs_input_grad[1]
+        return loss, scores, user
+
+    @staticmethod
+    def backward(ctx, g, _g_scores=None, _g_user=None):
+        lib = _lib.load()
+        hist, *params = ctx.saved_tensors
+        B, H, D = hist.shape
+        bp = _block_params(params, ctx.heads, ctx.engine, ctx.options)
+        if g is None:
+            g = torch.zeros((), dtype=torch.float32, device=hist.device)
+        unit = g.data_ptr() in _UNIT_GRADS
+        bufs, rets = _grad_targets(params, ctx.grad_bufs if unit else None)
+        bg = _block_grads(bufs)
+        d_hist = torch.empty_like(hist)
+        ws, dqa_rows = ctx.ws, ctx.dqa_rows
+
+        def run(phase):
+            _lib.check(lib.nrl_user_encoder_loss_bwd_phase(ctypes.byref(bp), ctypes.byref(bg), hist.data_ptr(), B, H, *ctx.drop,
+                                                           d_hist.data_ptr(), dqa_rows.data_ptr(), phase, ws.data_ptr(),
+                                                           ws.numel(), _stream()), "nrl_user_encoder_loss_bwd_phase")
+
+        defer = deferred_weight_grads._active
+        if not unit or defer is None or any(r is not None for r in rets):
+            run(0)
+        else:
+            run(1)
+            defer.stream.wait_stream(torch.cuda.current_stream())
+            with torch.cuda.stream(defer.stream):
+                run(2)
+            defer.keep.append((ws, hist, params, bufs, dqa_rows))
+        d_cand = ctx.d_cand if ctx.need_cand else None
+        if not unit:
+            d_hist = d_hist * g
+            d_cand = d_cand * g if d_cand is not None else None
+            rets = []
+            for i, t in enumerate(bufs):
+                gb = ctx.grad_bufs[i] if ctx.grad_bufs is not None else None
+                if gb is not None:
+                    gb.add_(t * g)
+                    rets.append(None)
+                else:
+                    rets.append(t * g)
+        ctx.ws = ctx.d_cand = ctx.dqa_rows = None
+        return (d_hist, d_cand, None, *rets, None, None, None, None, None, None)
 
 
 class ToDenseBatchFn(GradAwareFunction):
diff --git a/newsreclib_amd/sentirec_module.py b/newsreclib_amd/sentirec_module.py
--- a/newsreclib_amd/sentirec_module.py
+++ b/newsreclib_amd/sentirec_module.py
@@ -11,6 +11,8 @@
 
 
 class SentiRecModule(NRMSModule):
+    user_loss_fusable = False
+
     def __init__(
         self,
         dataset_attributes: List[str],
```

Result: faster. 49180 impressions/s (median of 6 runs) (+1.2%).
